# qintonguav/e2e-parking-carla

Measured on AMD Instinct MI355X. Metric: train samples/sec (4-cam frames) at B=8, 1/2/4/8 MI355X; CPU-ref baseline, higher is better.
Workload: dtype f32; 1 GPU; ParkingModel train step (fwd + control/seg/depth losses + bwd + Adam), 4 cams x 256x256, fp32, random init; global_batch=8, batch_per_gpu=8, parallelism=dp1

## Files before the change

e2e-parking-carla_amd/csrc/abi.cpp:

```cpp
#include <stdarg.h>
#include <stdio.h>

#include "e2ep.h"
#include "tune.h"

namespace e2ep {
static thread_local char g_err[512] = "";
void set_error(const char *fmt, ...) {
  va_list ap;
  va_start(ap, fmt);
  vsnprintf(g_err, sizeof(g_err), fmt, ap);
  va_end(ap);
}
int g_tune[TUNE_N] = {8192, 4096, 512, 512, 768, 1024, 512, 1, 1, 2, 1, 2, 2, 1, 2, 1, 1, 1, 1, 1, 1, 2, 1024, 2, 2048, 2, 1, 1, 2, 1, 2, 1, 1, 1, 1, 4, 2};
}

extern "C" {
int e2ep_abi_version(void) { return 4; }
int e2ep_tune(int key, int value) {
  if (key < 0 || key >= e2ep::TUNE_N || key == e2ep::TUNE_RETIRED_27 ||
      key == e2ep::TUNE_RETIRED_29 || key == e2ep::TUNE_RETIRED_31)
    return -1;
  const int prev = e2ep::g_tune[key];
  if (value > 0) e2ep::g_tune[key] = value;
  return prev;
}
const char *e2ep_last_error(void) { return e2ep::g_err; }
}
```

e2e-parking-carla_amd/csrc/conv.hip:

```cpp
#include <algorithm>

#include "common.h"
#include "conv.h"
#include "gemm.h"
#include "bnstats.h"
#include "handoff.h"

#pragma clang fp contract(on)

namespace e2ep {

typedef float f32x16 __attribute__((ext_vector_type(16)));
typedef __bf16 bf16x8 __attribute__((ext_vector_type(8)));
typedef _Float16 f16x8 __attribute__((ext_vector_type(8)));

constexpr int BM = 64, BK = 16;
constexpr int PADA = 4, PADB = 4;
constexpr int MAXPH = 4;
template <int BNT, int BMT>
constexpr int conv_gemm_lds_floats() { return 2 * BK * (BMT + PADA) + 2 * BK * (BNT + PADB); }

template <int MODE, int ACT, int BNT, int BMT, bool AV, int OP, bool ST, typename TS = float,
          typename TD = float>
__device__ __forceinline__ void conv_gemm_block(
    const float *__restrict__ w, const TS *__restrict__ src, const float *__restrict__ bias,
    TD *__restrict__ dst, long long dst_bytes, ConvGeom g, int M, int splits, int kper,
    float *__restrict__ part, unsigned int *__restrict__ cnt, double *__restrict__ stats, int bx,
    int by, int bz, int gx, float *lds) {
  constexpr int WC = BMT == 64 ? BNT / 2 : BNT / 4;
  constexpr int NACC = WC / 32;
  constexpr int BROWS = 256 / BNT;
  constexpr int BPER = BK / BROWS;
  constexpr int NA = BK * BMT / 256;
  float(*As)[BK][BMT + PADA] = reinterpret_cast<float(*)[BK][BMT + PADA]>(lds);
  float(*Bs)[BK][BNT + PADB] = reinterpret_cast<float(*)[BK][BNT + PADB]>(lds + 2 * BK * (BMT + PADA));
  __shared__ int s_tdy[MAXTAPS], s_tdx[MAXTAPS], s_trs[MAXTAPS];
  __shared__ int s_ntaps;

  const int tid = threadIdx.x, lane = tid & 63;
  const int wave = __builtin_amdgcn_readfirstlane(tid >> 6);
  const int wm = BMT == 64 ? (wave & 1) : 0, wn = BMT == 64 ? (wave >> 1) : wave;
  const int m0 = by * BMT, n0 = bx * BNT;
  const int split = bz % splits, z = bz / splits;
  const int RS = g.R * g.S;

  int py = 0, px = 0, Hc, Wc;
  if (MODE == 0) {
    Hc = g.P; Wc = g.Q;
  } else {
    py = z / g.sw; px = z % g.sw;
    Hc = py < g.H ? (g.H - py + g.sh - 1) / g.sh : 0;
    Wc = px < g.W ? (g.W - px + g.sw - 1) / g.sw : 0;
  }
  const int HWc = Hc * Wc;
  const int Ntot = g.N * HWc;
  if (n0 >= Ntot) return;

  if (tid == 0) {
    int n = 0;
    for (int r = 0; r < g.R; ++r) {
      int dy;
      if (MODE == 0) {
        dy = r * g.dh - g.ph;
      } else {
        const int ny = py + g.ph - r * g.dh;
        if (((ny % g.sh) + g.sh) % g.sh) continue;
        dy = floordiv(ny, g.sh);
      }
      for (int s = 0; s < g.S; ++s) {
        int dx;
        if (MODE == 0) {
          dx = s * g.dw - g.pw;
          if (!axis_live(dy, g.P, g.sh, g.H) || !axis_live(dx, g.Q, g.sw, g.W)) continue;
        } else {
          const int nx = px + g.pw - s * g.dw;
          if (((nx % g.sw) + g.sw) % g.sw) continue;
          dx = floordiv(nx, g.sw);
          if (!axis_live(dy, Hc, 1, g.P) || !axis_live(dx, Wc, 1, g.Q)) continue;
        }
        s_tdy[n] = dy;
        s_tdx[n] = dx;
        s_trs[n] = r * g.S + s;
        ++n;
      }
    }
    s_ntaps = n;
  }
  __syncthreads();
  const int ntaps = s_ntaps;
  const int Kc = MODE == 0 ? g.Cin : g.Cout;
  const int csteps = (Kc + BK - 1) / BK;
  const int ksteps_all = ntaps * csteps;
  const int kbeg = split * kper;
  const int kend = min(ksteps_all, kbeg + kper);
  const int nk = max(0, kend - kbeg);

  const int Hs = MODE == 0 ? g.H : g.P, Ws = MODE == 0 ? g.W : g.Q;
  const int HWs = Hs * Ws;
  constexpr int ES = sizeof(TS);
  const __amdgpu_buffer_rsrc_t rw = rsrc(w, 4LL * g.Cout * g.Cin * RS);
  const __amdgpu_buffer_rsrc_t rx = rsrc(src, (long long)ES * g.N * Kc * HWs);

  const int bn = tid % BNT;
  const int bk0 = __builtin_amdgcn_readfirstlane(tid / BNT);
  const int ncol = n0 + bn;
  const bool col_ok = ncol < Ntot;
  int img = 0, cp = 0;
  if (col_ok) {
    img = ncol / HWc;
    cp = ncol - img * HWc;
  }
  const int cy = cp / Wc, cx = cp - cy * Wc;
  const int ybase = MODE == 0 ? cy * g.sh : cy;
  const int xbase = MODE == 0 ? cx * g.sw : cx;
  const int simg = img * Kc * HWs;

  const int am = MODE == 0 ? tid / (BK / NA) : (tid & (BMT - 1));
  const int ac = MODE == 0 ? NA * (tid % (BK / NA)) : 0;
  const int ak0 = BMT == 64 ? __builtin_amdgcn_readfirstlane(tid / BMT) : tid / BMT;
  const bool arow_ok = (m0 + am) < M;
  const bool tm = g.wlayout == 1;
  const int a_mstride = MODE == 0 ? (tm ? g.Cin : g.Cin * RS) : (tm ? 1 : RS);
  const int a_cstride = MODE == 0 ? (tm ? 1 : RS) : (tm ? g.Cin : g.Cin * RS);
  const int a_tstride = tm ? g.Cout * g.Cin : 1;
  static_assert(!AV || (MODE == 0 && NA == 4), "AV: forward 64-row tiles only");
  const int arow = (m0 + am) * a_mstride;

  const int nrw = (int)min(4LL * g.Cout * g.Cin * RS, 0x7fffffffLL);
  const int nrx = (int)min((long long)ES * g.N * Kc * HWs, 0x7fffffffLL);

  float ra0[NA], rb0[BPER], ra1[NA], rb1[BPER];
  const int klast = kend - 1;
  auto load_tiles = [&](int ks_in, float(&ra)[NA], float(&rb)[BPER]) {
    const bool live = ks_in <= klast;
    const int ks = min(ks_in, klast);
    const int tap = g.korder ? ks % ntaps : ks / csteps;
    const int c0 = (g.korder ? ks / ntaps : ks - tap * csteps) * BK;
    const int dy = s_tdy[tap], dx = s_tdx[tap], rs = s_trs[tap] * a_tstride;
    if (MODE == 0) {
      const int c = c0 + ac;
      if (AV) {
        const float4 v = bload4(rw, (live && arow_ok && c < Kc) ? (arow + c + rs) * 4 : OOR);
        ra[0] = v.x; ra[1] = v.y; ra[NA > 2 ? 2 : 0] = v.z; ra[NA > 3 ? 3 : 0] = v.w;
      } else {
        const int abase = (live && arow_ok) ? (arow + rs) * 4 : nrw;
#pragma unroll
        for (int j = 0; j < NA; ++j)
          ra[j] = bload(rw, c + j < Kc ? abase + (c + j) * a_cstride * 4 : OOR);
      }
    } else {
      const int abase = (live && arow_ok) ? (arow + rs) * 4 : nrw;
#pragma unroll
      for (int j = 0; j < NA; ++j) {
        const int c = c0 + ak0 + (256 / BMT) * j;
        const int rterm = c < Kc ? c * a_cstride * 4 : nrw;
        ra[j] = bload(rw, abase + rterm);
      }
    }
    const int iy = ybase + dy, ix = xbase + dx;
// ... 785 lines not shown
  long long cap = pix / 2048;
  long long s = want < cap ? want : cap;
  if (s < 1) s = 1;
  if (s > 4096) s = 4096;
  return (int)s;
}

static void wgrad1x1_tiles(const ConvGeom &g, int &to, int &tc) {
  auto wide = [](int c) { return 8LL * cdiv(c, 64) * 64 <= 9LL * cdiv(c, 32) * 32; };
  to = tc = 32;
  if ((long long)g.N * g.P * g.Q < 65536) return;
  const int wo = wide(g.Cout) ? 64 : 32, wc = wide(g.Cin) ? 64 : 32;
  if ((long long)cdiv(g.Cout, wo) * cdiv(g.Cin, wc) * wgrad1x1_splits_for(g, wo, wc) < 128) return;
  to = wo;
  tc = wc;
}

static int wgrad1x1_splits(const ConvGeom &g) {
  int to, tc;
  wgrad1x1_tiles(g, to, tc);
  return wgrad1x1_splits_for(g, to, tc);
}

template <int TI, int TJ, int OP>
__device__ __forceinline__ void wgrad1x1_block(const float *__restrict__ gout,
                                               const float *__restrict__ x,
                                               float *__restrict__ part, ConvGeom g, int splits,
                                               int groups_per_split, int bt, int split,
                                               float (*red)[64]) {
  constexpr int NT = TI * TJ;
  const int lane = threadIdx.x & 63, wave = threadIdx.x >> 6;
  const int ntj = (g.Cin + 32 * TJ - 1) / (32 * TJ);
  const int ti = bt / ntj, tj = bt - ti * ntj;
  const int PQ = g.P * g.Q;
  const int ngroups = g.N * PQ / 8;
  const int gb = split * groups_per_split;
  const int ge = min(ngroups, gb + groups_per_split);
  const int row = lane & 31, h = lane >> 5;
  const int co0 = ti * 32 * TI + row, ci0 = tj * 32 * TJ + row;
  const __amdgpu_buffer_rsrc_t rg = rsrc(gout, 4LL * g.N * g.Cout * PQ);
  const __amdgpu_buffer_rsrc_t rx = rsrc(x, 4LL * g.N * g.Cin * PQ);
  const int gpq = PQ / 8;
  f32x16 acc[NT];
#pragma unroll
  for (int t = 0; t < NT; ++t) acc[t] = f32x16{0};
  for (int g0 = gb + wave * W1_GROUPS; g0 < ge; g0 += 4 * W1_GROUPS) {
    float4 a[W1_GROUPS][TI], b[W1_GROUPS][TJ];
#pragma unroll
    for (int u = 0; u < W1_GROUPS; ++u) {
      const int grp = g0 + u;
      const bool ok = grp < ge;
      const int n = grp / gpq, p = (grp - n * gpq) * 8 + 4 * h;
#pragma unroll
      for (int i = 0; i < TI; ++i) {
        const int co = co0 + 32 * i;
        a[u][i] = bload4(rg, (ok && co < g.Cout) ? (((n * g.Cout + co) * PQ) + p) * 4 : OOR);
      }
#pragma unroll
      for (int j = 0; j < TJ; ++j) {
        const int ci = ci0 + 32 * j;
        b[u][j] = bload4(rx, (ok && ci < g.Cin) ? (((n * g.Cin + ci) * PQ) + p) * 4 : OOR);
      }
    }
    if (OP == 0) {
#pragma unroll
      for (int u = 0; u < W1_GROUPS; ++u)
#pragma unroll
        for (int i = 0; i < TI; ++i)
#pragma unroll
          for (int j = 0; j < TJ; ++j) {
            f32x16 &c = acc[i * TJ + j];
            c = __builtin_amdgcn_mfma_f32_32x32x2f32(a[u][i].x, b[u][j].x, c, 0, 0, 0);
            c = __builtin_amdgcn_mfma_f32_32x32x2f32(a[u][i].y, b[u][j].y, c, 0, 0, 0);
            c = __builtin_amdgcn_mfma_f32_32x32x2f32(a[u][i].z, b[u][j].z, c, 0, 0, 0);
            c = __builtin_amdgcn_mfma_f32_32x32x2f32(a[u][i].w, b[u][j].w, c, 0, 0, 0);
          }
    } else {
#pragma unroll
      for (int u = 0; u < W1_GROUPS; u += 2)
#pragma unroll
        for (int i = 0; i < TI; ++i)
#pragma unroll
          for (int j = 0; j < TJ; ++j) {
            const bf16x8 av = {(__bf16)a[u][i].x, (__bf16)a[u][i].y, (__bf16)a[u][i].z,
                               (__bf16)a[u][i].w, (__bf16)a[u + 1][i].x, (__bf16)a[u + 1][i].y,
                               (__bf16)a[u + 1][i].z, (__bf16)a[u + 1][i].w};
            const bf16x8 bv = {(__bf16)b[u][j].x, (__bf16)b[u][j].y, (__bf16)b[u][j].z,
                               (__bf16)b[u][j].w, (__bf16)b[u + 1][j].x, (__bf16)b[u + 1][j].y,
                               (__bf16)b[u + 1][j].z, (__bf16)b[u + 1][j].w};
            acc[i * TJ + j] = __builtin_amdgcn_mfma_f32_32x32x16_bf16(av, bv, acc[i * TJ + j], 0, 0, 0);
          }
    }
  }
  for (int w = 0; w < 4; ++w) {
    if (wave == w)
#pragma unroll
      for (int t = 0; t < NT; ++t)
#pragma unroll
        for (int r = 0; r < 16; ++r)
          red[t * 16 + r][lane] = w == 0 ? acc[t][r] : red[t * 16 + r][lane] + acc[t][r];
    __syncthreads();
  }
  const int Kw = g.Cin;
  for (int e = threadIdx.x; e < NT * 16 * 64; e += 256) {
    const int tr = e >> 6, l = e & 63;
    const int t = tr >> 4, r = tr & 15;
    const int i = (r & 3) + 8 * (r >> 2) + 4 * (l >> 5), j = l & 31;
    const int oc = ti * 32 * TI + 32 * (t / TJ) + i, ic = tj * 32 * TJ + 32 * (t % TJ) + j;
    if (oc < g.Cout && ic < g.Cin) {
      part[((long long)split * g.Cout + oc) * Kw + ic] = red[tr][l];
    }
  }
}

template <int TI, int TJ, int OP>
__global__ void __launch_bounds__(256) k_wgrad_1x1(const float *__restrict__ gout,
                                                   const float *__restrict__ x,
                                                   float *__restrict__ part, ConvGeom g,
                                                   int splits, int groups_per_split) {
  __shared__ float red[TI * TJ * 16][64];
  wgrad1x1_block<TI, TJ, OP>(gout, x, part, g, splits, groups_per_split, blockIdx.x, blockIdx.y,
                             red);
}

template <int BNT, int BMT, int TI, int TJ>
__global__ void __launch_bounds__(256, 2) k_conv_bwd_pair1x1(
    const float *__restrict__ w, const float *__restrict__ gout, const float *__restrict__ res,
    float *__restrict__ dx, long long dx_bytes, ConvGeom g, int M, int splits, int kper,
    float *__restrict__ part1, unsigned int *__restrict__ cnt, int gx1, int gy1, int gz1,
    const float *__restrict__ x, float *__restrict__ part2, int splits2, int gps, int nt2,
    int wfirst) {
  constexpr int L1 = conv_gemm_lds_floats<BNT, BMT>();
  constexpr int L2 = TI * TJ * 16 * 64;
  __shared__ __attribute__((aligned(16))) float lds[L1 > L2 ? L1 : L2];
  const int n1 = gx1 * gy1 * gz1, n2 = nt2 * splits2;
  const int id = wfirst ? ((int)blockIdx.x >= n2 ? (int)blockIdx.x - n2 : n1 + (int)blockIdx.x)
                        : (int)blockIdx.x;
  if (id < n1) {
    conv_gemm_block<1, 0, BNT, BMT, false, 0, false>(w, gout, res, dx, dx_bytes, g, M, splits, kper,
                                                     part1, cnt, nullptr, id % gx1,
                                                     (id / gx1) % gy1, id / (gx1 * gy1), gx1, lds);
  } else {
    const int j = id - n1;
    wgrad1x1_block<TI, TJ, 0>(gout, x, part2, g, splits2, gps, j % nt2, j / nt2,
                              reinterpret_cast<float(*)[64]>(lds));
  }
}

__global__ void __launch_bounds__(1024) k_reduce_splits(const float *__restrict__ part, int splits,
                                                        int n, float *__restrict__ out,
                                                        int accumulate, int RS,
                                                        unsigned long long mask) {
  __shared__ float red[16][64];
  const int o = threadIdx.x & 63, r = threadIdx.x >> 6;
  const int i = blockIdx.x * 64 + o;
  const bool live = (mask >> (i % RS)) & 1ULL;
  float s0 = 0.f, s1 = 0.f, s2 = 0.f, s3 = 0.f;
  if (i < n && live) {
    int k = r;
    for (; k + 48 < splits; k += 64) {
      s0 += part[(size_t)(k + 0) * n + i];
      s1 += part[(size_t)(k + 16) * n + i];
      s2 += part[(size_t)(k + 32) * n + i];
      s3 += part[(size_t)(k + 48) * n + i];
    }
    for (; k < splits; k += 16) s0 += part[(size_t)k * n + i];
  }
  red[r][o] = (s0 + s1) + (s2 + s3);
  __syncthreads();
  if (r == 0 && i < n) {
    float s = 0.f;
#pragma unroll
    for (int j = 0; j < 16; ++j) s += red[j][o];
    out[i] = accumulate ? out[i] + s : s;
  }
}

__global__ void __launch_bounds__(256) k_reduce_splits4(const float *__restrict__ part, int splits,
                                                         int n, float *__restrict__ out,
                                                         int accumulate, int RS,
                                                         unsigned long long mask) {
  const int i = (blockIdx.x * 256 + threadIdx.x) * 4;
  if (i >= n) return;
  float4 acc = *reinterpret_cast<const float4 *>(part + i);
#pragma unroll 8
  for (int k = 1; k < splits; ++k) {
    const float4 v = *reinterpret_cast<const float4 *>(part + (size_t)k * n + i);
    acc.x += v.x;
    acc.y += v.y;
    acc.z += v.z;
    acc.w += v.w;
  }
  float r[4] = {acc.x, acc.y, acc.z, acc.w};
#pragma unroll
  for (int e = 0; e < 4; ++e)
    if (!((mask >> ((i + e) % RS)) & 1ULL)) r[e] = 0.f;
  float4 o = make_float4(r[0], r[1], r[2], r[3]);
  if (accumulate) {
    const float4 a = *reinterpret_cast<const float4 *>(out + i);
    o.x += a.x; o.y += a.y; o.z += a.z; o.w += a.w;
  }
  *reinterpret_cast<float4 *>(out + i) = o;
}

static void reduce_splits(const float *part, int splits, int n, float *out, int accumulate, int RS,
                          unsigned long long mask, hipStream_t s) {
  if (n % 4 == 0 && n >= 131072 && splits <= 64 && (reinterpret_cast<uintptr_t>(part) & 15) == 0 &&
      (reinterpret_cast<uintptr_t>(out) & 15) == 0)
    hipLaunchKernelGGL(k_reduce_splits4, dim3(cdiv(n / 4, 256)), dim3(256), 0, s, part, splits, n,
                       out, accumulate, RS, mask);
  else
    hipLaunchKernelGGL(k_reduce_splits, dim3(cdiv(n, 64)), dim3(1024), 0, s, part, splits, n, out,
                       accumulate, RS, mask);
}

constexpr int COLSUM_ROWS = 128;
__global__ void __launch_bounds__(256) k_col_sum_partial(const float *__restrict__ g, int rows,
                                                         int C, float *__restrict__ part) {
  const int tx = threadIdx.x & 63, ty = threadIdx.x >> 6;
  const int c = blockIdx.x * 64 + tx;
  const int r0 = blockIdx.y * COLSUM_ROWS, r1 = min(rows, r0 + COLSUM_ROWS);
  float s = 0.f;
  if (c < C) {
    float t[COLSUM_ROWS / 4];
#pragma unroll
    for (int u = 0; u < COLSUM_ROWS / 4; ++u) {
      const int r = r0 + ty + 4 * u;
      t[u] = r < r1 ? g[(long long)r * C + c] : 0.f;
    }
#pragma unroll
    for (int u = 0; u < COLSUM_ROWS / 4; ++u) s += t[u];
  }
  __shared__ float red[4][64];
  red[ty][tx] = s;
  __syncthreads();
  if (ty == 0 && c < C)
    part[(long long)blockIdx.y * C + c] = (red[0][tx] + red[1][tx]) + (red[2][tx] + red[3][tx]);
}

__global__ void k_col_sum_final(const float *__restrict__ part, int chunks, int C,
                                float *__restrict__ out) {
  const int c = blockIdx.x * blockDim.x + threadIdx.x;
  if (c >= C) return;
  float s = 0.f;
  for (int k0 = 0; k0 < chunks; k0 += 16) {
    float t[16];
#pragma unroll
    for (int u = 0; u < 16; ++u) t[u] = k0 + u < chunks ? part[(long long)(k0 + u) * C + c] : 0.f;
#pragma unroll
    for (int u = 0; u < 16; ++u) s += t[u];
  }
  out[c] = s;
}

__global__ void __launch_bounds__(1024) k_bias_grad(const float *__restrict__ g, int N, int C,
                                                    int HW, float *__restrict__ db) {
  const int c = blockIdx.x;
  float s = 0.f;
  if ((HW & 3) == 0) {
    const int HW4 = HW >> 2, tot = N * HW4;
    for (int t = threadIdx.x; t < tot; t += 1024) {
      const int n = t / HW4, p = t - n * HW4;
      const float4 v = *reinterpret_cast<const float4 *>(g + ((size_t)n * C + c) * HW + 4 * p);
      s += (v.x + v.y) + (v.z + v.w);
    }
  } else {
    const int tot = N * HW;
    for (int t = threadIdx.x; t < tot; t += 1024) {
      const int n = t / HW, p = t - n * HW;
      s += g[((size_t)n * C + c) * HW + p];
    }
  }
  __shared__ float red[16];
  s = wave_sum(s);
  if ((threadIdx.x & 63) == 0) red[threadIdx.x >> 6] = s;
  __syncthreads();
  if (threadIdx.x == 0) {
    float t = 0.f;
    for (int w = 0; w < 16; ++w) t += red[w];
    db[c] = t;
  }
}

__global__ void __launch_bounds__(256) k_skinny_gemm(const float *__restrict__ A, int ai, int ak,
                                                     const float *__restrict__ B, int bk, int bj,
                                                     const float *__restrict__ bias, int Mi, int Nj,
                                                     int K, float *__restrict__ C) {
  const int o = blockIdx.x * 4 + (threadIdx.x >> 6);
  if (o >= Mi * Nj) return;
  const int i = o / Nj, j = o - i * Nj;
  const int lane = threadIdx.x & 63;
  float s = 0.f;
  for (int k = lane; k < K; k += 64) s += A[(size_t)i * ai + (size_t)k * ak] * B[(size_t)k * bk + (size_t)j * bj];
  s = wave_sum(s);
  if (lane == 0) C[o] = s + (bias ? bias[j] : 0.f);
}

constexpr int DK = 32;

__device__ __forceinline__ int dk_w_index(const ConvGeom &g, int co, int k) {
  const int RS = g.R * g.S, ci = k / RS, rs = k - ci * RS;
  return g.wlayout == 1 ? (rs * g.Cout + co) * g.Cin + ci : (co * g.Cin + ci) * RS + rs;
}

__device__ __forceinline__ void dk_gather(const ConvGeom &g, const __amdgpu_buffer_rsrc_t &rx,
                                          int img, int oy, int ox, bool ok, float (&xin)[DK]) {
  const int RS = g.R * g.S, K = g.Cin * RS;
#pragma unroll
  for (int k = 0; k < DK; ++k) {
    const int ci = k / RS, rs = k - ci * RS, r = rs / g.S, sx = rs - r * g.S;
    const int iy = oy * g.sh - g.ph + r * g.dh, ix = ox * g.sw - g.pw + sx * g.dw;
    const bool in = ok && k < K && (unsigned)iy < (unsigned)g.H && (unsigned)ix < (unsigned)g.W;
    xin[k] = bload(rx, in ? (((img * g.Cin + ci) * g.H + iy) * g.W + ix) * 4 : OOR);
  }
}

constexpr int DCO = 64, DCH = 16;
__global__ void __launch_bounds__(256) k_conv_direct(const float *__restrict__ x,
                                                     const float *__restrict__ w,
                                                     const float *__restrict__ bias, ConvGeom g,
                                                     int act, float *__restrict__ y) {
  __shared__ float4 wl[DK][DCO / 4];
  __shared__ float xs[DK][256];
  const int K = g.Cin * g.R * g.S;
  for (int e = threadIdx.x; e < DK * DCO; e += 256) {
    const int k = e / DCO, co = e - k * DCO;
    reinterpret_cast<float *>(wl)[e] = (k < K && co < g.Cout) ? w[dk_w_index(g, co, k)] : 0.f;
  }
  const int PQ = g.P * g.Q;
  const int pix = blockIdx.x * 256 + threadIdx.x;
  const bool ok = pix < g.N * PQ;
  const int img = ok ? pix / PQ : 0, pq = ok ? pix - img * PQ : 0;
  const int oy = pq / g.Q, ox = pq - oy * g.Q;
  {
    const __amdgpu_buffer_rsrc_t rx = rsrc(x, 4LL * g.N * g.Cin * g.H * g.W);
    float xin[DK];
    dk_gather(g, rx, img, oy, ox, ok, xin);
#pragma unroll
    for (int k = 0; k < DK; ++k) xs[k][threadIdx.x] = xin[k];
  }
  __syncthreads();
  float *yp = y + (size_t)img * g.Cout * PQ + pq;
#pragma unroll 1
  for (int c0 = 0; c0 < g.Cout; c0 += DCH) {
    float acc[DCH];
#pragma unroll
    for (int j = 0; j < DCH; ++j) acc[j] = 0.f;
#pragma unroll 4
    for (int k = 0; k < K; ++k) {
      const float xv = xs[k][threadIdx.x];
#pragma unroll
      for (int j4 = 0; j4 < DCH / 4; ++j4) {
        const float4 wv = wl[k][c0 / 4 + j4];
        acc[4 * j4 + 0] = __builtin_fmaf(xv, wv.x, acc[4 * j4 + 0]);
        acc[4 * j4 + 1] = __builtin_fmaf(xv, wv.y, acc[4 * j4 + 1]);
        acc[4 * j4 + 2] = __builtin_fmaf(xv, wv.z, acc[4 * j4 + 2]);
        acc[4 * j4 + 3] = __builtin_fmaf(xv, wv.w, acc[4 * j4 + 3]);
      }
    }
    if (ok) {
#pragma unroll
// ... 753 lines not shown
```

e2e-parking-carla_amd/csrc/ln.hip:

```cpp
#include "common.h"
#include "dropout.h"

namespace e2ep {

constexpr int LN_MAXV = 8;

__global__ void __launch_bounds__(256) k_add_drop_ln_fwd(
    const float *__restrict__ a, const float *__restrict__ b, const float *__restrict__ u,
    const int *__restrict__ seed, float p, float scale, const float *__restrict__ gamma,
    const float *__restrict__ beta, int rows, int E, float eps, float *__restrict__ x,
    float *__restrict__ y, float *__restrict__ mean, float *__restrict__ rstd) {
  const int row = blockIdx.x * 4 + (threadIdx.x >> 6), lane = threadIdx.x & 63;
  if (row >= rows) return;
  const size_t base = (size_t)row * E;
  const bool hashed = !u && seed && p > 0.f;
  const uint32_t sm_ = hashed ? att_seedmix(seed) : 0u;
  float v[LN_MAXV];
  float s = 0.f;
#pragma unroll
  for (int j = 0; j < LN_MAXV; ++j) {
    const int c = lane + 64 * j;
    v[j] = 0.f;
    if (c < E) {
      float bv = b ? b[base + c] : 0.f;
      if (u) bv = u[base + c] >= p ? bv * scale : 0.f;
      else if (hashed) bv = att_keep(sm_, (uint32_t)(base + c), p) ? bv * scale : 0.f;
      v[j] = a[base + c] + bv;
      s += v[j];
    }
  }
  const float mu = wave_sum(s) / (float)E;
  float q = 0.f;
#pragma unroll
  for (int j = 0; j < LN_MAXV; ++j) {
    const int c = lane + 64 * j;
    if (c < E) {
      const float d = v[j] - mu;
      q += d * d;
    }
  }
  const float r = rsqrtf(wave_sum(q) / (float)E + eps);
#pragma unroll
  for (int j = 0; j < LN_MAXV; ++j) {
    const int c = lane + 64 * j;
    if (c < E) {
      if (x) x[base + c] = v[j];
      y[base + c] = (v[j] - mu) * r * (gamma ? gamma[c] : 1.f) + (beta ? beta[c] : 0.f);
    }
  }
  if (lane == 0) {
    mean[row] = mu;
    rstd[row] = r;
  }
}

constexpr int LN_ROWS_PER_WAVE = 1;

__global__ void __launch_bounds__(256) k_add_drop_ln_bwd(
    const float *__restrict__ dy, const float *__restrict__ x, const float *__restrict__ mean,
    const float *__restrict__ rstd, const float *__restrict__ gamma, const float *__restrict__ u,
    const int *__restrict__ seed, float p, float scale, int rows, int E, float *__restrict__ da,
    float *__restrict__ db, float *__restrict__ part) {
  const bool hashed = !u && seed && p > 0.f;
  const uint32_t sm_ = hashed ? att_seedmix(seed) : 0u;
  __shared__ float sg[4][LN_MAXV * 64], sb[4][LN_MAXV * 64];
  const int wave = threadIdx.x >> 6, lane = threadIdx.x & 63;
  float pg[LN_MAXV], pb[LN_MAXV];
#pragma unroll
  for (int j = 0; j < LN_MAXV; ++j) pg[j] = pb[j] = 0.f;
  const int r0 = (blockIdx.x * 4 + wave) * LN_ROWS_PER_WAVE;
  for (int i = 0; i < LN_ROWS_PER_WAVE; ++i) {
    const int row = r0 + i;
    if (row >= rows) break;
    const size_t base = (size_t)row * E;
    const float mu = mean[row], rs = rstd[row];
    float xh[LN_MAXV], gy[LN_MAXV];
    float s1 = 0.f, s2 = 0.f;
#pragma unroll
    for (int j = 0; j < LN_MAXV; ++j) {
      const int c = lane + 64 * j;
      xh[j] = gy[j] = 0.f;
      if (c < E) {
        const float g = dy[base + c];
        xh[j] = (x[base + c] - mu) * rs;
        gy[j] = g * (gamma ? gamma[c] : 1.f);
        pg[j] += g * xh[j];
        pb[j] += g;
        s1 += gy[j];
        s2 += gy[j] * xh[j];
      }
    }
    const float c1 = wave_sum(s1) / (float)E, c2 = wave_sum(s2) / (float)E;
#pragma unroll
    for (int j = 0; j < LN_MAXV; ++j) {
      const int c = lane + 64 * j;
      if (c < E) {
        const float dx = rs * (gy[j] - c1 - xh[j] * c2);
        if (da) da[base + c] = dx;
        if (db)
          db[base + c] = u        ? (u[base + c] >= p ? dx * scale : 0.f)
                         : hashed ? (att_keep(sm_, (uint32_t)(base + c), p) ? dx * scale : 0.f)
                                  : dx;
      }
    }
  }
  if (!part) return;
#pragma unroll
  for (int j = 0; j < LN_MAXV; ++j) {
    sg[wave][lane + 64 * j] = pg[j];
    sb[wave][lane + 64 * j] = pb[j];
  }
  __syncthreads();
  for (int c = threadIdx.x; c < E; c += 256) {
    part[(size_t)blockIdx.x * E + c] = (sg[0][c] + sg[1][c]) + (sg[2][c] + sg[3][c]);
    part[((size_t)gridDim.x + blockIdx.x) * E + c] = (sb[0][c] + sb[1][c]) + (sb[2][c] + sb[3][c]);
  }
}

__global__ void __launch_bounds__(1024) k_ln_param_grads(const float *__restrict__ part, int nblk,
                                                         int E, float *__restrict__ dgamma,
                                                         float *__restrict__ dbeta) {
  __shared__ float red[16][64];
  const int o = threadIdx.x & 63, r = threadIdx.x >> 6;
  const int c = blockIdx.x * 64 + o;
  const float *pp = part + (size_t)blockIdx.y * nblk * E;
  float s = 0.f;
  if (c < E)
    for (int k = r; k < nblk; k += 16) s += pp[(size_t)k * E + c];
  red[r][o] = s;
  __syncthreads();
  if (r == 0 && c < E) {
    float t = 0.f;
#pragma unroll
    for (int j = 0; j < 16; ++j) t += red[j][o];
    float *out = blockIdx.y == 0 ? dgamma : dbeta;
    if (out) out[c] = t;
  }
}

}

using namespace e2ep;

extern "C" {

static int add_drop_ln_fwd(const float *a, const float *b, const float *u, const int *seed,
                           float p, const float *gamma, const float *beta, int rows, int E,
                           float eps, float *x, float *y, float *mean, float *rstd,
                           hipStream_t stream) {
  E2EP_REQUIRE(rows > 0 && E > 0, E2EP_EINVAL, "e2ep_add_drop_ln_fwd: bad shape");
  E2EP_REQUIRE(E <= 64 * LN_MAXV, E2EP_ERANGE, "e2ep_add_drop_ln_fwd: E %d > %d", E, 64 * LN_MAXV);
  E2EP_REQUIRE(p >= 0.f && p < 1.f, E2EP_EINVAL, "e2ep_add_drop_ln_fwd: p must be in [0, 1)");
  E2EP_REQUIRE((long long)rows * E < 0xffffffffLL, E2EP_ERANGE, "e2ep_add_drop_ln_fwd: too large");
  const float scale = 1.f / (1.f - p);
  hipLaunchKernelGGL(k_add_drop_ln_fwd, dim3(cdiv(rows, 4)), dim3(256), 0, stream, a, b, u, seed,
                     p, scale, gamma, beta, rows, E, eps, x, y, mean, rstd);
  return launch_status("e2ep_add_drop_ln_fwd");
}

int e2ep_add_drop_ln_fwd(const float *a, const float *b, const float *u, float p,
                         const float *gamma, const float *beta, int rows, int E, float eps,
                         float *x, float *y, float *mean, float *rstd, void *stream) {
  return add_drop_ln_fwd(a, b, u, nullptr, p, gamma, beta, rows, E, eps, x, y, mean, rstd,
                         as_stream(stream));
}

int e2ep_add_drop_ln_fwd_seeded(const float *a, const float *b, const int *seed, float p,
                                const float *gamma, const float *beta, int rows, int E, float eps,
                                float *x, float *y, float *mean, float *rstd, void *stream) {
  E2EP_REQUIRE(seed || p == 0.f, E2EP_EINVAL, "e2ep_add_drop_ln_fwd_seeded: seed required for p > 0");
  return add_drop_ln_fwd(a, b, nullptr, seed, p, gamma, beta, rows, E, eps, x, y, mean, rstd,
                         as_stream(stream));
}

size_t e2ep_add_drop_ln_bwd_workspace(int rows, int E) {
  return (size_t)2 * cdiv(rows, 4 * LN_ROWS_PER_WAVE) * E * sizeof(float);
}

static int add_drop_ln_bwd(const float *dy, const float *x, const float *mean, const float *rstd,
                           const float *gamma, const float *u, const int *seed, float p, int rows,
                           int E, float *da, float *db, float *dgamma, float *dbeta,
                           void *workspace, hipStream_t stream) {
  E2EP_REQUIRE(rows > 0 && E > 0, E2EP_EINVAL, "e2ep_add_drop_ln_bwd: bad shape");
  E2EP_REQUIRE(E <= 64 * LN_MAXV, E2EP_ERANGE, "e2ep_add_drop_ln_bwd: E %d > %d", E, 64 * LN_MAXV);
  const float scale = 1.f / (1.f - p);
  const int nblk = cdiv(rows, 4 * LN_ROWS_PER_WAVE);
  float *part = (dgamma || dbeta) ? static_cast<float *>(workspace) : nullptr;
  E2EP_REQUIRE(!(dgamma || dbeta) || workspace, E2EP_EINVAL, "e2ep_add_drop_ln_bwd: workspace needed");
  hipLaunchKernelGGL(k_add_drop_ln_bwd, dim3(nblk), dim3(256), 0, stream, dy, x, mean, rstd,
                     gamma, u, seed, p, scale, rows, E, da, db, part);
  if (part)
    hipLaunchKernelGGL(k_ln_param_grads, dim3(cdiv(E, 64), 2), dim3(1024), 0, stream, part, nblk,
                       E, dgamma, dbeta);
  return launch_status("e2ep_add_drop_ln_bwd");
}

int e2ep_add_drop_ln_bwd(const float *dy, const float *x, const float *mean, const float *rstd,
                         const float *gamma, const float *u, float p, int rows, int E,
                         float *da, float *db, float *dgamma, float *dbeta, void *workspace,
                         void *stream) {
  return add_drop_ln_bwd(dy, x, mean, rstd, gamma, u, nullptr, p, rows, E, da, db, dgamma, dbeta,
                         workspace, as_stream(stream));
}

int e2ep_add_drop_ln_bwd_seeded(const float *dy, const float *x, const float *mean,
                                const float *rstd, const float *gamma, const int *seed, float p,
                                int rows, int E, float *da, float *db, float *dgamma,
                                float *dbeta, void *workspace, void *stream) {
  E2EP_REQUIRE(seed || p == 0.f, E2EP_EINVAL, "e2ep_add_drop_ln_bwd_seeded: seed required for p > 0");
  return add_drop_ln_bwd(dy, x, mean, rstd, gamma, nullptr, seed, p, rows, E, da, db, dgamma,
                         dbeta, workspace, as_stream(stream));
}

}
```

e2e-parking-carla_amd/csrc/se.hip:

```cpp
#include "common.h"

#pragma clang fp contract(on)

namespace e2ep {

constexpr int SE_MAXC = 4096, SE_MAXSQ = 256;
constexpr int SE_U = 4;

__device__ __forceinline__ float sigm(float v) { return sigmoid_f(v); }

struct SeIn {
  const float *sc, *sh;
  int C;
};
__device__ __forceinline__ float se_in(float v, float sc, float sh, bool t) {
  if (!t) return v;
  const float z = v * sc + sh;
  return swish_f(z);
}
__device__ __forceinline__ float4 se_in4(float4 v, float sc, float sh, bool t) {
  return make_float4(se_in(v.x, sc, sh, t), se_in(v.y, sc, sh, t), se_in(v.z, sc, sh, t),
                     se_in(v.w, sc, sh, t));
}

template <typename TX>
__device__ __forceinline__ float plane_sum(const TX *__restrict__ p, int HW, int lane,
                                           float sc, float sh, bool t) {
  float s = 0.f;
  if ((HW & 3) == 0) {
    const int HW4 = HW >> 2;
    for (int i0 = lane; i0 < HW4; i0 += 64 * SE_U) {
      float4 v[SE_U];
#pragma unroll
      for (int u = 0; u < SE_U; ++u) v[u] = ld4(p + 4 * min(i0 + u * 64, HW4 - 1));
#pragma unroll
      for (int u = 0; u < SE_U; ++u) {
        if (i0 + u * 64 >= HW4) break;
        const float4 w = se_in4(v[u], sc, sh, t);
        s += (w.x + w.y) + (w.z + w.w);
      }
    }
  } else {
    for (int i = lane; i < HW; i += 64) s += se_in(ld1(p + i), sc, sh, t);
  }
  return wave_sum(s);
}

template <typename TX>
__global__ void __launch_bounds__(256) k_se_squeeze(const TX *__restrict__ x, SeIn tf,
                                                    int planes, int HW,
                                                    float *__restrict__ pooled) {
  const int pl = blockIdx.x * 4 + (threadIdx.x >> 6);
  if (pl >= planes) return;
  const bool t = tf.sc != nullptr;
  const int c = pl % tf.C;
  const float s = plane_sum(x + (size_t)pl * HW, HW, threadIdx.x & 63, t ? tf.sc[c] : 1.f,
                            t ? tf.sh[c] : 0.f, t);
  if ((threadIdx.x & 63) == 0) pooled[pl] = s / (float)HW;
}

__global__ void __launch_bounds__(256) k_se_hidden(const float *__restrict__ pooled,
                                                   const float *__restrict__ w1,
                                                   const float *__restrict__ b1, int C, int sq,
                                                   float *__restrict__ hpre) {
  const int n = blockIdx.x, k = blockIdx.y * 4 + (threadIdx.x >> 6), lane = threadIdx.x & 63;
  if (k >= sq) return;
  const float *pn = pooled + (size_t)n * C, *wr = w1 + (size_t)k * C;
  float s0 = 0.f, s1 = 0.f;
  int c = lane;
  for (; c + 64 < C; c += 128) {
    s0 += wr[c] * pn[c];
    s1 += wr[c + 64] * pn[c + 64];
  }
  if (c < C) s0 += wr[c] * pn[c];
  const float s = wave_sum(s0 + s1);
  if (lane == 0) hpre[(size_t)n * sq + k] = s + (b1 ? b1[k] : 0.f);
}

constexpr int SE_CT = 32, SE_NT = 8;
__global__ void __launch_bounds__(256) k_se_logits(const float *__restrict__ hpre,
                                                   const float *__restrict__ w2,
                                                   const float *__restrict__ b2, int N, int C,
                                                   int sq, float *__restrict__ a) {
  extern __shared__ float lds[];
  const int ld = sq + 1;
  float *sw = lds, *sh = lds + SE_CT * ld;
  const int c0 = blockIdx.x * SE_CT, n0 = blockIdx.y * SE_NT;
  const int nc = min(SE_CT, C - c0), nn = min(SE_NT, N - n0);
  const float *src = w2 + (size_t)c0 * sq;
  for (int e = threadIdx.x; e < nc * sq; e += 256) {
    const int r = e / sq;
    sw[r * ld + (e - r * sq)] = src[e];
  }
  for (int e = threadIdx.x; e < nn * sq; e += 256) {
    const float z = hpre[(size_t)n0 * sq + e];
    sh[e] = z * sigm(z);
  }
  __syncthreads();
  const int ci = threadIdx.x % SE_CT, ni = threadIdx.x / SE_CT;
  if (ci >= nc || ni >= nn) return;
  const float *wr = sw + ci * ld, *hr = sh + ni * sq;
  float s = 0.f;
#pragma unroll 4
  for (int k = 0; k < sq; ++k) s += wr[k] * hr[k];
  a[(size_t)(n0 + ni) * C + c0 + ci] = s + (b2 ? b2[c0 + ci] : 0.f);
}

template <typename TX, typename TY = float>
__global__ void __launch_bounds__(256) k_se_excite(const TX *__restrict__ x, SeIn tf,
                                                   const float *__restrict__ a, int HW,
                                                   long long nvec, int vec,
                                                   TY *__restrict__ y) {
  const int i = (int)(blockIdx.x * blockDim.x + threadIdx.x);
  if (i >= nvec) return;
  const bool t = tf.sc != nullptr;
  const int pl = vec ? i / (HW >> 2) : i / HW;
  const int c = pl % tf.C;
  const float sc = t ? tf.sc[c] : 1.f, sh = t ? tf.sh[c] : 0.f;
  const float s = sigm(a[pl]);
  if (vec) {
    float4 v = se_in4(ld4(x + 4 * i), sc, sh, t);
    v.x *= s; v.y *= s; v.z *= s; v.w *= s;
    st4(y + 4 * i, v);
  } else {
    st1(y + i, se_in(ld1(x + i), sc, sh, t) * s);
  }
}

constexpr int SE_XP = 8;
template <typename TX, typename TY = float>
__global__ void __launch_bounds__(256) k_se_excite_mlp(const TX *__restrict__ x, SeIn tf,
                                                       const float *__restrict__ hpre,
                                                       const float *__restrict__ w2,
                                                       const float *__restrict__ b2, int sq,
                                                       float *__restrict__ a, int HW,
                                                       long long nvec, int vec,
                                                       TY *__restrict__ y) {
  __shared__ float sg[SE_XP];
  const int per = vec ? (HW >> 2) : HW;
  const int i0 = (int)(blockIdx.x * blockDim.x);
  const int last = (int)min((long long)i0 + (long long)blockDim.x, nvec) - 1;
  const int p0 = i0 / per, p1 = last / per;
  const int lane = threadIdx.x & 63, wv = threadIdx.x >> 6;
  for (int p = p0 + wv; p <= p1; p += 4) {
    const int n = p / tf.C, c = p - n * tf.C;
    const float *hr = hpre + (size_t)n * sq, *wr = w2 + (size_t)c * sq;
    float acc = 0.f;
    for (int k = lane; k < sq; k += 64) {
      const float z = hr[k];
      acc += wr[k] * (z * sigm(z));
    }
    acc = wave_sum(acc);
    const float av = acc + (b2 ? b2[c] : 0.f);
// ... 23 lines not shown
  const float *mean, *invstd, *gamma, *beta;
  double *sums;
};

template <bool BNS, typename TX, typename TD = float>
__global__ void __launch_bounds__(256) k_se_da(const TX *__restrict__ x, SeIn tf,
                                               const TD *__restrict__ dy,
                                               const float *__restrict__ a, int planes, int HW,
                                               float *__restrict__ da, SeBn bn) {
  const int pl = blockIdx.x * 4 + (threadIdx.x >> 6), lane = threadIdx.x & 63;
  if (pl >= planes) return;
  const bool t = tf.sc != nullptr;
  const int c = pl % tf.C;
  const float sc = t ? tf.sc[c] : 1.f, sh = t ? tf.sh[c] : 0.f;
  float mu = 0.f, is = 1.f, gm = 1.f, bt = 0.f;
  if constexpr (BNS) {
    mu = bn.mean[c];
    is = bn.invstd[c];
    gm = bn.gamma ? bn.gamma[c] : 1.f;
    bt = bn.beta ? bn.beta[c] : 0.f;
  }
  double s1 = 0.0, s2 = 0.0, s3 = 0.0, s4 = 0.0;
  const TX *xp = x + (size_t)pl * HW;
  const TD *gp = dy + (size_t)pl * HW;
  float acc = 0.f;
  if ((HW & 3) == 0) {
    const int HW4 = HW >> 2;
    for (int i0 = lane; i0 < HW4; i0 += 64 * SE_U) {
      float4 xv[SE_U], gv[SE_U];
#pragma unroll
      for (int u = 0; u < SE_U; ++u) {
        const int i = min(i0 + u * 64, HW4 - 1);
        xv[u] = ld4(xp + 4 * i);
        gv[u] = ld4(gp + 4 * i);
      }
#pragma unroll
      for (int u = 0; u < SE_U; ++u) {
        if (i0 + u * 64 >= HW4) break;
        const float4 g = gv[u];
        if constexpr (BNS) {
          const float xv4[4] = {xv[u].x, xv[u].y, xv[u].z, xv[u].w};
          const float gv4[4] = {g.x, g.y, g.z, g.w};
          float a0 = 0.f, a1 = 0.f, a2 = 0.f, a3 = 0.f, a4 = 0.f;
#pragma unroll
          for (int j = 0; j < 4; ++j) {
            const float xh = (xv4[j] - mu) * is;
            const float zb = xh * gm + bt;
            const float sg = sigmoid_f(zb);
            const float sp = sg * (1.f + zb * (1.f - sg));
            a0 += (zb * sg) * gv4[j];
            a1 += gv4[j] * sp;
            a2 += sp;
            a3 += gv4[j] * sp * xh;
            a4 += sp * xh;
          }
          acc += a0;
          s1 += a1; s2 += a2; s3 += a3; s4 += a4;
        } else {
          const float4 w = se_in4(xv[u], sc, sh, t);
          acc += (w.x * g.x + w.y * g.y) + (w.z * g.z + w.w * g.w);
        }
      }
    }
  } else {
    for (int i = lane; i < HW; i += 64) {
      const float xv = ld1(xp + i), g = ld1(gp + i);
      if constexpr (BNS) {
        const float xh = (xv - mu) * is;
        const float zb = xh * gm + bt;
        const float sg = sigmoid_f(zb);
        const float sp = sg * (1.f + zb * (1.f - sg));
        acc += (zb * sg) * g;
        s1 += g * sp; s2 += sp; s3 += g * sp * xh; s4 += sp * xh;
      } else {
        acc += se_in(xv, sc, sh, t) * g;
      }
    }
  }
  acc = wave_sum(acc);
  if constexpr (BNS) {
#pragma unroll
    for (int o = 32; o > 0; o >>= 1) {
      s1 += __shfl_xor(s1, o, 64);
      s2 += __shfl_xor(s2, o, 64);
      s3 += __shfl_xor(s3, o, 64);
      s4 += __shfl_xor(s4, o, 64);
    }
    if (lane == 0) {
      double *o = bn.sums + 4LL * pl;
      o[0] = s1; o[1] = s2; o[2] = s3; o[3] = s4;
    }
  }
  if (lane == 0) {
    const float s = sigm(a[pl]);
    da[pl] = acc * s * (1.f - s);
  }
}

constexpr int SE_DH_SPAN = 256;
static_assert(SE_MAXC / SE_DH_SPAN == 16, "e2ep_se_bwd workspace (e2ep.h) holds 16 dh partials");
__global__ void __launch_bounds__(256) k_se_dh(const float *__restrict__ da,
                                               const float *__restrict__ w2, int C, int sq, int KT,
                                               float *__restrict__ dhp) {
  __shared__ float red[256];
  const int n = blockIdx.x, j = blockIdx.y;
  const int k = threadIdx.x % KT, sl = threadIdx.x / KT, nsl = 256 / KT;
  const int cb = j * SE_DH_SPAN, ce = min(C, cb + SE_DH_SPAN);
  const float *dn = da + (size_t)n * C;
  float s = 0.f;
  if (k < sq)
#pragma unroll 4
    for (int c = cb + sl; c < ce; c += nsl) s += w2[(size_t)c * sq + k] * dn[c];
  red[threadIdx.x] = s;
  __syncthreads();
  if (threadIdx.x < KT && k < sq) {
    float t = 0.f;
    for (int q = 0; q < nsl; ++q) t += red[q * KT + k];
    dhp[((size_t)n * gridDim.y + j) * sq + k] = t;
  }
}

__global__ void __launch_bounds__(256) k_se_dpooled(const float *__restrict__ dhp, int spans,
                                                    const float *__restrict__ hpre,
                                                    const float *__restrict__ w1, int C, int sq,
                                                    float *__restrict__ dhpre,
                                                    float *__restrict__ dpooled) {
  __shared__ float sd[SE_MAXSQ];
  const int n = blockIdx.x;
  for (int k = threadIdx.x; k < sq; k += 256) {
    float t = 0.f;
    for (int j = 0; j < spans; ++j) t += dhp[((size_t)n * spans + j) * sq + k];
    const float z = hpre[(size_t)n * sq + k], sg = sigm(z);
    const float g = t * (sg * (1.f + z * (1.f - sg)));
    if (blockIdx.y == 0) dhpre[(size_t)n * sq + k] = g;
    sd[k] = g;
  }
  __syncthreads();
  const int c = blockIdx.y * 256 + threadIdx.x;
  if (c < C) {
    float s = 0.f;
#pragma unroll 8
    for (int k = 0; k < sq; ++k) s += w1[(size_t)k * C + c] * sd[k];
    dpooled[(size_t)n * C + c] = s;
  }
}

__global__ void __launch_bounds__(256) k_se_wgrad(const float *__restrict__ pooled,
                                                  const float *__restrict__ hpre,
                                                  const float *__restrict__ da,
                                                  const float *__restrict__ dhpre, int N, int C,
                                                  int sq, float *__restrict__ dw1,
                                                  float *__restrict__ db1, float *__restrict__ dw2,
                                                  float *__restrict__ db2) {
  const int i = blockIdx.x * blockDim.x + threadIdx.x;
  const int n1 = sq * C, n2 = C * sq;
  float s = 0.f;
  if (i < n1) {
    const int k = i / C, c = i - k * C;
#pragma unroll 8
    for (int n = 0; n < N; ++n) s += dhpre[(size_t)n * sq + k] * pooled[(size_t)n * C + c];
    if (dw1) dw1[i] = s;
  } else if (i < n1 + n2) {
    const int j = i - n1, c = j / sq, k = j - c * sq;
#pragma unroll 8
    for (int n = 0; n < N; ++n) {
      const float z = hpre[(size_t)n * sq + k];
      s += da[(size_t)n * C + c] * (z * sigm(z));
    }
    if (dw2) dw2[j] = s;
  } else if (i < n1 + n2 + sq) {
    const int k = i - n1 - n2;
#pragma unroll 8
    for (int n = 0; n < N; ++n) s += dhpre[(size_t)n * sq + k];
    if (db1) db1[k] = s;
  } else if (i < n1 + n2 + sq + C) {
    const int c = i - n1 - n2 - sq;
#pragma unroll 8
    for (int n = 0; n < N; ++n) s += da[(size_t)n * C + c];
    if (db2) db2[c] = s;
  }
}

__global__ void __launch_bounds__(256) k_se_dx(const float *__restrict__ dy,
                                               const float *__restrict__ a,
                                               const float *__restrict__ dpooled, int HW,
                                               long long nvec, int vec, float *__restrict__ dx) {
  const long long i = (long long)blockIdx.x * blockDim.x + threadIdx.x;
  if (i >= nvec) return;
  const float inv = 1.f / (float)HW;
  if (vec) {
    const long long pl = i / (HW >> 2);
    const float s = sigm(a[pl]), d = dpooled[pl] * inv;
    float4 g = reinterpret_cast<const float4 *>(dy)[i];
    g.x = g.x * s + d; g.y = g.y * s + d; g.z = g.z * s + d; g.w = g.w * s + d;
    reinterpret_cast<float4 *>(dx)[i] = g;
  } else {
    const long long pl = i / HW;
    dx[i] = dy[i] * sigm(a[pl]) + dpooled[pl] * inv;
  }
}

}

using namespace e2ep;

static int se_fwd_impl(const void *x, const float *x_scale, const float *x_shift, const float *w1,
                       const float *b1, const float *w2, const float *b2, int N, int C, int HW, int sq,
                       float *pooled, float *hpre, float *a, void *y, void *stream, int io,
                       bool squeeze) {
  E2EP_REQUIRE(io == 0 || ((io == E2EP_IO_X_BF16 || io == (E2EP_IO_X_BF16 | E2EP_IO_DX_BF16)) &&
                           HW % 4 == 0),
               E2EP_EINVAL, "e2ep_se_fwd: storage mask %d not supported (0, X or X|DX bf16, "
               "HW %% 4 == 0)", io);
  E2EP_REQUIRE(N > 0 && C > 0 && HW > 0 && sq > 0, E2EP_EINVAL, "e2ep_se_fwd: bad shape");
  E2EP_REQUIRE(!x_scale == !x_shift, E2EP_EINVAL, "e2ep_se_fwd: x_scale / x_shift both or neither");
  const SeIn tf{x_scale, x_shift, C};
  E2EP_REQUIRE(C <= SE_MAXC && sq <= SE_MAXSQ, E2EP_ERANGE, "e2ep_se_fwd: C %d > %d or sq %d > %d",
               C, SE_MAXC, sq, SE_MAXSQ);
  hipStream_t s = as_stream(stream);
  const int planes = N * C;
  const int vec = (HW & 3) == 0;
  const long long nvec = (long long)planes * HW / (vec ? 4 : 1);
  E2EP_REQUIRE(nvec < (1LL << 29), E2EP_ERANGE, "e2ep_se_fwd: %lld vectors >= 2^29", nvec);
  if (!squeeze)
    ;
  else if (io)
    hipLaunchKernelGGL(k_se_squeeze<bf16_t>, dim3(cdiv(planes, 4)), dim3(256), 0, s,
                       static_cast<const bf16_t *>(x), tf, planes, HW, pooled);
  else
    hipLaunchKernelGGL(k_se_squeeze<float>, dim3(cdiv(planes, 4)), dim3(256), 0, s,
                       static_cast<const float *>(x), tf, planes, HW, pooled);
  hipLaunchKernelGGL(k_se_hidden, dim3(N, cdiv(sq, 4)), dim3(256), 0, s, pooled, w1, b1, C, sq,
                     hpre);
  const int per = vec ? HW / 4 : HW;
  if (g_tune[TUNE_SE_EXCITE_MLP] == 2 && cdiv(256, per) + 1 <= SE_XP) {
#define E2EP_SEX(TXV, TYV)                                                                      \
  hipLaunchKernelGGL((k_se_excite_mlp<TXV, TYV>), dim3(cdiv(nvec, 256)), dim3(256), 0, s,       \
                     static_cast<const TXV *>(x), tf, hpre, w2, b2, sq, a, HW, nvec, vec,        \
                     static_cast<TYV *>(y))
    if (io & E2EP_IO_DX_BF16) E2EP_SEX(bf16_t, bf16_t);
    else if (io) E2EP_SEX(bf16_t, float);
    else E2EP_SEX(float, float);
#undef E2EP_SEX
    return launch_status("e2ep_se_fwd");
  }
  hipLaunchKernelGGL(k_se_logits, dim3(cdiv(C, SE_CT), cdiv(N, SE_NT)), dim3(256),
                     (SE_CT * (sq + 1) + SE_NT * sq) * sizeof(float), s, hpre, w2, b2, N, C, sq, a);
  if (io & E2EP_IO_DX_BF16)
    hipLaunchKernelGGL((k_se_excite<bf16_t, bf16_t>), dim3(cdiv(nvec, 256)), dim3(256), 0, s,
                       static_cast<const bf16_t *>(x), tf, a, HW, nvec, vec, static_cast<bf16_t *>(y));
  else if (io)
    hipLaunchKernelGGL((k_se_excite<bf16_t, float>), dim3(cdiv(nvec, 256)), dim3(256), 0, s,
                       static_cast<const bf16_t *>(x), tf, a, HW, nvec, vec, static_cast<float *>(y));
  else
    hipLaunchKernelGGL((k_se_excite<float, float>), dim3(cdiv(nvec, 256)), dim3(256), 0, s,
                       static_cast<const float *>(x), tf, a, HW, nvec, vec, static_cast<float *>(y));
  return launch_status("e2ep_se_fwd");
}

extern "C" {

int e2ep_se_fwd(const void *x, const float *x_scale, const float *x_shift, const float *w1,
                const float *b1, const float *w2, const float *b2, int N, int C, int HW, int sq,
                float *pooled, float *hpre, float *a, void *y, void *stream, int io) {
  return se_fwd_impl(x, x_scale, x_shift, w1, b1, w2, b2, N, C, HW, sq, pooled, hpre, a, y, stream,
                     io, true);
}

int e2ep_se_fwd_pooled(const void *x, const float *x_scale, const float *x_shift, const float *w1,
                       const float *b1, const float *w2, const float *b2, int N, int C, int HW,
                       int sq, const float *pooled, float *hpre, float *a, void *y, void *stream,
                       int io) {
  E2EP_REQUIRE(pooled, E2EP_EINVAL, "e2ep_se_fwd_pooled: pooled is required");
  return se_fwd_impl(x, x_scale, x_shift, w1, b1, w2, b2, N, C, HW, sq,
                     const_cast<float *>(pooled), hpre, a, y, stream, io, false);
}

static int se_bwd_impl(const void *x, int io, const float *x_scale, const float *x_shift,
                       const void *dy, const float *w1, const float *w2, const float *pooled,
                       const float *hpre, const float *a, int N, int C, int HW, int sq, float *dx,
                       float *dpooled_out, float *dw1, float *db1, float *dw2, float *db2,
                       float *workspace, const SeBn &bn, void *stream) {
  E2EP_REQUIRE(N > 0 && C > 0 && HW > 0 && sq > 0, E2EP_EINVAL, "e2ep_se_bwd: bad shape");
  E2EP_REQUIRE(!x_scale == !x_shift, E2EP_EINVAL, "e2ep_se_bwd: x_scale / x_shift both or neither");
  E2EP_REQUIRE(io == 0 || ((io == E2EP_IO_X_BF16 || io == (E2EP_IO_X_BF16 | E2EP_IO_DY_BF16)) &&
                           HW % 4 == 0 && !dx),
               E2EP_EINVAL, "e2ep_se_bwd: storage mask %d not supported (0, X or X|DY bf16 with "
               "dx formed by the BN backward, HW %% 4 == 0)", io);
  E2EP_REQUIRE(!(x_scale && dx), E2EP_EINVAL,
               "e2ep_se_bwd: with an input transform dx is formed by e2ep_bn_bwd (gate_logit / "
               "gate_dpooled); pass dx = NULL");
  const SeIn tf{x_scale, x_shift, C};
  E2EP_REQUIRE(C <= SE_MAXC && sq <= SE_MAXSQ, E2EP_ERANGE, "e2ep_se_bwd: C %d > %d or sq %d > %d",
               C, SE_MAXC, sq, SE_MAXSQ);
  hipStream_t s = as_stream(stream);
  const int planes = N * C;
  float *da = workspace, *dhpre = workspace + 2 * planes;
  float *dpooled = dpooled_out ? dpooled_out : workspace + planes;
  float *dhp = workspace + 2 * planes + N * sq;
  const int spans = cdiv(C, SE_DH_SPAN);
  int KT = 1;
  while (KT < sq) KT *= 2;
  const float *xf = static_cast<const float *>(x);
  const bf16_t *xh = static_cast<const bf16_t *>(x);
  const float *df = static_cast<const float *>(dy);
  const bf16_t *dh = static_cast<const bf16_t *>(dy);
  const dim3 gda(cdiv(planes, 4));
  const bool hx = io & E2EP_IO_X_BF16, hd = io & E2EP_IO_DY_BF16;
#define SE_DA(BNSV)                                                                                   \
  do {                                                                                                \
    if (hx && hd)                                                                                     \
      hipLaunchKernelGGL((k_se_da<BNSV, bf16_t, bf16_t>), gda, dim3(256), 0, s, xh, tf, dh, a, planes, \
                         HW, da, bn);                                                                 \
    else if (hx)                                                                                      \
      hipLaunchKernelGGL((k_se_da<BNSV, bf16_t, float>), gda, dim3(256), 0, s, xh, tf, df, a, planes, \
                         HW, da, bn);                                                                 \
    else                                                                                              \
      hipLaunchKernelGGL((k_se_da<BNSV, float, float>), gda, dim3(256), 0, s, xf, tf, df, a, planes,  \
                         HW, da, bn);                                                                 \
  } while (0)
  if (bn.sums) SE_DA(true);
  else SE_DA(false);
#undef SE_DA
  hipLaunchKernelGGL(k_se_dh, dim3(N, spans), dim3(256), 0, s, da, w2, C, sq, KT, dhp);
  hipLaunchKernelGGL(k_se_dpooled, dim3(N, cdiv(C, 256)), dim3(256), 0, s, dhp, spans, hpre, w1,
                     C, sq, dhpre, dpooled);
  if (dw1 || db1 || dw2 || db2) {
    const int outs = 2 * sq * C + sq + C;
    hipLaunchKernelGGL(k_se_wgrad, dim3(cdiv(outs, 256)), dim3(256), 0, s, pooled, hpre, da, dhpre,
                       N, C, sq, dw1, db1, dw2, db2);
  }
  if (dx) {
    const int vec = (HW & 3) == 0;
    const long long nvec = (long long)planes * HW / (vec ? 4 : 1);
    hipLaunchKernelGGL(k_se_dx, dim3(cdiv(nvec, 256)), dim3(256), 0, s, static_cast<const float *>(dy), a,
                       dpooled, HW, nvec, vec, dx);
  }
  return launch_status("e2ep_se_bwd");
}

int e2ep_se_bwd(const void *x, const float *x_scale, const float *x_shift, const void *dy,
                const float *w1, const float *w2, const float *pooled, const float *hpre,
                const float *a, int N, int C, int HW, int sq, float *dx, float *dpooled_out,
                float *dw1, float *db1, float *dw2, float *db2, float *workspace, void *stream,
                int io) {
  return se_bwd_impl(x, io, x_scale, x_shift, dy, w1, w2, pooled, hpre, a, N, C, HW, sq, dx,
                     dpooled_out, dw1, db1, dw2, db2, workspace, SeBn{}, stream);
}

int e2ep_se_bwd_bn(const void *x, const float *x_scale, const float *x_shift,
                   const float *bn_mean, const float *bn_invstd, const float *gamma,
                   const float *beta, const void *dy, const float *w1, const float *w2,
                   const float *pooled, const float *hpre, const float *a, int N, int C, int HW,
                   int sq, float *dpooled_out, float *dw1, float *db1, float *dw2, float *db2,
                   double *plane_sums, float *workspace, void *stream, int io) {
  E2EP_REQUIRE(x_scale && x_shift && bn_mean && bn_invstd && dpooled_out && plane_sums,
               E2EP_EINVAL, "e2ep_se_bwd_bn: the BN transform, its statistics, dpooled_out and "
               "plane_sums are required");
  return se_bwd_impl(x, io, x_scale, x_shift, dy, w1, w2, pooled, hpre, a, N, C, HW, sq, nullptr,
                     dpooled_out, dw1, db1, dw2, db2, workspace,
                     SeBn{bn_mean, bn_invstd, gamma, beta, plane_sums}, stream);
}

}
```

e2e-parking-carla_amd/csrc/tune.h:

```cpp
#pragma once

namespace e2ep {
enum Tune {
  TUNE_BN_SPLIT_TARGET = 0,
  TUNE_BN_SPLIT_MIN = 1,
  TUNE_BN_APPLY_PER = 2,
  TUNE_DW_WGRAD_TARGET = 3,
  TUNE_GEMM_SPLIT_TARGET = 4,
  TUNE_WGRAD1X1_TARGET = 5,
  TUNE_CONV_WIDE_MIN = 6,
  TUNE_CONV_FORCE_TILE = 7,
  TUNE_CONV_FORCE_SPLITS = 8,
  TUNE_WGRAD_GEN = 9,
  TUNE_LP_FORCE_TILE = 10,
  TUNE_LP = 11,
  TUNE_LP_WGRAD = 12,
  TUNE_LP_WGRAD_TILE = 13,
  TUNE_LP32 = 14,
  TUNE_LP32W = 15,
  TUNE_LP_LK = 16,
  TUNE_LPW_LK = 17,
  TUNE_KORDER = 18,
  TUNE_XCD = 19,
  TUNE_ATT_LANES = 20,
  TUNE_ATT_MF = 21,
  TUNE_LPW_TARGET = 22,
  TUNE_DW_VEC = 23,
  TUNE_DW_FWD_BLOCKS = 24,
  TUNE_BNS_WIDE = 25,
  TUNE_BNS_WIDE_LO = 26,
  TUNE_RETIRED_27 = 27,
  TUNE_SPLITK_FOLD = 28,
  TUNE_RETIRED_29 = 29,
  TUNE_PAIR1X1_ORDER = 30,
  TUNE_RETIRED_31 = 31,
  TUNE_LSS_FWD = 32,
  TUNE_BN_ORDER = 33,
  TUNE_SE_EXCITE_MLP = 34,
  TUNE_STEM_DIRECT = 35,
  TUNE_MBCONV_MID = 36,
  TUNE_N = 37
};
extern int g_tune[TUNE_N];
}
```

e2e-parking-carla_amd/e2ep_amd/_lib.py:

```python
import ctypes
import os

import torch

_HERE = os.path.dirname(os.path.abspath(__file__))
LIB_PATH = os.environ.get("E2EP_LIB", os.path.join(_HERE, "libe2ep_hip.so"))

_p, _i, _i64, _f, _sz = ctypes.c_void_p, ctypes.c_int, ctypes.c_longlong, ctypes.c_float, ctypes.c_size_t
_d = ctypes.c_double
_fp3 = ctypes.POINTER(ctypes.c_float)

SIGNATURES = {
    "e2ep_abi_version": (_i, []),
    "e2ep_last_error": (ctypes.c_char_p, []),
    "e2ep_rig_transforms": (_i, [_p, _p, _i, _p, _p, _p]),
    "e2ep_geom_index": (_i, [_p, _p, _p, _fp3, _fp3, _i, _i, _i, _i, _i, _i, _i, _i, _p, _p]),
    "e2ep_lss_plan_workspace": (_sz, [_i, _i]),
    "e2ep_lss_tiles": (_i, [_i]),
    "e2ep_debug_fwd_trace": (_i, [_p]),
    "e2ep_lss_plan": (_i, [_p, _i, _i, _i, _i, _i, _i, _p, _p, _p, _p, _sz, _p]),
    "e2ep_lss_fwd": (_i, [_p, _p, _p, _p, _p, _i, _i, _i, _i, _i, _i, _p, _i64, _p]),
    "e2ep_lss_bwd": (_i, [_p, _p, _p, _p, _i, _i, _i, _i, _i, _i, _p, _p, _p]),
    "e2ep_transpose": (_i, [_p, _i64, _i, _i, _i, _p, _p]),
    "e2ep_transpose_multi": (_i, [_p, _i, _i, _p]),
    "e2ep_target_bev": (_i, [_p, _p, _i, _i, _i, _f, _f, _p, _i64, _p]),
    "e2ep_conv_fwd_workspace": (_sz, [_p]),
    "e2ep_conv_fwd": (_i, [_p, _p, _p, _p, _i, _i, _p, _p, _sz, _p, _i]),
    "e2ep_conv_fwd_stats_tiles": (_i, [_p, _i]),
    "e2ep_conv_fwd_stats": (_i, [_p, _p, _p, _p, _i, _i, _p, _p, _sz, _p, _sz, _p, _i]),
    "e2ep_conv_dgrad_workspace": (_sz, [_p, _i]),
    "e2ep_conv_dgrad": (_i, [_p, _p, _p, _i, _i, _p, _p, _sz, _p]),
    "e2ep_conv_dgrad_acc": (_i, [_p, _p, _p, _i, _i, _p, _p, _p, _sz, _p, _i]),
    "e2ep_conv_gemm_variant": (_i, [_i]),
    "e2ep_conv_split_params": (_i, [_i, _i, _i]),
    "e2ep_conv_precision": (_i, [_i]),
    "e2ep_gemm_precision": (_i, [_i]),
    "e2ep_fusion_tokens_fwd": (_i, [_p, _p, _p, _i, _i, _i, _i, _f, _p, _p, _p]),
    "e2ep_fusion_tokens_bwd": (_i, [_p, _i, _i, _i, _i, _f, _p, _p, _p, _p, _p]),
    "e2ep_embed_tokens_fwd": (_i, [_p, _i, _p, _i, _p, _i, _i, _i, _f, _p, _p, _p]),
    "e2ep_embed_tokens_bwd": (_i, [_p, _p, _i, _i, _i, _i, _i, _f, _p, _p, _p, _p]),
    "e2ep_conv_wgrad_kstep": (_i, [_i]),
    "e2ep_conv_wgrad_splits": (_i, [_p]),
    "e2ep_conv_wgrad_workspace": (_sz, [_p, _i]),
    "e2ep_conv_wgrad": (_i, [_p, _p, _p, _i, _p, _sz, _p, _i, _p, _i]),
    "e2ep_conv_bwd_pair_ok": (_i, [_p, _i]),
    "e2ep_conv_bwd": (_i, [_p, _p, _p, _p, _i, _p, _p, _p, _sz, _i, _p, _sz, _p, _p, _i]),
    "e2ep_bias_grad": (_i, [_p, _i, _i, _i, _p, _p]),
    "e2ep_col_sum_workspace": (_sz, [_i, _i]),
    "e2ep_col_sum": (_i, [_p, _i, _i, _p, _p, _p]),
    "e2ep_skinny_gemm": (_i, [_p, _i, _i, _p, _i, _i, _p, _i, _i, _i, _p, _p]),
    "e2ep_bn_workspace": (_sz, [_i, _i, _i, _i]),
    "e2ep_bn_fwd": (_i, [_p, _p, _p, _p, _p, _f, _p, _p, _i, _i, _i, _i, _i, _f, _f, _i, _p, _p, _p, _p, _sz, _p]),
    "e2ep_bn_stats": (_i, [_p, _p, _p, _p, _p, _i, _i, _i, _i, _i, _f, _f, _p, _p, _p, _p, _p, _sz, _p, _i]),
    "e2ep_bn_fwd_split": (_i, [_i, _i, _i, _i]),
    "e2ep_bn_finalize_part_workspace": (_sz, [_i, _i]),
    "e2ep_bn_finalize_part": (_i, [_p, _i, _p, _p, _p, _p, _i, _i, _i, _i, _f, _f, _p, _p, _p, _p, _p, _sz, _p]),
    "e2ep_bn_apply": (_i, [_p, _p, _p, _p, _p, _f, _i, _i, _i, _i, _i, _p, _p]),
    "e2ep_bn_bwd": (_i, [_p, _p, _p, _p, _p, _p, _p, _p, _f, _p, _p, _i, _i, _i, _i, _i, _i, _p, _p, _p, _p, _p, _sz, _p, _i]),
    "e2ep_act_fwd": (_i, [_p, _i64, _i, _p, _p]),
    "e2ep_act_bwd": (_i, [_p, _p, _i64, _i, _p, _p]),
    "e2ep_cat_channels": (_i, [_p, _p, _i, _i, _i64, _p, _p]),
    "e2ep_split_channels": (_i, [_p, _p, _i, _i, _i64, _p, _p]),
    "e2ep_sum3": (_i, [_p, _p, _p, _p, _p]),
    "e2ep_add_f32": (_i, [_p, _p, _i64, _p, _p]),
    "e2ep_rng_draw": (_i, [_p, _i, _p, _i, _p, _p]),
    "e2ep_eq_mask_i64": (_i, [_p, _i64, _i, _i, _i64, _p, _p]),
    "e2ep_add_i64_multi": (_i, [_p, _i, _i64, _p]),
    "e2ep_resize_fwd": (_i, [_p, _i, _i, _i64, _i, _i, _i, _i, _f, _f, _p, _i64, _p]),
    "e2ep_resize_bwd_workspace": (_sz, [_i, _i, _i]),
    "e2ep_resize_bwd": (_i, [_p, _i64, _i, _i, _i, _i, _i, _f, _f, _p, _i, _p, _p]),
    "e2ep_resize_bwd_cl": (_i, [_p, _i64, _i, _i, _i, _i, _i, _i, _f, _f, _p, _p]),
    "e2ep_dwconv_fwd": (_i, [_p, _p, _p, _p, _p, _i, _p, _p]),
    "e2ep_dwconv_fwd_stats_tiles": (_i, [_p]),
    "e2ep_dwconv_fwd_stats": (_i, [_p, _p, _p, _p, _p, _i, _p, _p, _sz, _p, _i]),
    "e2ep_dwconv_dgrad": (_i, [_p, _p, _p, _p, _p, _i]),
    "e2ep_dwconv_wgrad_workspace": (_sz, [_p]),
    "e2ep_dwconv_wgrad": (_i, [_p, _p, _p, _p, _p, _i, _p, _sz, _p, _p, _i]),
    "e2ep_dwconv_bwd_pair_ok": (_i, [_p]),
    "e2ep_dwconv_bwd": (_i, [_p, _p, _p, _p, _p, _p, _i, _p, _p, _sz, _p, _p, _i]),
    "e2ep_maxpool3s2_fwd": (_i, [_p, _i, _i, _i, _p, _p, _p]),
    "e2ep_maxpool3s2_bwd": (_i, [_p, _p, _i, _i, _i, _p, _p]),
    "e2ep_avgpool_fwd": (_i, [_p, _i, _i, _p, _p]),
    "e2ep_avgpool_bwd": (_i, [_p, _i, _i, _p, _p]),
    "e2ep_add_drop_ln_fwd": (_i, [_p, _p, _p, _f, _p, _p, _i, _i, _f, _p, _p, _p, _p, _p]),
    "e2ep_add_drop_ln_bwd_workspace": (_sz, [_i, _i]),
    "e2ep_add_drop_ln_fwd_seeded": (_i, [_p, _p, _p, _f, _p, _p, _i, _i, _f, _p, _p, _p, _p, _p]),
    "e2ep_add_drop_ln_bwd_seeded": (_i, [_p, _p, _p, _p, _p, _p, _f, _i, _i, _p, _p, _p, _p, _p, _p]),
    "e2ep_add_drop_ln_bwd": (_i, [_p, _p, _p, _p, _p, _p, _f, _i, _i, _p, _p, _p, _p, _p, _p]),
    "e2ep_attn_fwd": (_i, [_p, _p, _p] + [_i] * 11 + [_f, _i, _p, _f, _p, _p, _p, _p]),
    "e2ep_attn_weights": (_i, [_p, _p, _p] + [_i] * 9 + [_f, _i, _p, _i, _p, _p]),
    "e2ep_attn_bwd_workspace": (_sz, [_i, _i, _i]),
    "e2ep_attn_bwd": (_i, [_p] * 6 + [_i] * 11 + [_f, _i, _p, _f, _p, _p, _p, _p, _p, _p]),
    "e2ep_attn_bwd_part": (_i, [_p] * 6 + [_i] * 11 + [_f, _i, _p, _f, _p, _p, _p, _p, _p, _i, _p]),
    "e2ep_attn_keep_mask": (_i, [_p, _i, _i, _i, _f, _p, _p]),
    "e2ep_softmax_c_fwd": (_i, [_p, _i, _i, _i, _p, _p]),
    "e2ep_softmax_c_bwd": (_i, [_p, _p, _i, _i, _i, _p, _p]),
    "e2ep_relu_dropout_fwd": (_i, [_p, _i64, _f, _p, _p, _p]),
    "e2ep_relu_dropout_bwd": (_i, [_p, _p, _i64, _f, _p, _p, _p]),
    "e2ep_se_fwd": (_i, [_p, _p, _p, _p, _p, _p, _p, _i, _i, _i, _i, _p, _p, _p, _p, _p, _i]),
    "e2ep_se_fwd_pooled": (_i, [_p, _p, _p, _p, _p, _p, _p, _i, _i, _i, _i, _p, _p, _p, _p, _p, _i]),
    "e2ep_mbconv_mid_ok": (_i, [_p]),
    "e2ep_mbconv_mid_fwd": (_i, [_p, _p, _p, _p, _p, _p, _p, _f, _f, _p, _p, _p, _p, _p, _f, _f, _p, _p, _p, _p]),
    "e2ep_mbconv_mid_bwd": (_i, [_p] * 20),
    "e2ep_se_bwd": (_i, [_p, _p, _p, _p, _p, _p, _p, _p, _p, _i, _i, _i, _i, _p, _p, _p, _p, _p, _p, _p, _p, _i]),
    "e2ep_se_bwd_bn": (_i, [_p, _p, _p, _p, _p, _p, _p, _p, _p, _p, _p, _p, _p, _i, _i, _i, _i, _p, _p, _p, _p, _p, _p, _p, _p, _i]),
    "e2ep_bn_bwd_planes": (_i, [_p, _p, _p, _p, _p, _p, _p, _p, _p, _i, _i, _i, _i, _i, _p, _p, _p, _p, _i]),
    "e2ep_bn_bwd_split": (_i, [_i, _i, _i, _i]),
    "e2ep_bn_eval_multi": (_i, [_p, _i, _p]),
    "e2ep_se_gate_fwd": (_i, [_p, _p, _i, _i, _p, _p]),
    "e2ep_se_gate_bwd": (_i, [_p, _p, _p, _i, _i, _p, _p, _p]),
    "e2ep_adam_chunk_elems": (_i, []),
    "e2ep_adam_step": (_i, [_p, _i, _p, _p, _p, _p, _p, _p, _p, _p, _d, _d, _d, _d, _f, _p, _p]),
    "e2ep_grad_gather": (_i, [_p, _i, _p, _p, _p, _p]),
    "e2ep_grad_sqnorm": (_i, [_p, _i, _p, _p, _p, _p, _p]),
    "e2ep_grad_norm_finalize": (_i, [_p, _i, _f, _d, _i, _p, _p, _p, _p, _p]),
    "e2ep_adam_step_clipped": (_i, [_p, _i, _p, _p, _p, _p, _p, _p, _p, _p, _d, _d, _d, _d, _f,
                                    _p, _p, _p, _p]),
    "e2ep_grad_accumulate": (_i, [_p, _i, _p, _p, _p, _p]),
    "e2ep_graph_replace_memsets": (_i, [_p, ctypes.POINTER(_i)]),
    "e2ep_graph_exec_create": (_i, [_p, _p]),
    "e2ep_graph_exec_launch": (_i, [_p, _p]),
    "e2ep_graph_exec_destroy": (_i, [_p]),
    "e2ep_capture_unjoined": (_i, [_p, _p, ctypes.POINTER(_i)]),
    "e2ep_tokens_init": (_i, [_p, _i, _i, _i, _p, _i, _i64, _p]),
    "e2ep_token_argmax_append": (_i, [_p, _i64, _i, _i, _p, _i, _i, _p]),
    "e2ep_dec_self_attn": (_i, [_p, _i, _p, _p, _f, _p, _i, _p, _p, _p, _i, _i64, _p, _p, _p, _p,
                                _i, _i, _i, _i, _i, _p]),
    "e2ep_dec_cross_attn": (_i, [_p, _i, _p, _p, _f, _p, _p, _p, _i, _p, _i, _i, _i, _i, _p]),
    "e2ep_dec_row_gemv": (_i, [_p, _i, _p, _p, _f, _p, _p, _p, _i, _p, _p, _f, _p, _i, _i, _i, _i,
                               _i, _p]),
    "e2ep_dwconv_bf16_ok": (_i, [_p]),
    "e2ep_control_ce_workspace": (_sz, [_i]),
    "e2ep_control_ce_fwd": (_i, [_p, _p, _i, _i, _i, _i, _i, _i, _p, _p, _p, _p, _p]),
    "e2ep_control_ce_bwd": (_i, [_p, _p, _p, _p, _p, _i, _i, _i, _i, _i, _i, _p, _p]),
    "e2ep_seg_ce_workspace": (_sz, [_i, _i]),
    "e2ep_seg_ce_fwd": (_i, [_p, _p, _p, _i, _i, _i, _i, _p, _p, _p]),
    "e2ep_seg_ce_bwd": (_i, [_p, _p, _p, _p, _i, _i, _i, _i, _p, _p]),
    "e2ep_depth_bce_workspace": (_sz, [_i, _i, _i, _i]),
    "e2ep_depth_bce_fwd": (_i, [_p, _p, _i, _i, _i, _i, _i, _f, _f, _p, _p, _p, _p, _p]),
    "e2ep_depth_bce_fwd_f64": (_i, [_p, _p, _i, _i, _i, _i, _i, _d, _d, _p, _p, _p, _p, _p]),
    "e2ep_gemm_workspace": (_sz, [_i, _i, _i]),
    "e2ep_gemm_force": (_i, [_i, _i, _i]),
    "e2ep_gemm_skinny": (_i, [_i]),
    "e2ep_gemm_split_min": (_i, [_i]),
    "e2ep_bn_small": (_i, [_i]),
    "e2ep_bn_small_limits": (_i, [_i, _i]),
    "e2ep_tune": (_i, [_i, _i]),
    "e2ep_gemm": (_i, [_p, _i, _i, _p, _i, _i, _p, _p, _i, _p, _i, _i, _i, _i, _i, _p, _sz, _p]),
    "e2ep_gemm_rowsum_workspace": (_sz, [_i, _i, _i]),
    "e2ep_gemm_rowsum": (_i, [_p, _i, _p, _i, _p, _i, _p, _i, _i, _i, _p, _sz, _p]),
    "e2ep_linear_bwd": (_i, [_p, _i, _p, _i, _p, _i, _p, _i, _p, _i, _p, _i, _p, _i, _i, _i, _p, _sz, _p, _sz, _p]),
    "e2ep_decode_frames": (_i, [_p, _p, _p, _i64, _i, _p, _p, _p]),
    "e2ep_widen_u8_i64": (_i, [_p, _p, _i64, _i, _p, _p]),
    "e2ep_depth_bce_bwd": (_i, [_p, _p, _p, _p, _i, _i, _i, _p, _p]),
    "e2ep_decode_bgra": (_i, [_p, _i, _i, _i, _i, _p, _p, _p]),
    "e2ep_slot_stats_workspace": (_sz, [_i, _i]),
    "e2ep_slot_partials": (_i, [_p, _i64, _i64, _i64, _i64, _i, _i, _i, _i, _i, _p, _p, _p, _sz, _p]),
    "e2ep_slot_finish": (_i, [_p, _sz, _i, _i, _i, _d, _d, _p, _p, _p, _p, _i, _i, _i, _i, _p, _p,
                              _p]),
    "e2ep_target_select": (_i, [_p, _p, _i, _p, _p]),
}

_LIB = None
_ERR = None


class E2EPError(RuntimeError):
    pass


def load():
    global _LIB, _ERR
    if _LIB is not None:
        return _LIB
    if _ERR is not None:
        raise _ERR
    try:
        lib = ctypes.CDLL(LIB_PATH, mode=ctypes.RTLD_GLOBAL)
        for name, (res, args) in SIGNATURES.items():
            fn = getattr(lib, name)
            fn.restype, fn.argtypes = res, args
    except (OSError, AttributeError) as e:
        _ERR = E2EPError(f"libe2ep_hip.so unavailable ({LIB_PATH}): {e}. Build it with "
                         f"`make -C e2e-parking-carla_amd/csrc` or __graft_entry__.build().")
        raise _ERR
    _LIB = lib
    if os.environ.get("E2EP_CONV_VARIANT"):
        lib.e2ep_conv_gemm_variant(int(os.environ["E2EP_CONV_VARIANT"]))
    if os.environ.get("E2EP_GEMM_SKINNY"):
        lib.e2ep_gemm_skinny(int(os.environ["E2EP_GEMM_SKINNY"]))
    if os.environ.get("E2EP_CONV_SPLIT"):
        v = [int(x) for x in os.environ["E2EP_CONV_SPLIT"].split(",")] + [0]
        lib.e2ep_conv_split_params(v[0], v[1], v[2])
    if os.environ.get("E2EP_BN_SMALL_LIMITS"):
        f, b = (int(x) for x in os.environ["E2EP_BN_SMALL_LIMITS"].split(","))
        lib.e2ep_bn_small_limits(f, b)
    if os.environ.get("E2EP_TUNE"):
        for kv in os.environ["E2EP_TUNE"].split(","):
            k, v = kv.split("=")
            lib.e2ep_tune(int(k), int(v))
    if os.environ.get("E2EP_GEMM_SPLIT_MIN"):
        lib.e2ep_gemm_split_min(int(os.environ["E2EP_GEMM_SPLIT_MIN"]))
    return lib


def call(name, *args):
    lib = load()
    rc = getattr(lib, name)(*args)
    if rc != 0:
        raise E2EPError(f"{name} failed ({rc}): {lib.e2ep_last_error().decode()}")


def call_raw(name, *args):
    return getattr(load(), name)(*args)


def ptr(t):
    return None if t is None else ctypes.c_void_p(t.data_ptr())


def nbytes(t):
    return 0 if t is None else t.numel() * t.element_size()


def stream():
    return ctypes.c_void_p(torch.cuda.current_stream().cuda_stream)


def dims(vals):
    return (ctypes.c_int * len(vals))(*[int(v) for v in vals])


def host3(vals):
    return (ctypes.c_float * 3)(*[float(v) for v in vals])
```

e2e-parking-carla_amd/e2ep_amd/bev_stem.py:

```python
import torch

from . import _lib, conv, timing


class _BevStem(torch.autograd.Function):
    @staticmethod
    def forward(ctx, bev, tgt, w, size):
        B, C, X, Y = bev.shape
        H, W = size
        assert bev.stride(3) == 1 and bev.stride(2) == Y and bev.stride(1) == X * Y
        tgt = tgt.contiguous()
        Cin = C + 1
        x = torch.empty(B, Cin, H, W, dtype=torch.float32, device=bev.device)
        s = _lib.stream()
        sh, sw = X / H, Y / W
        with timing.region("resize_fwd"):
            _lib.call("e2ep_resize_fwd", _lib.ptr(bev), B, C, bev.stride(0), X, Y, H, W, sh, sw,
                      _lib.ptr(x), Cin * H * W, s)
            _lib.call("e2ep_resize_fwd", _lib.ptr(tgt), B, 1, X * Y, X, Y, H, W, sh, sw,
                      _lib.ptr(x[:, C:]), Cin * H * W, s)
        Cout, _, R, S = w.shape
        P, Q = (H + 6 - R) // 2 + 1, (W + 6 - S) // 2 + 1
        dims = (B, Cin, H, W, Cout, R, S, P, Q, 2, 2, 3, 3, 1, 1)
        wt = conv.tap_major(w)
        y = conv.conv_fwd(x, wt, None, dims, 0,
                          torch.empty(B, Cout, P, Q, dtype=torch.float32, device=bev.device), w_layout=1)
        ctx.save_for_backward(x, w, wt)
        ctx.meta = (B, C, X, Y, H, W, sh, sw, dims)
        return y

    @staticmethod
    def backward(ctx, gy):
        x, w, wt = ctx.saved_tensors
        B, C, X, Y, H, W, sh, sw, dims = ctx.meta
        gy = gy.contiguous()
        s = _lib.stream()
        d = _lib.dims(dims)
        dbev = dw = None
        fork = None
        if ctx.needs_input_grad[2]:
            dw = torch.empty_like(w)
            ws = torch.empty(_lib.load().e2ep_conv_wgrad_splits(d) * dw.numel(), dtype=torch.float32,
                             device=gy.device)
            fork = conv._Fork(gy.device, on=ctx.needs_input_grad[0],
                              work_us=conv.est_us(conv.conv_flops(dims)))
            with fork:
                conv.conv_wgrad(gy, x, dims, dw, ws)
        if ctx.needs_input_grad[0]:
            dres = conv.conv_dgrad(gy, wt, dims, C,
                                   torch.empty(B, C, H, W, dtype=torch.float32, device=gy.device), w_layout=1)
            dbev = torch.empty(B, C, X, Y, dtype=torch.float32, device=gy.device,
                               memory_format=torch.channels_last)
            with timing.region("resize_bwd"):
                _lib.call("e2ep_resize_bwd_cl", _lib.ptr(dres), H * W, B, C, X, Y, H, W, sh, sw,
                          _lib.ptr(dbev), s)
        if fork is not None:
            fork.join()
        return dbev, None, dw, None


def bev_stem(bev, tgt, weight, size=(256, 256)):
    if not bev.is_cuda:
        raise _lib.E2EPError("e2ep bev_stem runs on a HIP device only")
    return _BevStem.apply(bev, tgt.detach(), weight, tuple(size))
```

e2e-parking-carla_amd/e2ep_amd/conv.py:

```python
import os

import torch

from . import _lib, streams, timing


def _ws(nbytes, device):
    return torch.empty(nbytes // 4, dtype=torch.float32, device=device) if nbytes else None


def _rname(kind, dims, extra=""):
    return f"{kind}{tuple(dims)}{extra}" if timing.detail() else kind


def conv_flops(dims, in_channels=None):
    N, Cin, H, W, Cout, R, S, P, Q = dims[:9]
    return 2.0 * N * Cout * P * Q * (in_channels or Cin) * R * S


class TapMajorBatch:

    def __init__(self):
        self.recorded = None
        self._log = None
        self._views = {}
        self._key = None
        self._table = None
        self._buf = None
        self._tiles = 0
        self.active = False

    def _build(self, ws):
        dev = ws[0].device
        sizes = [w.numel() for w in ws]
        self._buf = torch.empty(sum(sizes), dtype=torch.float32, device=dev)
        rows, off, tile0 = [], 0, 0
        views = []
        for w, n in zip(ws, sizes):
            Cout, Cin, R, S = w.shape
            v = self._buf[off:off + n].view(R * S, Cout, Cin)
            r, c = Cout * Cin, R * S
            ct = (c + 63) // 64
            rows.append([w.data_ptr(), v.data_ptr(), r, c, tile0, ct])
            tile0 += ((r + 63) // 64) * ct
            off += n
            views.append(v)
        self._table = torch.tensor(rows, dtype=torch.int64).to(dev)
        self._tiles = tile0
        self._key = [(w.data_ptr(), tuple(w.shape)) for w in ws]
        self._vlist = views

    def __enter__(self):
        ws = self.recorded
        if ws is None:
            self._log = []
        elif [(w.data_ptr(), tuple(w.shape)) for w in ws] != self._key:
            self.recorded, self._log = None, []
        else:
            _lib.call("e2ep_transpose_multi", _lib.ptr(self._table), len(ws), self._tiles,
                      _lib.stream())
            self._views = {id(w): v for w, v in zip(ws, self._vlist)}
        self.active = True
        _TAP_BATCH.append(self)
        return self

    def __exit__(self, *exc):
        _TAP_BATCH.pop()
        self.active = False
        self._views = {}
        if (self.recorded is None and self._log is not None and not exc[0]
                and not torch.cuda.is_current_stream_capturing()):
            log = [w for w in self._log if w.dtype == torch.float32 and w.is_contiguous()]
            if 0 < len(log) <= 256:
                self.recorded = log
                self._build(log)
        self._log = None
        return False

    def lookup(self, w):
        v = self._views.get(id(w))
        if v is None and self._log is not None and all(w is not o for o in self._log):
            self._log.append(w)
        return v


_TAP_BATCH = []


def tap_major(w):
    Cout, Cin, R, S = w.shape
    if R * S == 1:
        return w.contiguous()
    if _TAP_BATCH:
        v = _TAP_BATCH[-1].lookup(w)
        if v is not None:
            return v
    out = torch.empty(R * S, Cout, Cin, dtype=torch.float32, device=w.device)
    _lib.call("e2ep_transpose", _lib.ptr(w.contiguous()), Cout * Cin * R * S, 1, Cout * Cin, R * S,
              _lib.ptr(out), _lib.stream())
    return out


_IO_X, _IO_DX = 1, 4


def _io_x(x):
    return _IO_X if x.dtype == torch.bfloat16 else 0


def conv_fwd(x, w, b, dims, act, y, w_layout=0, stats=None):
    d = _lib.dims(dims)
    ws = _ws(_lib.load().e2ep_conv_fwd_workspace(d), x.device)
    with timing.region(_rname("conv_fwd", dims), conv_flops(dims)):
        if stats is None:
            _lib.call("e2ep_conv_fwd", _lib.ptr(x), _lib.ptr(w), _lib.ptr(b), d, act, w_layout,
                      _lib.ptr(y), _lib.ptr(ws), _lib.nbytes(ws), _lib.stream(), _io_x(x))
        else:
            _lib.call("e2ep_conv_fwd_stats", _lib.ptr(x), _lib.ptr(w), _lib.ptr(b), d, act, w_layout,
                      _lib.ptr(y), _lib.ptr(ws), _lib.nbytes(ws), _lib.ptr(stats),
                      _lib.nbytes(stats), _lib.stream(), _io_x(x))
    return y


_BN_STATS = [os.environ.get("E2EP_NO_BN_STATS", "0") in ("", "0")]


def bn_partials(y):
    return getattr(y, "_e2ep_bn_part", None)


def conv_dgrad(gy, w, dims, m_channels, dx, w_layout=0, res=None):
    d = _lib.dims(dims)
    ws = _ws(_lib.load().e2ep_conv_dgrad_workspace(d, m_channels), gy.device)
    with timing.region(_rname("conv_dgrad", dims, f"gc{m_channels}"), conv_flops(dims, m_channels)):
        _lib.call("e2ep_conv_dgrad_acc", _lib.ptr(gy), _lib.ptr(w), d, m_channels, w_layout,
                  _lib.ptr(res), _lib.ptr(dx), _lib.ptr(ws), _lib.nbytes(ws), _lib.stream(),
                  _IO_DX if dx.dtype == torch.bfloat16 else 0)
    return dx


def conv_wgrad(gy, x, dims, dw, ws=None):
    d = _lib.dims(dims)
    splits = _lib.load().e2ep_conv_wgrad_splits(d)
    if ws is None:
        ws = torch.empty(splits * dw.numel(), dtype=torch.float32, device=gy.device)
    with timing.region(_rname("conv_wgrad", dims), conv_flops(dims)):
        _lib.call("e2ep_conv_wgrad", _lib.ptr(gy), _lib.ptr(x), d, splits, _lib.ptr(ws), _lib.nbytes(ws),
                  _lib.ptr(dw), 0, _lib.stream(), _io_x(x))
    return dw


_SIDE = {}
_OVERLAP = [os.environ.get("E2EP_WGRAD_OVERLAP", "1") != "0"]
_FORK_MIN_US = [float(os.environ.get("E2EP_FORK_MIN_US", "0"))]


def est_us(flops=0.0, nbytes=0.0):
    return flops / 4e7 + nbytes / 3e6


def set_fork_min_us(us):
    prev = _FORK_MIN_US[0]
    _FORK_MIN_US[0] = float(us)
    return prev


def set_wgrad_overlap(on):
    prev = _OVERLAP[0]
    _OVERLAP[0] = bool(on)
    return prev


def wgrad_overlap():
    return _OVERLAP[0]


_WGRAD_STREAM = [os.environ.get("E2EP_WGRAD_STREAM", "own")]
_FORK_FROM_BRANCH = os.environ.get("E2EP_FORK_FROM_BRANCH", "0") == "1"


def side_stream(device):
    idx = device.index if device.index is not None else torch.cuda.current_device()
    if _WGRAD_STREAM[0] in ("cam", "heads"):
        return streams._side(torch.device("cuda", idx), _WGRAD_STREAM[0])
    key = (idx, torch.cuda.current_stream(idx).cuda_stream)
    st = _SIDE.get(key)
    if st is None:
        st = _SIDE[key] = torch.cuda.Stream(device=idx)
    return st


class _Fork:

    def __init__(self, device, on=True, work_us=float("inf")):
        self.main = torch.cuda.current_stream(device)
        self.on = (on and _OVERLAP[0] and work_us >= _FORK_MIN_US[0]
                   and (_FORK_FROM_BRANCH or not streams.is_branch_stream(self.main)))
        self.side = side_stream(device) if self.on else self.main

    def __enter__(self):
        if self.on:
            self.side.wait_stream(self.main)
            self._ctx = torch.cuda.stream(self.side)
            self._ctx.__enter__()
        return self

    def __exit__(self, *exc):
        if self.on:
            self._ctx.__exit__(*exc)
        return False

    def join(self):
        if self.on:
            self.main.wait_stream(self.side)


_CONV_PAIR = [os.environ.get("E2EP_CONV_PAIR", "1") != "0"]


def set_conv_pair(on):
    prev = _CONV_PAIR[0]
    _CONV_PAIR[0] = bool(on)
    return prev


def _conv_bwd_pair(gy, x, wt, dims, gc, gskip, wshape):
    N, Cin, H, W = dims[:4]
    lib = _lib.load()
    d = _lib.dims(dims)
    dw = torch.empty(wshape, dtype=torch.float32, device=x.device)
    splits = lib.e2ep_conv_wgrad_splits(d)
    wsw = torch.empty(splits * dw.numel(), dtype=torch.float32, device=x.device)
    wsd = _ws(lib.e2ep_conv_dgrad_workspace(d, gc), gy.device)
    res = gskip.contiguous() if (gskip is not None and gc == Cin) else None
    dxg = torch.empty(N, gc, H, W, dtype=x.dtype, device=x.device)
    with timing.region(_rname("conv_bwd", dims, f"gc{gc}"), conv_flops(dims, gc) + conv_flops(dims)):
        _lib.call("e2ep_conv_bwd", _lib.ptr(gy), _lib.ptr(x), _lib.ptr(wt), d, gc, _lib.ptr(res),
                  _lib.ptr(dxg), _lib.ptr(wsd), _lib.nbytes(wsd), splits, _lib.ptr(wsw),
                  _lib.nbytes(wsw), _lib.ptr(dw), _lib.stream(), (_IO_X | _IO_DX) if _io_x(x) else 0)
    if gc == Cin:
        dx = dxg
    elif gskip is not None:
        dx = gskip.clone()
        dx[:, :gc] += dxg
    else:
        dx = torch.zeros_like(x)
        dx[:, :gc] = dxg
    return dx, dw


class _Conv2d(torch.autograd.Function):
    @staticmethod
    def forward(ctx, x, w, b, dims, act, grad_channels, skip=False, stats=None):
        x = x.contiguous()
        wt = tap_major(w)
        N, Cin, H, W, Cout, R, S, P, Q = dims[:9]
        y = conv_fwd(x, wt, b, dims, act, torch.empty(N, Cout, P, Q, dtype=torch.float32, device=x.device),
                     w_layout=1, stats=stats)
        ctx.dims, ctx.act, ctx.has_bias, ctx.gc = dims, act, b is not None, grad_channels
        ctx.save_for_backward(x, wt, y if act else None)
        ctx.wshape = w.shape
        ctx.skip = skip
        ctx.set_materialize_grads(False)
        return (y, x) if skip else y

    @staticmethod
    def backward(ctx, gy, gskip=None):
        x, wt, y = ctx.saved_tensors
        dims = ctx.dims
        N, Cin, H, W, Cout, R, S, P, Q = dims[:9]
        gy = gy.contiguous()
        s = _lib.stream()
        if ctx.act == 1:
            gm = torch.empty_like(gy)
            _lib.call("e2ep_act_bwd", _lib.ptr(y), _lib.ptr(gy), gy.numel(), 1, _lib.ptr(gm), s)
            gy = gm
        dx = dw = db = None
        want_w, want_b = ctx.needs_input_grad[1], ctx.has_bias and ctx.needs_input_grad[2]
        gc = ctx.gc or Cin
        xb = x.dtype == torch.bfloat16
        if want_w and ctx.needs_input_grad[0] and _CONV_PAIR[0] and (not xb or gskip is None) and \
                _lib.load().e2ep_conv_bwd_pair_ok(_lib.dims(dims), gc):
            dx, dw = _conv_bwd_pair(gy, x, wt, dims, gc, gskip, ctx.wshape)
            if want_b:
                db = torch.empty(Cout, dtype=torch.float32, device=x.device)
                _lib.call("e2ep_bias_grad", _lib.ptr(gy), N, Cout, P * Q, _lib.ptr(db), s)
            return dx, dw, db, None, None, None, None, None
        fork = None
        if want_w or want_b:
            if want_w:
                dw = torch.empty(ctx.wshape, dtype=torch.float32, device=x.device)
                ws = torch.empty(_lib.load().e2ep_conv_wgrad_splits(_lib.dims(dims)) * dw.numel(),
                                 dtype=torch.float32, device=x.device)
            if want_b:
                db = torch.empty(Cout, dtype=torch.float32, device=x.device)
            fork = _Fork(x.device, on=ctx.needs_input_grad[0], work_us=est_us(conv_flops(dims)))
            with fork:
                if want_w:
                    conv_wgrad(gy, x, dims, dw, ws)
                if want_b:
                    _lib.call("e2ep_bias_grad", _lib.ptr(gy), N, Cout, P * Q, _lib.ptr(db),
                              _lib.stream())
        if ctx.needs_input_grad[0]:
            res = gskip.contiguous() if (gskip is not None and gc == Cin) else None
            dxg = conv_dgrad(gy, wt, dims, gc, torch.empty(N, gc, H, W, dtype=x.dtype, device=x.device),
                             w_layout=1, res=res)
            if gc == Cin:
                dx = dxg
            elif gskip is not None:
                dx = gskip.clone()
                dx[:, :gc] += dxg
            else:
                dx = torch.zeros_like(x)
                dx[:, :gc] = dxg
        if fork is not None:
            fork.join()
        if dx is None and gskip is not None and ctx.needs_input_grad[0]:
            dx = gskip
        return dx, dw, db, None, None, None, None, None


def _skinny(A, ai, ak, B, bk, bj, bias, Mi, Nj, K, out):
    _lib.call("e2ep_skinny_gemm", _lib.ptr(A), ai, ak, _lib.ptr(B), bk, bj, _lib.ptr(bias), Mi, Nj,
              K, _lib.ptr(out), _lib.stream())
    return out


class _Linear1x1(torch.autograd.Function):

    @staticmethod
    def forward(ctx, x, w, b):
        N, K = x.shape[0], x.shape[1]
        M = w.shape[0]
        x2 = x.reshape(N, K).contiguous()
        w2 = w.reshape(M, K).contiguous()
        y = torch.empty(N, M, dtype=torch.float32, device=x.device)
        _skinny(x2, K, 1, w2, 1, K, b, N, M, K, y)
        ctx.save_for_backward(x2, w2)
        ctx.has_bias, ctx.wshape, ctx.xshape = b is not None, w.shape, x.shape
        return y.view(N, M, 1, 1)

    @staticmethod
    def backward(ctx, gy):
        x2, w2 = ctx.saved_tensors
        N, K = x2.shape
        M = w2.shape[0]
        g = gy.reshape(N, M).contiguous()
        dx = dw = db = None
        if ctx.needs_input_grad[0]:
            dx = _skinny(g, M, 1, w2, K, 1, None, N, K, M,
                         torch.empty(N, K, dtype=torch.float32, device=g.device)).view(ctx.xshape)
        if ctx.needs_input_grad[1]:
            dw = _skinny(g, 1, M, x2, K, 1, None, M, K, N,
                         torch.empty(M, K, dtype=torch.float32, device=g.device)).view(ctx.wshape)
        if ctx.has_bias and ctx.needs_input_grad[2]:
            db = torch.empty(M, dtype=torch.float32, device=g.device)
            _lib.call("e2ep_bias_grad", _lib.ptr(g), N, M, 1, _lib.ptr(db), _lib.stream())
        return dx, dw, db


def conv2d(x, w, b=None, stride=(1, 1), pad=(0, 0, 0, 0), dilation=(1, 1), act=0, grad_channels=None,
           skip=False, bn_stats=False):
    if not x.is_cuda:
        raise _lib.E2EPError("e2ep conv2d runs on a HIP device only")
    N, Cin, H, W = x.shape
    Cout, cin_w, R, S = w.shape
    if cin_w != Cin:
        raise _lib.E2EPError(f"e2ep conv2d: groups must be 1 (w {tuple(w.shape)}, x {tuple(x.shape)})")
    if H == 1 and W == 1 and R == 1 and S == 1 and act == 0 and not any(pad) and grad_channels is None:
        y = _Linear1x1.apply(x, w, b)
        return (y, x) if skip else y
    sh, sw = stride
    dh, dw = dilation
    l, r, t, btm = pad
    P = (H + t + btm - dh * (R - 1) - 1) // sh + 1
    Q = (W + l + r - dw * (S - 1) - 1) // sw + 1
    dims = (N, Cin, H, W, Cout, R, S, P, Q, sh, sw, t, l, dh, dw)
    lib = _lib.load()
    tiles = (lib.e2ep_conv_fwd_stats_tiles(_lib.dims(dims), 1)
             if bn_stats and _BN_STATS[0] and lib.e2ep_bn_fwd_split(N, Cout, P, Q) else 0)
    if tiles <= 0:
        return _Conv2d.apply(x, w, b, dims, act, grad_channels, bool(skip))
    part = torch.empty(Cout * tiles * 2, dtype=torch.float64, device=x.device)
    out = _Conv2d.apply(x, w, b, dims, act, grad_channels, bool(skip), part)
    y = out[0] if skip else out
    y._e2ep_bn_part = (part, tiles)
    return out
```

e2e-parking-carla_amd/e2ep_amd/nn_ops.py:

```python
import ctypes
import os

import torch
import torch.nn.functional as F

from . import _lib, conv, rng, timing

ACT = {None: 0, "none": 0, "relu": 1, "swish": 2}


def _dev(*ts):
    for t in ts:
        if t is not None and not t.is_cuda:
            raise _lib.E2EPError("e2ep ops run on a HIP device only; got a CPU tensor")


def _ws(nbytes, device):
    return torch.empty(max(int(nbytes), 16), dtype=torch.uint8, device=device)


_IO_X, _IO_DY, _IO_DX = 1, 2, 4
_BF16_STORE = [int(os.environ.get("E2EP_BF16_STORE", "0"))]


def set_bf16_store(level):
    prev = _BF16_STORE[0]
    _BF16_STORE[0] = int(level) * (2 if level is True else 1)
    return prev


def _store_bf16(train, level=1):
    if not (train and _BF16_STORE[0] >= level):
        return False
    from . import precision
    return precision.get() == "bf16"


def _is_bf16(t):
    return t is not None and t.dtype == torch.bfloat16



class _BnAct(torch.autograd.Function):
    @staticmethod
    def forward(ctx, x, gamma, beta, res, rm, rv, train, momentum, eps, act, dc_rand, dc_keep,
                part=None, tiles=0):
        x = x.contiguous()
        res = res.contiguous() if res is not None else None
        N, C, H, W = x.shape
        y = torch.empty_like(x)
        if part is not None and train:
            st = torch.empty(4, C, dtype=torch.float32, device=x.device)
            mean, invstd = st[0], st[1]
            with timing.region(timing.name("bn_fwd", x.shape, "_BnAct")):
                fws = _ws(_lib.load().e2ep_bn_finalize_part_workspace(C, tiles), x.device)
                _lib.call("e2ep_bn_finalize_part", _lib.ptr(part), tiles, _lib.ptr(gamma),
                          _lib.ptr(beta), _lib.ptr(rm), _lib.ptr(rv), N, C, H, W, float(momentum),
                          float(eps), _lib.ptr(st[0]), _lib.ptr(st[1]), _lib.ptr(st[2]),
                          _lib.ptr(st[3]), _lib.ptr(fws), _lib.nbytes(fws), _lib.stream())
                _lib.call("e2ep_bn_apply", _lib.ptr(x), _lib.ptr(st[2]), _lib.ptr(st[3]),
                          _lib.ptr(res), _lib.ptr(dc_rand), float(dc_keep), N, C, H, W, act,
                          _lib.ptr(y), _lib.stream())
            ctx.save_for_backward(x, gamma, beta, res, mean, invstd, dc_rand)
            ctx.train, ctx.act, ctx.dc_keep = train, act, dc_keep
            return y
        mean = torch.empty(C, dtype=torch.float32, device=x.device)
        invstd = torch.empty_like(mean)
        ws = _ws(_lib.load().e2ep_bn_workspace(N, C, H, W), x.device)
        with timing.region(timing.name("bn_fwd", x.shape, "_BnAct")):
            _lib.call("e2ep_bn_fwd", _lib.ptr(x), _lib.ptr(gamma), _lib.ptr(beta), _lib.ptr(res),
                      _lib.ptr(dc_rand), float(dc_keep), _lib.ptr(rm), _lib.ptr(rv), N, C, H, W,
                      int(train), float(momentum), float(eps), act, _lib.ptr(mean),
                      _lib.ptr(invstd), _lib.ptr(y), _lib.ptr(ws), _lib.nbytes(ws), _lib.stream())
        ctx.save_for_backward(x, gamma, beta, res, mean, invstd, dc_rand)
        ctx.train, ctx.act, ctx.dc_keep = train, act, dc_keep
        return y

    @staticmethod
    def backward(ctx, dy):
        x, gamma, beta, res, mean, invstd, dc_rand = ctx.saved_tensors
        dy = dy.contiguous()
        N, C, H, W = x.shape
        nig = ctx.needs_input_grad
        dx = torch.empty_like(x) if nig[0] else None
        dg = torch.empty_like(gamma) if (gamma is not None and nig[1]) else None
        db = torch.empty_like(beta) if (beta is not None and nig[2]) else None
        dres_is_dy = res is not None and nig[3] and ctx.act == 0
        dres = torch.empty_like(x) if (res is not None and nig[3] and not dres_is_dy) else None
        ws = _ws(_lib.load().e2ep_bn_workspace(N, C, H, W), x.device)
        with timing.region(timing.name("bn_bwd", x.shape, "_BnAct")):
            _lib.call("e2ep_bn_bwd", _lib.ptr(x), _lib.ptr(dy), _lib.ptr(mean), _lib.ptr(invstd),
                      _lib.ptr(gamma), _lib.ptr(beta), _lib.ptr(res), _lib.ptr(dc_rand),
                      float(ctx.dc_keep), None, None, N, C, H, W, int(ctx.train), ctx.act, _lib.ptr(dx),
                      _lib.ptr(dg), _lib.ptr(db), _lib.ptr(dres), _lib.ptr(ws), _lib.nbytes(ws), _lib.stream(),
                      0)
        if dres_is_dy:
            dres = dy
        return dx, dg, db, dres, None, None, None, None, None, None, None, None, None, None


class BnCounters:

    def __init__(self):
        self.recorded = None
        self._log = None
        self.batched = False

    def __enter__(self):
        if self.recorded is None:
            self._log = []
        else:
            ctrs = [bn.num_batches_tracked for bn in self.recorded]
            key = tuple(c.data_ptr() for c in ctrs)
            if getattr(self, "_table_key", None) == key:
                _lib.call("e2ep_add_i64_multi", _lib.ptr(self._table), len(ctrs), 1, _lib.stream())
            else:
                torch._foreach_add_(ctrs, 1)
            self.batched = True
        _COUNTERS.append(self)
        return self

    def __exit__(self, *exc):
        _COUNTERS.pop()
        if self.recorded is None and self._log is not None and not exc[0]:
            self.recorded = self._log
            ctrs = [bn.num_batches_tracked for bn in self.recorded]
            if (ctrs and all(c.is_cuda and c.dtype == torch.int64 for c in ctrs)
                    and not torch.cuda.is_current_stream_capturing()):
                self._table = torch.tensor([c.data_ptr() for c in ctrs], dtype=torch.int64,
                                           device=ctrs[0].device)
                self._table_key = tuple(c.data_ptr() for c in ctrs)
        self._log = None
        self.batched = False
        return False

    def note(self, bn):
        if self.batched:
            return
        bn.num_batches_tracked.add_(1)
        if self._log is not None:
            self._log.append(bn)


_COUNTERS = []


class EvalBnBatch:

    def __init__(self):
        self.recorded = None
        self._log = None
        self._views = {}
        self._key = None
        self._table = None
        self._buf = None
        self.active = False

    @staticmethod
    def _key_of(bns):
# ... 294 lines not shown
                          _lib.ptr(db), None, _lib.ptr(ws), _lib.nbytes(ws), s, _IO_DY if hb else 0)
        if fork is not None:
            fork.join()
        return dx, dg, db, None, None, None, None, None, None, dw, None, None, None, None, None


def depthwise_conv2d(x, w, stride, pad, bn_stats=False):
    _dev(x)
    N, C, H, W = x.shape
    K = w.shape[-1]
    l, r, t, b = pad
    P = (H + t + b - K) // stride + 1
    Q = (W + l + r - K) // stride + 1
    dims = (N, C, H, W, K, P, Q, stride, t, l)
    ys, tiles = _dw_stats_buffer(dims, x.device, bn_stats)
    y = _DwConv.apply(x, w, dims, ys)
    if ys is not None:
        y._e2ep_bn_part = (ys, tiles)
    return y


def _dw_stats_buffer(dims, device, want):
    lib = _lib.load()
    if not want or not conv._BN_STATS[0] or not lib.e2ep_bn_fwd_split(dims[0], dims[1], dims[5], dims[6]):
        return None, 0
    tiles = lib.e2ep_dwconv_fwd_stats_tiles(_lib.dims(dims))
    if tiles <= 0:
        return None, 0
    return torch.empty(dims[1] * tiles * 2, dtype=torch.float64, device=device), tiles


def bn_act_depthwise_conv2d(x, bn, act, w, stride, pad, bn_stats=False):
    _dev(x)
    train = _bn_train_and_count(bn)
    rm = bn.running_mean if bn.track_running_stats else None
    rv = bn.running_var if bn.track_running_stats else None
    mom = bn.momentum if bn.momentum is not None else 0.1
    N, C, H, W = x.shape
    K = w.shape[-1]
    l, r, t, b = pad
    P = (H + t + b - K) // stride + 1
    Q = (W + l + r - K) // stride + 1
    pp = conv.bn_partials(x) if train else None
    dims = (N, C, H, W, K, P, Q, stride, t, l)
    ys, tiles = _dw_stats_buffer(dims, x.device, bn_stats)
    y = _BnActDwConv.apply(x, bn.weight, bn.bias, rm, rv, train, mom, bn.eps, ACT[act], w, dims,
                           *(pp or (None, 0)), ys, None if train else _eval_bn_stats(bn))
    if ys is not None:
        y._e2ep_bn_part = (ys, tiles)
    return y


class _MaxPool(torch.autograd.Function):
    @staticmethod
    def forward(ctx, x):
        x = x.contiguous()
        N, C, H, W = x.shape
        P, Q = (H - 1) // 2 + 1, (W - 1) // 2 + 1
        y = torch.empty(N, C, P, Q, dtype=torch.float32, device=x.device)
        arg = torch.empty(N, C, P, Q, dtype=torch.int8, device=x.device)
        _lib.call("e2ep_maxpool3s2_fwd", _lib.ptr(x), N * C, H, W, _lib.ptr(y), _lib.ptr(arg),
                  _lib.stream())
        ctx.save_for_backward(arg)
        ctx.shape = x.shape
        return y

    @staticmethod
    def backward(ctx, gy):
        (arg,) = ctx.saved_tensors
        N, C, H, W = ctx.shape
        dx = torch.empty(N, C, H, W, dtype=torch.float32, device=gy.device)
        _lib.call("e2ep_maxpool3s2_bwd", _lib.ptr(gy.contiguous()), _lib.ptr(arg), N * C, H, W,
                  _lib.ptr(dx), _lib.stream())
        return dx


def max_pool3s2(x):
    _dev(x)
    return _MaxPool.apply(x)


class _AvgPool(torch.autograd.Function):
    @staticmethod
    def forward(ctx, x):
        x = x.contiguous()
        N, C, H, W = x.shape
        y = torch.empty(N, C, 1, 1, dtype=torch.float32, device=x.device)
        _lib.call("e2ep_avgpool_fwd", _lib.ptr(x), N * C, H * W, _lib.ptr(y), _lib.stream())
        ctx.shape = x.shape
        return y

    @staticmethod
    def backward(ctx, gy):
        N, C, H, W = ctx.shape
        dx = torch.empty(N, C, H, W, dtype=torch.float32, device=gy.device)
        _lib.call("e2ep_avgpool_bwd", _lib.ptr(gy.contiguous()), N * C, H * W, _lib.ptr(dx),
                  _lib.stream())
        return dx


def global_avg_pool(x):
    _dev(x)
    return _AvgPool.apply(x)


class _SeGate(torch.autograd.Function):
    @staticmethod
    def forward(ctx, x, a):
        x = x.contiguous()
        a = a.contiguous()
        N, C, H, W = x.shape
        y = torch.empty_like(x)
        with timing.region(timing.name("se_gate_fwd", x.shape, "_SeGate")):
            _lib.call("e2ep_se_gate_fwd", _lib.ptr(x), _lib.ptr(a), N * C, H * W, _lib.ptr(y),
                      _lib.stream())
        ctx.save_for_backward(x, a)
        return y

    @staticmethod
    def backward(ctx, dy):
        x, a = ctx.saved_tensors
        N, C, H, W = x.shape
        dx = torch.empty_like(x)
        da = torch.empty_like(a)
        with timing.region(timing.name("se_gate_bwd", x.shape, "_SeGate")):
            _lib.call("e2ep_se_gate_bwd", _lib.ptr(x), _lib.ptr(a), _lib.ptr(dy.contiguous()), N * C,
                      H * W, _lib.ptr(dx), _lib.ptr(da), _lib.stream())
        return dx, da


def se_gate(x, a):
    _dev(x, a)
    return _SeGate.apply(x, a)


class _SqueezeExcite(torch.autograd.Function):
    @staticmethod
    def forward(ctx, x, w1, b1, w2, b2):
        x = x.contiguous()
        N, C, H, W = x.shape
        sq = w1.shape[0]
        dev = x.device
        pooled = torch.empty(N, C, dtype=torch.float32, device=dev)
        hpre = torch.empty(N, sq, dtype=torch.float32, device=dev)
        a = torch.empty(N, C, dtype=torch.float32, device=dev)
        y = torch.empty_like(x)
        w1c, w2c = w1.reshape(sq, C).contiguous(), w2.reshape(C, sq).contiguous()
        with timing.region(timing.name("se_fwd", x.shape, "_SqueezeExcite")):
            _lib.call("e2ep_se_fwd", _lib.ptr(x), None, None, _lib.ptr(w1c), _lib.ptr(b1), _lib.ptr(w2c),
                      _lib.ptr(b2), N, C, H * W, sq, _lib.ptr(pooled), _lib.ptr(hpre), _lib.ptr(a),
                      _lib.ptr(y), _lib.stream(), 0)
        ctx.save_for_backward(x, w1c, w2c, pooled, hpre, a)
        ctx.shapes = (w1.shape, w2.shape, b1 is not None, b2 is not None)
        return y

    @staticmethod
    def backward(ctx, dy):
        x, w1c, w2c, pooled, hpre, a = ctx.saved_tensors
        w1s, w2s, hb1, hb2 = ctx.shapes
        N, C, H, W = x.shape
        sq = w1c.shape[0]
        nig = ctx.needs_input_grad
        dev = x.device
        dx = torch.empty_like(x) if nig[0] else None
        dw1 = torch.empty(w1s, dtype=torch.float32, device=dev) if nig[1] else None
        db1 = torch.empty(sq, dtype=torch.float32, device=dev) if (hb1 and nig[2]) else None
        dw2 = torch.empty(w2s, dtype=torch.float32, device=dev) if nig[3] else None
        db2 = torch.empty(C, dtype=torch.float32, device=dev) if (hb2 and nig[4]) else None
        ws = torch.empty(2 * N * C + 17 * N * sq, dtype=torch.float32, device=dev)
        with timing.region(timing.name("se_bwd", x.shape, "_SqueezeExcite")):
            _lib.call("e2ep_se_bwd", _lib.ptr(x), None, None, _lib.ptr(dy.contiguous()),
                      _lib.ptr(w1c), _lib.ptr(w2c), _lib.ptr(pooled), _lib.ptr(hpre), _lib.ptr(a),
                      N, C, H * W, sq, _lib.ptr(dx), None, _lib.ptr(dw1), _lib.ptr(db1), _lib.ptr(dw2), _lib.ptr(db2),
                      _lib.ptr(ws), _lib.stream(), 0)
        return dx, dw1, db1, dw2, db2


_SE_BN_SUMS = [os.environ.get("E2EP_BN_SE_SUMS", "1") != "0"]


def set_se_bn_sums(on):
    prev = _SE_BN_SUMS[0]
    _SE_BN_SUMS[0] = bool(on)
    return prev


class _BnSwishSE(torch.autograd.Function):

    @staticmethod
    def forward(ctx, x, gamma, beta, rm, rv, train, momentum, eps, w1, b1, w2, b2, part=None,
                tiles=0, pre=None):
        x = x.contiguous()
        N, C, H, W = x.shape
        sq = w1.shape[0]
        dev = x.device
        f32 = dict(dtype=torch.float32, device=dev)
        stats = pre if pre is not None else torch.empty(4, C, **f32)
        s = _lib.stream()
        with timing.region(timing.name("bn_fwd", x.shape, "_BnSwishSE")):
            if pre is not None:
                pass
            elif part is not None and train:
                fws = _ws(_lib.load().e2ep_bn_finalize_part_workspace(C, tiles), x.device)
                _lib.call("e2ep_bn_finalize_part", _lib.ptr(part), tiles, _lib.ptr(gamma),
                          _lib.ptr(beta), _lib.ptr(rm), _lib.ptr(rv), N, C, H, W, float(momentum),
                          float(eps), _lib.ptr(stats[0]), _lib.ptr(stats[1]), _lib.ptr(stats[2]),
                          _lib.ptr(stats[3]), _lib.ptr(fws), _lib.nbytes(fws), s)
            else:
                ws = _ws(_lib.load().e2ep_bn_workspace(N, C, H, W), dev)
                _lib.call("e2ep_bn_stats", _lib.ptr(x), _lib.ptr(gamma), _lib.ptr(beta), _lib.ptr(rm),
                          _lib.ptr(rv), N, C, H, W, int(train), float(momentum), float(eps),
                          _lib.ptr(stats[0]), _lib.ptr(stats[1]), _lib.ptr(stats[2]),
                          _lib.ptr(stats[3]), _lib.ptr(ws), _lib.nbytes(ws), s,
                          _IO_X if _is_bf16(x) else 0)
        pooled, hpre, a = torch.empty(N, C, **f32), torch.empty(N, sq, **f32), torch.empty(N, C, **f32)
        hb = _is_bf16(x)
        yb = hb and _BF16_STORE[0] >= 2
        y = torch.empty(x.shape, dtype=torch.bfloat16 if yb else torch.float32, device=dev)
        w1c, w2c = w1.reshape(sq, C).contiguous(), w2.reshape(C, sq).contiguous()
        with timing.region(timing.name("se_fwd", x.shape, "_BnSwishSE")):
            _lib.call("e2ep_se_fwd", _lib.ptr(x), _lib.ptr(stats[2]), _lib.ptr(stats[3]),
                      _lib.ptr(w1c), _lib.ptr(b1), _lib.ptr(w2c), _lib.ptr(b2), N, C, H * W, sq,
                      _lib.ptr(pooled), _lib.ptr(hpre), _lib.ptr(a), _lib.ptr(y), s,
                      (_IO_X | (_IO_DX if yb else 0)) if hb else 0)
        ctx.save_for_backward(x, gamma, beta, stats, w1c, w2c, pooled, hpre, a)
        ctx.shapes = (w1.shape, w2.shape, b1 is not None, b2 is not None)
        ctx.train = train
        return y

    @staticmethod
    def backward(ctx, dy):
        x, gamma, beta, stats, w1c, w2c, pooled, hpre, a = ctx.saved_tensors
        w1s, w2s, hb1, hb2 = ctx.shapes
        N, C, H, W = x.shape
        sq = w1c.shape[0]
        nig = ctx.needs_input_grad
        dev = x.device
        f32 = dict(dtype=torch.float32, device=dev)
        dy = dy.contiguous()
        s = _lib.stream()
        dw1 = torch.empty(w1s, **f32) if nig[8] else None
        db1 = torch.empty(sq, **f32) if (hb1 and nig[9]) else None
        dw2 = torch.empty(w2s, **f32) if nig[10] else None
        db2 = torch.empty(C, **f32) if (hb2 and nig[11]) else None
        dpooled = torch.empty(N, C, **f32)
        ws = torch.empty(2 * N * C + 17 * N * sq, **f32)
        dx = torch.empty_like(x) if nig[0] else None
        dg = torch.empty_like(gamma) if (gamma is not None and nig[1]) else None
        db = torch.empty_like(beta) if (beta is not None and nig[2]) else None
        hb = _is_bf16(x)
        io_in = (_IO_X | (_IO_DY if _is_bf16(dy) else 0)) if hb else 0
        fused = (_SE_BN_SUMS[0] and ctx.train and dx is not None
                 and _lib.load().e2ep_bn_bwd_split(N, C, H, W) == 1)
        if fused:
            planes = torch.empty(N * C * 4, dtype=torch.float64, device=dev)
            with timing.region(timing.name("se_bwd", x.shape, "_BnSwishSE")):
                _lib.call("e2ep_se_bwd_bn", _lib.ptr(x), _lib.ptr(stats[2]), _lib.ptr(stats[3]),
                          _lib.ptr(stats[0]), _lib.ptr(stats[1]), _lib.ptr(gamma), _lib.ptr(beta),
                          _lib.ptr(dy), _lib.ptr(w1c), _lib.ptr(w2c), _lib.ptr(pooled),
                          _lib.ptr(hpre), _lib.ptr(a), N, C, H * W, sq, _lib.ptr(dpooled),
                          _lib.ptr(dw1), _lib.ptr(db1), _lib.ptr(dw2), _lib.ptr(db2),
                          _lib.ptr(planes), _lib.ptr(ws), s, io_in)
            with timing.region(timing.name("bn_bwd", x.shape, "_BnSwishSE")):
                _lib.call("e2ep_bn_bwd_planes", _lib.ptr(x), _lib.ptr(dy), _lib.ptr(stats[0]),
                          _lib.ptr(stats[1]), _lib.ptr(gamma), _lib.ptr(beta), _lib.ptr(a),
                          _lib.ptr(dpooled), _lib.ptr(planes), N, C, H, W, ACT["swish"],
                          _lib.ptr(dx), _lib.ptr(dg), _lib.ptr(db), s, (io_in | _IO_DX) if hb else 0)
            return dx, dg, db, None, None, None, None, None, dw1, db1, dw2, db2, None, None, None
        with timing.region(timing.name("se_bwd", x.shape, "_BnSwishSE")):
            _lib.call("e2ep_se_bwd", _lib.ptr(x), _lib.ptr(stats[2]), _lib.ptr(stats[3]),
                      _lib.ptr(dy), _lib.ptr(w1c), _lib.ptr(w2c), _lib.ptr(pooled),
                      _lib.ptr(hpre), _lib.ptr(a), N, C, H * W, sq, None, _lib.ptr(dpooled),
                      _lib.ptr(dw1), _lib.ptr(db1), _lib.ptr(dw2), _lib.ptr(db2), _lib.ptr(ws), s,
                      io_in)
        if dx is not None or dg is not None or db is not None:
            bws = _ws(_lib.load().e2ep_bn_workspace(N, C, H, W), dev)
            with timing.region(timing.name("bn_bwd", x.shape, "_BnSwishSE")):
                _lib.call("e2ep_bn_bwd", _lib.ptr(x), _lib.ptr(dy), _lib.ptr(stats[0]),
                          _lib.ptr(stats[1]), _lib.ptr(gamma), _lib.ptr(beta), None, None, 1.0,
                          _lib.ptr(a), _lib.ptr(dpooled), N, C, H, W, int(ctx.train), ACT["swish"],
                          _lib.ptr(dx), _lib.ptr(dg), _lib.ptr(db), None, _lib.ptr(bws), _lib.nbytes(bws), s,
                          (io_in | _IO_DX) if hb else 0)
        return dx, dg, db, None, None, None, None, None, dw1, db1, dw2, db2, None, None, None


def bn_swish_squeeze_excite(x, bn, w1, b1, w2, b2):
    _dev(x)
    train = _bn_train_and_count(bn)
    rm = bn.running_mean if bn.track_running_stats else None
    rv = bn.running_var if bn.track_running_stats else None
    mom = bn.momentum if bn.momentum is not None else 0.1
    pp = conv.bn_partials(x) if train else None
    return _BnSwishSE.apply(x, bn.weight, bn.bias, rm, rv, train, mom, bn.eps, w1, b1, w2, b2,
                            *(pp or (None, 0)), None if train else _eval_bn_stats(bn))


def _bn_trains(bn):
    return bn.training or not bn.track_running_stats


def _mid_dims(N, C, H, W, w, stride, pad):
    K = w.shape[-1]
    l, r, t, b = pad
    P = (H + t + b - K) // stride + 1
    Q = (W + l + r - K) // stride + 1
    return (N, C, H, W, K, P, Q, stride, t, l)


def mbconv_mid_ok(shape, dtype, bn0, bn1, w, stride, pad):
    if dtype != torch.float32 or not (_bn_trains(bn0) and _bn_trains(bn1)) or _store_bf16(True):
        return False
    return _lib.load().e2ep_mbconv_mid_ok(_lib.dims(_mid_dims(*shape, w, stride, pad))) == 1


class _MBConvMid(torch.autograd.Function):

    @staticmethod
    def forward(ctx, x, g0, b0, rm0, rv0, mom0, eps0, w, dims, g1, b1, rm1, rv1, mom1, eps1,
                w1, sb1, w2, sb2):
        x = x.contiguous()
        w = w.contiguous()
        N, C = dims[:2]
        sq = w1.shape[0]
        f32 = dict(dtype=torch.float32, device=x.device)
        st0, st1 = torch.empty(4, C, **f32), torch.empty(4, C, **f32)
        y1, pooled = torch.empty_like(x), torch.empty(N, C, **f32)
        s = _lib.stream()
        with timing.region(timing.name("mbconv_mid_fwd", x.shape, "_MBConvMid")):
            _lib.call("e2ep_mbconv_mid_fwd", _lib.ptr(x), _lib.ptr(w), _lib.dims(dims), _lib.ptr(g0),
                      _lib.ptr(b0), _lib.ptr(rm0), _lib.ptr(rv0), float(mom0), float(eps0),
                      _lib.ptr(st0), _lib.ptr(g1), _lib.ptr(b1), _lib.ptr(rm1), _lib.ptr(rv1),
                      float(mom1), float(eps1), _lib.ptr(st1), _lib.ptr(y1), _lib.ptr(pooled), s)
        hpre, a, y = torch.empty(N, sq, **f32), torch.empty(N, C, **f32), torch.empty_like(x)
        w1c, w2c = w1.reshape(sq, C).contiguous(), w2.reshape(C, sq).contiguous()
        with timing.region(timing.name("se_fwd", x.shape, "_MBConvMid")):
            _lib.call("e2ep_se_fwd_pooled", _lib.ptr(y1), _lib.ptr(st1[2]), _lib.ptr(st1[3]),
                      _lib.ptr(w1c), _lib.ptr(sb1), _lib.ptr(w2c), _lib.ptr(sb2), N, C, 256, sq,
                      _lib.ptr(pooled), _lib.ptr(hpre), _lib.ptr(a), _lib.ptr(y), s, 0)
        ctx.save_for_backward(x, y1, w, g0, b0, st0, g1, b1, st1, w1c, w2c, pooled, hpre, a)
        ctx.dims = dims
        ctx.shapes = (w1.shape, w2.shape, sb1 is not None, sb2 is not None)
        return y

    @staticmethod
    def backward(ctx, dy):
        x, y1, w, g0, b0, st0, g1, b1, st1, w1c, w2c, pooled, hpre, a = ctx.saved_tensors
        w1s, w2s, hb1, hb2 = ctx.shapes
        N, C = ctx.dims[:2]
        sq = w1c.shape[0]
        nig = ctx.needs_input_grad
        f32 = dict(dtype=torch.float32, device=x.device)
        dy = dy.contiguous()
        s = _lib.stream()
        dw1 = torch.empty(w1s, **f32) if nig[15] else None
        dsb1 = torch.empty(sq, **f32) if (hb1 and nig[16]) else None
        dw2 = torch.empty(w2s, **f32) if nig[17] else None
        dsb2 = torch.empty(C, **f32) if (hb2 and nig[18]) else None
        dpooled = torch.empty(N, C, **f32)
        ws = torch.empty(2 * N * C + 17 * N * sq, **f32)
        with timing.region(timing.name("se_bwd", x.shape, "_MBConvMid")):
            _lib.call("e2ep_se_bwd", _lib.ptr(y1), _lib.ptr(st1[2]), _lib.ptr(st1[3]), _lib.ptr(dy),
                      _lib.ptr(w1c), _lib.ptr(w2c), _lib.ptr(pooled), _lib.ptr(hpre), _lib.ptr(a),
                      N, C, 256, sq, None, _lib.ptr(dpooled), _lib.ptr(dw1), _lib.ptr(dsb1),
                      _lib.ptr(dw2), _lib.ptr(dsb2), _lib.ptr(ws), s, 0)
        dx, dw = torch.empty_like(x), torch.empty_like(w)
        dg0 = torch.empty_like(g0) if (g0 is not None and nig[1]) else None
        db0 = torch.empty_like(b0) if (b0 is not None and nig[2]) else None
        dg1 = torch.empty_like(g1) if (g1 is not None and nig[9]) else None
        db1 = torch.empty_like(b1) if (b1 is not None and nig[10]) else None
        with timing.region(timing.name("mbconv_mid_bwd", x.shape, "_MBConvMid")):
            _lib.call("e2ep_mbconv_mid_bwd", _lib.ptr(dy), _lib.ptr(a), _lib.ptr(dpooled),
                      _lib.ptr(y1), _lib.ptr(x), _lib.ptr(w), _lib.dims(ctx.dims), _lib.ptr(st1),
                      _lib.ptr(g1), _lib.ptr(b1), _lib.ptr(st0), _lib.ptr(g0), _lib.ptr(b0),
                      _lib.ptr(dx), _lib.ptr(dg1), _lib.ptr(db1), _lib.ptr(dg0), _lib.ptr(db0),
                      _lib.ptr(dw), s)
        return (dx if nig[0] else None, dg0, db0, None, None, None, None, dw if nig[7] else None,
                None, dg1, db1, None, None, None, None, dw1, dsb1, dw2, dsb2)


def mbconv_mid(x, bn0, w, stride, pad, bn1, w1, b1, w2, b2):
    _dev(x)
    _bn_train_and_count(bn0)
    _bn_train_and_count(bn1)

    def args(bn):
        rs = bn.track_running_stats
        return (bn.weight, bn.bias, bn.running_mean if rs else None, bn.running_var if rs else None,
                bn.momentum if bn.momentum is not None else 0.1, bn.eps)

    dims = _mid_dims(*x.shape, w, stride, pad)
    return _MBConvMid.apply(x, *args(bn0), w, dims, *args(bn1), w1, b1, w2, b2)


def squeeze_excite(x, w1, b1, w2, b2):
    _dev(x)
    return _SqueezeExcite.apply(x, w1, b1, w2, b2)


class _CatChannels(torch.autograd.Function):
    @staticmethod
    def forward(ctx, *xs):
        xs = [x.contiguous() for x in xs]
        N, _, H, W = xs[0].shape
        chans = [x.shape[1] for x in xs]
        y = torch.empty(N, sum(chans), H, W, dtype=torch.float32, device=xs[0].device)
        n = len(xs)
        _lib.call("e2ep_cat_channels", (ctypes.c_void_p * n)(*[x.data_ptr() for x in xs]),
                  (ctypes.c_int * n)(*chans), n, N, H * W, _lib.ptr(y), _lib.stream())
        ctx.chans = chans
        return y

    @staticmethod
    def backward(ctx, g):
        g = g.contiguous()
        N, _, H, W = g.shape
        outs = [torch.empty(N, c, H, W, dtype=torch.float32, device=g.device) for c in ctx.chans]
        n = len(outs)
        _lib.call("e2ep_split_channels", _lib.ptr(g), (ctypes.c_int * n)(*ctx.chans), n, N, H * W,
                  (ctypes.c_void_p * n)(*[o.data_ptr() for o in outs]), _lib.stream())
        return tuple(outs)


def cat_channels(xs):
    _dev(*xs)
    if (len(xs) > 8 or any(x.dim() != 4 or x.dtype != torch.float32 for x in xs)
            or (xs[0].shape[2] * xs[0].shape[3]) % 4):
        return torch.cat(xs, 1)
    return _CatChannels.apply(*xs)


class _Transpose12(torch.autograd.Function):

    @staticmethod
    def forward(ctx, x):
        x = x.contiguous()
        B, R, C = x.shape
        out = torch.empty(B, C, R, dtype=torch.float32, device=x.device)
        _lib.call("e2ep_transpose", _lib.ptr(x), R * C, B, R, C, _lib.ptr(out), _lib.stream())
        return out

    @staticmethod
    def backward(ctx, g):
        g = g.contiguous()
        B, C, R = g.shape
        dx = torch.empty(B, R, C, dtype=torch.float32, device=g.device)
        _lib.call("e2ep_transpose", _lib.ptr(g), R * C, B, C, R, _lib.ptr(dx), _lib.stream())
        return dx


def transpose12(x):
    _dev(x)
    return _Transpose12.apply(x)


class _Fork2(torch.autograd.Function):
    @staticmethod
    def forward(ctx, x):
        return x.view_as(x), x.view_as(x)

    @staticmethod
    def backward(ctx, g1, g2):
        if g1 is None or g2 is None:
            return g2 if g1 is None else g1
        g1, g2 = g1.contiguous(), g2.contiguous()
        out = torch.empty_like(g1)
        _lib.call("e2ep_add_f32", _lib.ptr(g1), _lib.ptr(g2), g1.numel(), _lib.ptr(out),
                  _lib.stream())
        return out


def fork2(x):
    _dev(x)
    return _Fork2.apply(x)


class _Sum3(torch.autograd.Function):
    @staticmethod
    def forward(ctx, a, b, c):
        out = torch.empty((), dtype=torch.float32, device=a.device)
        _lib.call("e2ep_sum3", _lib.ptr(a), _lib.ptr(b), _lib.ptr(c), _lib.ptr(out), _lib.stream())
        return out

    @staticmethod
    def backward(ctx, g):
        return g, g, g


def sum3(a, b, c):
    _dev(a, b, c)
    return _Sum3.apply(a, b, c)


def eq_mask(tok, value):
    if tok.dtype != torch.int64 or tok.dim() != 2 or tok.stride(1) != 1 or not tok.is_cuda:
        raise _lib.E2EPError("eq_mask: (B, T) int64 device tensor with unit column stride")
    B, T = tok.shape
    m = torch.empty(B, T, dtype=torch.bool, device=tok.device)
    _lib.call("e2ep_eq_mask_i64", _lib.ptr(tok), tok.stride(0), B, T, int(value), _lib.ptr(m),
              _lib.stream())
    return m


class _AddDropLN(torch.autograd.Function):
    @staticmethod
    def forward(ctx, a, b, gamma, beta, u, seed, p, eps):
        a = a.contiguous()
        b = b.contiguous()
        E = a.shape[-1]
        rows = a.numel() // E
        x = torch.empty_like(a)
        y = torch.empty_like(a)
        mean = torch.empty(rows, dtype=torch.float32, device=a.device)
        rstd = torch.empty_like(mean)
        fn, mask = ("e2ep_add_drop_ln_fwd", u) if seed is None else ("e2ep_add_drop_ln_fwd_seeded", seed)
        with timing.region(timing.name("ln_fwd", a.shape, "_AddDropLN")):
            _lib.call(fn, _lib.ptr(a), _lib.ptr(b), _lib.ptr(mask), float(p),
                      _lib.ptr(gamma), _lib.ptr(beta), rows, E, float(eps), _lib.ptr(x), _lib.ptr(y),
                      _lib.ptr(mean), _lib.ptr(rstd), _lib.stream())
        ctx.save_for_backward(x, mean, rstd, gamma, mask)
        ctx.p, ctx.rows, ctx.E, ctx.seeded = float(p), rows, E, seed is not None
        return y

    @staticmethod
    def backward(ctx, dy):
        x, mean, rstd, gamma, mask = ctx.saved_tensors
        nig = ctx.needs_input_grad
        da = torch.empty_like(x) if nig[0] else None
        db = torch.empty_like(x) if nig[1] else None
        dg = torch.empty_like(gamma) if (gamma is not None and nig[2]) else None
        dbeta = torch.empty_like(gamma) if (gamma is not None and nig[3]) else None
        ws = _ws(_lib.load().e2ep_add_drop_ln_bwd_workspace(ctx.rows, ctx.E), x.device)
        with timing.region(timing.name("ln_bwd", x.shape, "_AddDropLN")):
            _lib.call("e2ep_add_drop_ln_bwd_seeded" if ctx.seeded else "e2ep_add_drop_ln_bwd",
                      _lib.ptr(dy.contiguous()), _lib.ptr(x), _lib.ptr(mean),
                      _lib.ptr(rstd), _lib.ptr(gamma), _lib.ptr(mask), ctx.p, ctx.rows, ctx.E,
                      _lib.ptr(da), _lib.ptr(db), _lib.ptr(dg), _lib.ptr(dbeta), _lib.ptr(ws),
                      _lib.stream())
        return da, db, dg, dbeta, None, None, None, None


def add_drop_layer_norm(a, b, norm, p=0.0, u=None, seed=None):
    _dev(a, b)
    if p > 0.0 and u is None and seed is None:
        seed = rng.seed(a.device)
    if p == 0.0:
        u = seed = None
    return _AddDropLN.apply(a, b, norm.weight, norm.bias, u, seed, p, norm.eps)


def gemm(A, a_kcontig, B, b_kcontig, M, N, K, bias=None, cadd=None, out=None, relu=False,
         tag="gemm", ws=None):
    for t, n in ((A, "A"), (B, "B")):
        if t.dim() != 2 or t.stride(1) != 1 or t.dtype != torch.float32:
            raise _lib.E2EPError(f"gemm: {n} must be a 2-D fp32 matrix with unit inner stride")
    want_a = (M, K) if a_kcontig else (K, M)
    want_b = (N, K) if b_kcontig else (K, N)
    if tuple(A.shape) != want_a or tuple(B.shape) != want_b:
        raise _lib.E2EPError(f"gemm: A {tuple(A.shape)} / B {tuple(B.shape)} vs M={M} N={N} K={K}")
    if out is None:
        out = torch.empty(M, N, dtype=torch.float32, device=A.device)
    if cadd is not None and (cadd.shape != (M, N) or cadd.stride(1) != 1):
        raise _lib.E2EPError("gemm: cadd must be (M, N) with unit inner stride")
    if ws is None:
        ws = _ws(_lib.load().e2ep_gemm_workspace(M, N, K), A.device)
    with timing.region(timing.name("gemm", (M, N, K), tag), 2.0 * M * N * K):
        _lib.call("e2ep_gemm", _lib.ptr(A), A.stride(0), int(a_kcontig), _lib.ptr(B), B.stride(0),
                  int(b_kcontig), _lib.ptr(bias), _lib.ptr(cadd),
                  cadd.stride(0) if cadd is not None else 0, _lib.ptr(out), out.stride(0), M, N, K,
                  int(relu), _lib.ptr(ws), _lib.nbytes(ws), _lib.stream())
    return out


class _Linear(torch.autograd.Function):

    @staticmethod
    def forward(ctx, x, weight, bias, skip=False, relu=False):
        K = x.shape[-1]
        x2 = x.reshape(-1, K)
        if x2.stride(1) != 1 or x2.stride(0) != K:
            x2 = x2.contiguous()
        N = weight.shape[0]
        y = gemm(x2, True, weight, True, x2.shape[0], N, K, bias=bias, relu=relu, tag="linear_fwd")
        ctx.save_for_backward(x2, weight, y if relu else None)
        ctx.has_bias, ctx.relu, ctx.xshape = bias is not None, relu, x.shape
        y = y.view(*x.shape[:-1], N)
        return (y, x) if skip else y

    @staticmethod
    def backward(ctx, gy, gskip=None):
        x2, weight, y = ctx.saved_tensors
        nig = ctx.needs_input_grad
        M, K = x2.shape
        N = weight.shape[0]
        g2 = gy.reshape(M, N)
        if g2.stride(1) != 1 or g2.stride(0) != N:
            g2 = g2.contiguous()
        if ctx.relu:
            gr = torch.empty_like(g2)
            _lib.call("e2ep_act_bwd", _lib.ptr(y), _lib.ptr(g2), g2.numel(), 1, _lib.ptr(gr),
                      _lib.stream())
            g2 = gr
        dx, dw, db = _linear_bwd(g2, x2, weight, nig[0], nig[1], ctx.has_bias and nig[2], gskip)
        return (dx.view(ctx.xshape) if dx is not None else None), dw, db, None, None


_PAIR = [os.environ.get("E2EP_LINEAR_PAIR", "1") != "0"]


def _linear_bwd(g2, x2, weight, want_x, want_w, want_b, gskip=None, dw=None, db=None):
    M, K = x2.shape
    N = weight.shape[0]
    dx = None
    if want_x and want_w and want_b and _PAIR[0]:
        if dw is None:
            dw = torch.empty(N, K, dtype=torch.float32, device=g2.device)
        if db is None:
            db = torch.empty(N, dtype=torch.float32, device=g2.device)
        cadd = gskip.reshape(M, K) if gskip is not None else None
        if cadd is not None and cadd.stride(1) != 1:
            cadd = cadd.contiguous()
        dx = torch.empty(M, K, dtype=torch.float32, device=g2.device)
        lib = _lib.load()
        wsx = _ws(lib.e2ep_gemm_workspace(M, K, N), g2.device)
        wsw = _ws(lib.e2ep_gemm_rowsum_workspace(N, K, M), g2.device)
        w2 = weight if weight.stride(1) == 1 else weight.contiguous()
        with timing.region(timing.name("gemm", (M, N, K), "linear_bwd_pair"), 4.0 * M * N * K):
            _lib.call("e2ep_linear_bwd", _lib.ptr(g2), g2.stride(0), _lib.ptr(x2), x2.stride(0),
                      _lib.ptr(w2), w2.stride(0), _lib.ptr(cadd),
                      cadd.stride(0) if cadd is not None else 0, _lib.ptr(dx), dx.stride(0),
                      _lib.ptr(dw), dw.stride(0), _lib.ptr(db), M, N, K, _lib.ptr(wsx),
                      _lib.nbytes(wsx), _lib.ptr(wsw), _lib.nbytes(wsw), _lib.stream())
        return dx, dw, db
    fork = None
    if want_w or want_b:
        if want_w:
            if dw is None:
                dw = torch.empty(N, K, dtype=torch.float32, device=g2.device)
            wsw = _ws(_lib.load().e2ep_gemm_rowsum_workspace(N, K, M) if want_b
                      else _lib.load().e2ep_gemm_workspace(N, K, M), g2.device)
        if want_b:
            if db is None:
                db = torch.empty(N, dtype=torch.float32, device=g2.device)
            wsb = None if want_w else _ws(_lib.load().e2ep_col_sum_workspace(M, N), g2.device)
        fork = conv._Fork(g2.device, on=want_x, work_us=conv.est_us(2.0 * N * K * M))
        with fork:
            if want_w and want_b:
                with timing.region(timing.name("gemm", (N, K, M), "linear_wgrad"), 2.0 * N * K * M):
                    _lib.call("e2ep_gemm_rowsum", _lib.ptr(g2), g2.stride(0), _lib.ptr(x2),
                              x2.stride(0), _lib.ptr(dw), dw.stride(0), _lib.ptr(db), N, K, M,
                              _lib.ptr(wsw), _lib.nbytes(wsw), _lib.stream())
            elif want_w:
                gemm(g2, False, x2, False, N, K, M, out=dw, ws=wsw, tag="linear_wgrad")
            else:
                _lib.call("e2ep_col_sum", _lib.ptr(g2), M, N, _lib.ptr(db), _lib.ptr(wsb),
                          _lib.stream())
    if want_x:
        cadd = gskip.reshape(M, K) if gskip is not None else None
        if cadd is not None and cadd.stride(1) != 1:
            cadd = cadd.contiguous()
        dx = gemm(g2, True, weight, False, M, K, N, cadd=cadd, tag="linear_dgrad")
    if fork is not None:
        fork.join()
    return dx, (dw if want_w else None), (db if want_b else None)


def _rows2(x):
    K = x.shape[-1]
    x2 = x.reshape(-1, K)
    return x2 if (x2.stride(1) == 1 and x2.stride(0) == K) else x2.contiguous()


class _InProjQKV(torch.autograd.Function):

    @staticmethod
    def forward(ctx, xq, xkv, weight, bias, E):
        xq2, xkv2 = _rows2(xq), _rows2(xkv)
        K = xq2.shape[1]
        Wq, Wkv = weight[:E], weight[E:]
        bq, bkv = (None, None) if bias is None else (bias[:E], bias[E:])
        q = gemm(xq2, True, Wq, True, xq2.shape[0], E, K, bias=bq, tag="linear_fwd")
        kv = gemm(xkv2, True, Wkv, True, xkv2.shape[0], 2 * E, K, bias=bkv, tag="linear_fwd")
        ctx.save_for_backward(xq2, xkv2, weight)
        ctx.E, ctx.has_bias, ctx.shapes = E, bias is not None, (xq.shape, xkv.shape)
        ctx.set_materialize_grads(False)
        return q.view(*xq.shape[:-1], E), kv.view(*xkv.shape[:-1], 2 * E), xq, xkv
# ... 158 lines not shown
```

e2e-parking-carla_amd/e2ep_amd/train.py:

```python
import os

import torch
import torch.distributed as dist

from . import _lib, graphs, segments
from .optim import FlatAdam

BUCKET_MB = 25.0


def _rig_key(batch):
    k, e = batch.get("intrinsics"), batch.get("extrinsics")
    if not (torch.is_tensor(k) and torch.is_tensor(e)):
        return None
    k, e = k.detach().float().cpu().contiguous(), e.detach().float().cpu().contiguous()
    return (tuple(k.shape), tuple(e.shape), k.numpy().tobytes(), e.numpy().tobytes())


class GradBuckets:

    def __init__(self, params, opt, flat, bucket_mb=BUCKET_MB):
        self.params, self.opt, self.flat = params, opt, flat
        self.cuda = flat.is_cuda
        cap = int(bucket_mb * 2 ** 20) // 4
        spans = opt.spans
        self.buckets = []
        i1 = len(params)
        while i1 > 0:
            i0, n = i1, 0
            while i0 > 0 and (n == 0 or n + spans[i0 - 1][1] <= cap):
                i0 -= 1
                n += spans[i0][1]
            lo = spans[i0][0]
            hi = flat.numel() if i1 == len(params) else spans[i1][0]
            self.buckets.append((i0, i1, lo, hi))
            i1 = i0
        self.of = {}
        for b, (i0, i1, _, _) in enumerate(self.buckets):
            for i in range(i0, i1):
                self.of[i] = b
        self.comm = torch.cuda.Stream(device=flat.device) if self.cuda else None
        self.has = torch.zeros(len(params), dtype=torch.int64, device=flat.device)
        self.active = False
        self._handles = [p.register_post_accumulate_grad_hook(self._hook_for(i))
                         for i, p in enumerate(params)]

    def _hook_for(self, i):
        def hook(_p):
            if self.active:
                self._arrived(i)
        return hook

    def arm(self):
        self.pending = [i1 - i0 for (i0, i1, _, _) in self.buckets]
        self.streams = [[] for _ in self.buckets]
        self.next = 0
        self.works = []
        self.active = True
        if self.cuda:
            self.main = torch.cuda.current_stream()
            self.capturing = torch.cuda.is_current_stream_capturing()

    def _arrived(self, i):
        b = self.of[i]
        if self.cuda and not self.capturing:
            here = torch.cuda.current_stream()
            if here != self.main and all(here != s for s in self.streams[b]):
                self.streams[b].append(here)
        self.pending[b] -= 1
        while self.next < len(self.buckets) and self.pending[self.next] == 0:
            self._launch(self.next)
            self.next += 1

    def _launch(self, b):
        i0, i1, lo, hi = self.buckets[b]
        if not self.cuda:
            self.opt.prepare(params=(i0, i1))
            self.opt.gather_grads(self.flat, params=(i0, i1))
            self.works.append(dist.all_reduce(self.flat[lo:hi], async_op=True))
            return
        ev = torch.cuda.Event()
        ev.record(self.main)
        self.comm.wait_event(ev)
        for st in self.streams[b]:
            ev2 = torch.cuda.Event()
            ev2.record(st)
            self.comm.wait_event(ev2)
        with torch.cuda.stream(self.comm):
            if not self.capturing:
                self.opt.prepare(params=(i0, i1))
            self.opt.gather_grads(self.flat, params=(i0, i1))
            self.works.append(dist.all_reduce(self.flat[lo:hi], async_op=True))

    def finish(self):
        while self.next < len(self.buckets):
            self._launch(self.next)
            self.next += 1
        for w in self.works:
            w.wait()
        if self.cuda:
            self.main.wait_stream(self.comm)
        self.opt.prepare()
        self.opt.has_grad(self.has)
        dist.all_reduce(self.has, op=dist.ReduceOp.MAX)
        self.works = []
        self.active = False


class TrainStep:

    def __init__(self, module, batch, lr=1e-4, weight_decay=1e-4, world=1, graph=True,
                 warmup=3, optimizer=None, bucket_mb=BUCKET_MB, overlap=None, ddp=None,
                 segment=True, max_grad_norm=None, skip_nonfinite=None, accumulate=None):
        self.module = module
        self.batch = batch
        self.world = world
        self.ddp = world > 1 if ddp is None else bool(ddp)
        self.graph = graph
        self.params = [p for p in module.parameters() if p.requires_grad]
        self.opt = optimizer if optimizer is not None else FlatAdam(
            self.params, lr=lr, weight_decay=weight_decay)
        cfg = getattr(module, "cfg", None)
        skip_given = skip_nonfinite is not None
        if max_grad_norm is None:
            max_grad_norm = getattr(cfg, "gradient_clip_val", None)
        if not skip_given:
            skip_nonfinite = getattr(cfg, "skip_nonfinite_steps", None)
        if accumulate is None:
            accumulate = getattr(cfg, "accumulate_grad_batches", None)
        self.accumulate = 1 if accumulate is None else int(accumulate)
        if self.accumulate < 1:
            raise ValueError(f"TrainStep: accumulate must be >= 1, got {accumulate}")
        if isinstance(self.opt, FlatAdam):
            if max_grad_norm is not None:
                self.opt.max_grad_norm = float(max_grad_norm)
            if skip_given or skip_nonfinite:
                self.opt.skip_nonfinite = bool(skip_nonfinite)
        elif max_grad_norm is not None or skip_nonfinite or self.accumulate > 1:
            raise ValueError("TrainStep: max_grad_norm, skip_nonfinite and accumulate need a "
                             "FlatAdam optimizer")
        self._micro = 0
        dev = self.params[0].device
        flat = self.ddp or self.accumulate > 1
        self.flat_grad = (torch.zeros(self.opt.numel, dtype=torch.float32, device=dev)
                          if flat else None)
        self.has_grad = (torch.zeros(len(self.params), dtype=torch.int64, device=dev)
                         if flat else None)
        self.backend = dist.get_backend() if self.ddp else None
        if overlap is None:
            overlap = os.environ.get("E2EP_DDP_OVERLAP", "1") != "0"
        self._bucket_mb = bucket_mb
        self.overlap = bool(self.ddp and overlap and not graph and self.accumulate == 1 and
                            (self.backend == "nccl" or not self.flat_grad.is_cuda))
        self.buckets = (GradBuckets(self.params, self.opt, self.flat_grad, bucket_mb)
                        if self.overlap else None)
        if self.buckets is not None:
            self.has_grad = self.buckets.has
        self._host = (torch.empty(self.opt.numel, dtype=torch.float32, pin_memory=True)
                      if self.ddp and self.backend != "nccl" and not self.overlap
                      and self.flat_grad.is_cuda else None)
        self.loss = None
        self.g_bwd = self.g_gather = self.g_acc = self.g_opt = None
        self.segmented = bool(segment and self.ddp and graph and self.accumulate == 1 and
                              (self.backend == "nccl" or self._host is not None))
        self.g_s1 = self.g_s1g = self.g_s2 = self.g_s2g = None
        self.seg_buckets = None
        self._rig = _rig_key(batch)
        self._test_skip = None
        self._plans = []
        if graph:
            self._plans = [m.prepare_capture(batch) for m in module.modules()
                           if hasattr(m, "prepare_capture")]
            self._capture(warmup)

    def _fwd_bwd(self):
        self.opt.zero_grad(set_to_none=True)
        if self.buckets is not None:
            self.buckets.arm()
        loss = self.module.training_step(self.batch, 0)
        if getattr(self, "_one", None) is None or self._one.device != loss.device:
            self._one = torch.ones((), dtype=loss.dtype, device=loss.device)
        loss.backward(self._one)
        if self.buckets is not None:
            self.buckets.finish()
        return loss.detach()

    def _gather(self):
        if self.ddp and self.buckets is None:
            self.opt.gather_grads(self.flat_grad)
            self.opt.has_grad(self.has_grad)

    def _allreduce(self):
        if not self.ddp or self.buckets is not None:
            return
        if self._host is None:
            dist.all_reduce(self.flat_grad)
            dist.all_reduce(self.has_grad, op=dist.ReduceOp.MAX)
            return
        self._host.copy_(self.flat_grad, non_blocking=True)
        has = self.has_grad.cpu()
        torch.cuda.current_stream().synchronize()
        dist.all_reduce(self._host)
        dist.all_reduce(has, op=dist.ReduceOp.MAX)
        self.flat_grad.copy_(self._host, non_blocking=True)
        self.has_grad.copy_(has, non_blocking=True)

    def _update(self):
        if self.flat_grad is not None:
            self.opt.step(self.flat_grad, 1.0 / (self.world * self.accumulate),
                          has_grad=self.has_grad)
        else:
            self.opt.step()

    def _accumulate(self, first):
        self.opt.accumulate_grads(self.flat_grad, first)
        self.opt.has_grad(self.has_grad, union=not first)

    def _eager(self):
        loss = self._fwd_bwd()
        self.opt.prepare()
        if self.accumulate > 1:
            k = self._micro
            self._accumulate(k == 0)
            if k == self.accumulate - 1:
                self._allreduce()
                self._update()
            self._micro = (k + 1) % self.accumulate
            return loss
        self._gather()
        self._allreduce()
        self._update()
        return loss

    def _stage1(self):
        self.opt.zero_grad(set_to_none=True)
        with segments.record() as rec:
            loss = self.module.training_step(self.batch, 0)
        self._pairs = rec.pairs
        loss.backward()
        return loss.detach()

    def _stage2(self):
        segments.backward_rest(self._pairs)

    def _buckets_of(self, i0, i1, bucket_mb):
        cap = int(bucket_mb * 2 ** 20) // 4
        spans, out = self.opt.spans, []
        end = self.opt.numel if i1 == len(self.params) else spans[i1][0]
        j1 = i1
        while j1 > i0:
            j0, n = j1, 0
            while j0 > i0 and (n == 0 or n + spans[j0 - 1][1] <= cap):
                j0 -= 1
                n += spans[j0][1]
            lo = spans[j0][0]
            out.append((lo, end))
            end, j1 = lo, j0
        return out

    def _capture_segmented(self, bucket_mb):
        segments.ensure_anchor(self.params[0].device)
        g1, loss, _ = graphs.capture(self._stage1)
        if not self._pairs:
            return False
        has1 = [p.grad is not None for p in self.params]
        if not any(has1):
            return False
        i1 = has1.index(True)
        if not all(has1[i1:]):
            return False
        self.opt.prepare(params=(i1, len(self.params)))
        g1g, _, _ = graphs.capture(lambda: self.opt.gather_grads(self.flat_grad,
                                                                 params=(i1, len(self.params))),
                                   pool=g1.pool())
        marks = segments.grad_marks(self.params[i1:])
        g2, _, _ = graphs.capture(self._stage2, pool=g1.pool())
        if not segments.stage2_leaves_stage1(self.params[i1:], marks):
            return False
        self.opt.prepare()
        if i1 > 0:
            g2g, _, _ = graphs.capture(lambda: self.opt.gather_grads(self.flat_grad, params=(0, i1)),
                                       pool=g1.pool())
        else:
            g2g = None
        self.g_s1, self.g_s1g, self.g_s2, self.g_s2g, self.loss = g1, g1g, g2, g2g, loss
        self.seg_buckets = (self._buckets_of(i1, len(self.params), bucket_mb),
                            self._buckets_of(0, i1, bucket_mb))
        self.comm = torch.cuda.Stream(device=self.flat_grad.device)
        self.opt.has_grad(self.has_grad)
        if self._host is None:
            dist.all_reduce(self.has_grad, op=dist.ReduceOp.MAX)
        else:
            has = self.has_grad.cpu()
            dist.all_reduce(has, op=dist.ReduceOp.MAX)
            self.has_grad.copy_(has)
        return True

    def _replay_segmented(self):
        if self._host is not None:
            self._replay_segmented_host()
            return
        main = torch.cuda.current_stream()
        works = []

        def issue(stage, ranges):
            ev = torch.cuda.Event()
            ev.record(main)
            self.comm.wait_event(ev)
            with torch.cuda.stream(self.comm):
                for j, (lo, hi) in enumerate(ranges):
                    if self._test_skip != (stage, j):
                        works.append(dist.all_reduce(self.flat_grad[lo:hi], async_op=True))

        self.g_s1.replay()
        self.g_s1g.replay()
        issue(0, self.seg_buckets[0])
        self.g_s2.replay()
        if self.g_s2g is not None:
            self.g_s2g.replay()
        issue(1, self.seg_buckets[1])
        for w in works:
            w.wait()
        self.g_opt.replay()

    def _replay_segmented_host(self):
        main = torch.cuda.current_stream()
        h, flat = self._host, self.flat_grad

        def copy_out(ranges):
            ev = torch.cuda.Event()
            ev.record(main)
            self.comm.wait_event(ev)
            with torch.cuda.stream(self.comm):
                for lo, hi in ranges:
                    h[lo:hi].copy_(flat[lo:hi], non_blocking=True)
            done = torch.cuda.Event()
            done.record(self.comm)
            return done

        def exchange(stage, ranges, done):
            done.synchronize()
            works = [dist.all_reduce(h[lo:hi], async_op=True)
                     for j, (lo, hi) in enumerate(ranges) if self._test_skip != (stage, j)]
            for w in works:
                w.wait()
            with torch.cuda.stream(self.comm):
                for lo, hi in ranges:
                    flat[lo:hi].copy_(h[lo:hi], non_blocking=True)

        self.g_s1.replay()
        self.g_s1g.replay()
        d1 = copy_out(self.seg_buckets[0])
        self.g_s2.replay()
        exchange(0, self.seg_buckets[0], d1)
        if self.g_s2g is not None:
            self.g_s2g.replay()
        exchange(1, self.seg_buckets[1], copy_out(self.seg_buckets[1]))
        main.wait_stream(self.comm)
        self.g_opt.replay()

    def _capture(self, warmup):
        s = torch.cuda.Stream()
        s.wait_stream(torch.cuda.current_stream())
        with torch.cuda.stream(s):
            for _ in range(warmup):
                self._eager()
        torch.cuda.current_stream().wait_stream(s)
        torch.cuda.synchronize()
        if self.segmented:
            self.segmented = self._capture_segmented(self._bucket_mb)
            if self.segmented:
                self.g_opt, _, _ = graphs.capture(self._update, pool=self.g_s1.pool())
                return
            self.opt.zero_grad(set_to_none=True)
            self._pairs = None
        self.g_bwd, self.loss, self.memsets = graphs.capture(self._fwd_bwd)
        self.opt.prepare()
        if self.accumulate > 1:
            self.g_gather, _, _ = graphs.capture(lambda: self._accumulate(True),
                                                 pool=self.g_bwd.pool())
            self.g_acc, _, _ = graphs.capture(lambda: self._accumulate(False),
                                              pool=self.g_bwd.pool())
        elif self.ddp and self.buckets is None:
            self.g_gather, _, _ = graphs.capture(self._gather, pool=self.g_bwd.pool())
        self.g_opt, _, _ = graphs.capture(self._update, pool=self.g_bwd.pool())

    def __call__(self, batch=None):
        if batch is not None:
            if self.graph and _rig_key(batch) != self._rig:
                raise _lib.E2EPError(
                    "TrainStep(graph=True) captured the lift-splat plan of the first batch's "
                    "camera rig; this batch has different intrinsics/extrinsics (build a new "
                    "TrainStep, or use graph=False, which plans every batch's rig)")
            for k, v in batch.items():
                if torch.is_tensor(v) and torch.is_tensor(self.batch.get(k)) and self.batch[k].is_cuda:
                    self.batch[k].copy_(v, non_blocking=True)
# ... 28 lines not shown
```

include/e2ep.h:

```cpp
#ifndef E2EP_H
#define E2EP_H

#include <stddef.h>
#include <stdint.h>

#ifdef __cplusplus
extern "C" {
#endif

#define E2EP_EINVAL (-1)
#define E2EP_ERANGE (-2)

int e2ep_abi_version(void);
const char *e2ep_last_error(void);


#define E2EP_IO_X_BF16 1
#define E2EP_IO_DY_BF16 2
#define E2EP_IO_DX_BF16 4


int e2ep_rig_transforms(const float *K, const float *E, int BN, float *combine, float *trans,
                        void *stream);

// ... 168 lines not shown
                         void *stream);

int e2ep_attn_fwd(const float *q, const float *k, const float *v, int B, int H, int Sq, int Sk,
                  int dh, int q_ss, int q_sb, int kv_ss, int kv_sb, int o_ss, int o_sb,
                  float scale, int causal, const uint8_t *key_pad, float p, const int32_t *seed,
                  float *o, float *lse, void *stream);
int e2ep_attn_weights(const float *q, const float *k, const float *lse, int B, int H, int Sq,
                      int Sk, int dh, int q_ss, int q_sb, int kv_ss, int kv_sb, float scale,
                      int causal, const uint8_t *key_pad, int average, float *w, void *stream);
size_t e2ep_attn_bwd_workspace(int B, int H, int Sq);
int e2ep_attn_bwd(const float *q, const float *k, const float *v, const float *o, const float *dout,
                  const float *lse, int B, int H, int Sq, int Sk, int dh, int q_ss, int q_sb,
                  int kv_ss, int kv_sb, int o_ss, int o_sb, float scale, int causal,
                  const uint8_t *key_pad, float p, const int32_t *seed, float *dq, float *dk,
                  float *dv, void *workspace, void *stream);
int e2ep_attn_bwd_part(const float *q, const float *k, const float *v, const float *o,
                       const float *dout, const float *lse, int B, int H, int Sq, int Sk, int dh,
                       int q_ss, int q_sb, int kv_ss, int kv_sb, int o_ss, int o_sb, float scale,
                       int causal, const uint8_t *key_pad, float p, const int32_t *seed, float *dq,
                       float *dk, float *dv, void *workspace, int part, void *stream);
int e2ep_attn_keep_mask(const int32_t *seed, int BH, int Sq, int Sk, float p, uint8_t *out,
                        void *stream);
int e2ep_softmax_c_fwd(const float *x, int N, int C, int HW, float *y, void *stream);
int e2ep_softmax_c_bwd(const float *y, const float *dy, int N, int C, int HW, float *dx,
                       void *stream);
int e2ep_relu_dropout_fwd(const float *x, long long n, float p, const int32_t *seed, float *y,
                          void *stream);
int e2ep_relu_dropout_bwd(const float *x, const float *dy, long long n, float p,
                          const int32_t *seed, float *dx, void *stream);

int e2ep_resize_fwd(const float *x, int N, int C, long long x_nstride, int Hi, int Wi, int Ho,
                    int Wo, float scale_h, float scale_w, float *y, long long y_nstride,
                    void *stream);
size_t e2ep_resize_bwd_workspace(int planes, int Ho, int Wi);
int e2ep_resize_bwd(const float *g, long long g_pstride, int planes, int Hi, int Wi, int Ho,
                    int Wo, float scale_h, float scale_w, float *gx, int accumulate,
                    void *workspace, void *stream);
int e2ep_resize_bwd_cl(const float *g, long long g_pstride, int N, int C, int Hi, int Wi, int Ho,
                       int Wo, float scale_h, float scale_w, float *gxT, void *stream);

int e2ep_dwconv_fwd(const float *x, const float *w, const int *dims, const float *in_scale,
                    const float *in_shift, int in_act, float *y, void *stream);
int e2ep_dwconv_fwd_stats_tiles(const int *dims);
int e2ep_dwconv_fwd_stats(const float *x, const float *w, const int *dims, const float *in_scale,
                          const float *in_shift, int in_act, void *y, double *stats,
                          size_t stats_bytes, void *stream, int io);
int e2ep_dwconv_dgrad(const void *gy, const float *w, const int *dims, void *dx, void *stream,
                      int io);
int e2ep_dwconv_bwd_pair_ok(const int *dims);
int e2ep_dwconv_bf16_ok(const int *dims);
int e2ep_dwconv_bwd(const void *gy, const float *x, const float *w, const int *dims,
                    const float *in_scale, const float *in_shift, int in_act, void *dx,
                    void *workspace, size_t workspace_bytes, float *dw, void *stream,
                    int io );
size_t e2ep_dwconv_wgrad_workspace(const int *dims);
int e2ep_dwconv_wgrad(const void *gy, const float *x, const int *dims, const float *in_scale,
                      const float *in_shift, int in_act, void *workspace, size_t workspace_bytes,
                      float *dw, void *stream, int io );

int e2ep_maxpool3s2_fwd(const float *x, int planes, int H, int W, float *y, int8_t *arg,
                        void *stream);
int e2ep_maxpool3s2_bwd(const float *gy, const int8_t *arg, int planes, int H, int W, float *dx,
                        void *stream);
int e2ep_avgpool_fwd(const float *x, int planes, int HW, float *y, void *stream);
int e2ep_avgpool_bwd(const float *gy, int planes, int HW, float *dx, void *stream);
int e2ep_se_gate_fwd(const float *x, const float *a, int planes, int HW, float *y, void *stream);
int e2ep_se_gate_bwd(const float *x, const float *a, const float *dy, int planes, int HW,
                     float *dx, float *da, void *stream);

int e2ep_fusion_tokens_fwd(const float *bev, const float *motion, const float *pos, int B, int C,
                           int S, int E, float p, const int32_t *seed, float *tokens,
                           void *stream);
int e2ep_fusion_tokens_bwd(const float *dtokens, int B, int C, int S, int E, float p,
                           const int32_t *seed, float *dbev, float *dmotion, float *dpos,
                           void *stream);
int e2ep_embed_tokens_fwd(const int64_t *tok, int tok_stride, const float *table, int V,
                          const float *pos, int B, int T, int E, float p, const int32_t *seed,
                          float *out, void *stream);
int e2ep_tokens_init(const int64_t *prefix, int prefix_stride, int B, int L, int64_t *seq, int T,
                     int64_t pad, void *stream);
int e2ep_token_argmax_append(const float *logits, long long row_stride, int B, int V,
                             int64_t *seq, int seq_stride, int pos, void *stream);
int e2ep_embed_tokens_bwd(const float *dout, const int64_t *tok, int tok_stride, int V, int B,
                          int T, int E, float p, const int32_t *seed, float *dtable, float *dpos,
                          void *stream);

int e2ep_dec_self_attn(const float *x, int ldx, const float *gamma, const float *beta, float eps,
                       const float *table, int V, const float *pos, float *x0, const int64_t *seq,
                       int seq_stride, int64_t pad, const float *w_in, const float *b_in,
                       float *cache, float *out, int B, int T, int t, int E, int H, void *stream);
int e2ep_dec_cross_attn(const float *x, int ldx, const float *gamma, const float *beta, float eps,
                        const float *w_q, const float *b_q, const float *kv, int ldkv, float *out,
                        int B, int Sk, int E, int H, void *stream);
int e2ep_dec_row_gemv(const float *x, int ldx, const float *gamma, const float *beta, float eps,
                      const float *w, const float *bias, const float *res, int ldr,
                      const float *res_gamma, const float *res_beta, float res_eps, float *out,
                      int ldo, int B, int N, int K, int relu, void *stream);

int e2ep_adam_chunk_elems(void);
int e2ep_adam_step(const int *chunks, int n_chunks, const long long *offsets,
                   const long long *grad_ptrs, const float *grad_flat, float *param, float *exp_avg,
                   float *exp_avg_sq, float *step, const double *lr, double beta1, double beta2,
                   double eps, double weight_decay, float grad_scale, int *stepped,
                   void *stream);
int e2ep_grad_gather(const int *chunks, int n_chunks, const long long *offsets,
                     const long long *grad_ptrs, float *grad_flat, void *stream);
int e2ep_grad_sqnorm(const int *chunks, int n_chunks, const long long *offsets,
                     const long long *grad_ptrs, const float *grad_flat, double *partials,
                     void *stream);
int e2ep_grad_norm_finalize(const double *partials, int n_chunks, float grad_scale,
                            double max_norm, int skip_nonfinite, double *norm, float *clip_coef,
                            int *skip, long long *skipped, void *stream);
int e2ep_adam_step_clipped(const int *chunks, int n_chunks, const long long *offsets,
                           const long long *grad_ptrs, const float *grad_flat, float *param,
                           float *exp_avg, float *exp_avg_sq, float *step, const double *lr,
                           double beta1, double beta2, double eps, double weight_decay,
                           float grad_scale, const float *clip_coef, const int *skip,
                           int *stepped, void *stream);
int e2ep_grad_accumulate(const int *chunks, int n_chunks, const long long *offsets,
                         const long long *grad_ptrs, float *grad_flat, void *stream);

size_t e2ep_control_ce_workspace(int rows);
int e2ep_control_ce_fwd(const float *logits, const long long *gt, int B, int T, int gt_stride,
                        int gt_offset, int vocab, int pad, float *loss, float *lse, float *count,
                        void *workspace, void *stream);
int e2ep_control_ce_bwd(const float *logits, const long long *gt, const float *lse,
                        const float *count, const float *gloss, int B, int T, int gt_stride,
                        int gt_offset, int vocab, int pad, float *dlogits, void *stream);
size_t e2ep_seg_ce_workspace(int images, int HW);
int e2ep_seg_ce_fwd(const float *logits, const long long *target, const float *weights, int images,
                    int C, int HW, int ignore, float *loss, void *workspace, void *stream);
int e2ep_seg_ce_bwd(const float *logits, const long long *target, const float *weights,
                    const float *gloss, int images, int C, int HW, int ignore, float *dlogits,
                    void *stream);
size_t e2ep_depth_bce_workspace(int BN, int H, int W, int down);
int e2ep_depth_bce_fwd(const float *prob, const float *gt, int BN, int D, int H, int W, int down,
                       float lo, float step, float *loss, float *den, int *cls, void *workspace,
                       void *stream);
int e2ep_depth_bce_fwd_f64(const float *prob, const double *gt, int BN, int D, int H, int W,
                           int down, double lo, double step, float *loss, float *den, int *cls,
                           void *workspace, void *stream);
int e2ep_depth_bce_bwd(const float *prob, const int *cls, const float *den, const float *gloss,
                       int BN, int D, int hw, float *dprob, void *stream);

size_t e2ep_gemm_workspace(int M, int N, int K);
int e2ep_gemm_force(int tile, int splits, int unused);
int e2ep_gemm_skinny(int max_rows);
int e2ep_gemm_precision(int precision);
int e2ep_gemm_split_min(int ksteps);

int e2ep_bn_small(int on);
int e2ep_bn_small_limits(int fwd_max_vec, int bwd_max_vec);
int e2ep_tune(int key, int value);
int e2ep_gemm(const float *A, int lda, int a_kcontig, const float *B, int ldb, int b_kcontig,
              const float *bias, const float *Cadd, int ldadd, float *C, int ldc, int M, int N,
              int K, int relu, void *workspace, size_t workspace_bytes, void *stream);
size_t e2ep_gemm_rowsum_workspace(int M, int N, int K);
int e2ep_gemm_rowsum(const float *A, int lda, const float *B, int ldb, float *C, int ldc,
                     float *rowsum, int M, int N, int K, void *workspace,
                     size_t workspace_bytes, void *stream);
int e2ep_linear_bwd(const float *dy, int ldy, const float *x, int ldx, const float *w, int ldw,
                    const float *gskip, int ldskip, float *dx, int lddx, float *dw, int lddw,
                    float *db, int M, int N, int K, void *ws_dx, size_t ws_dx_bytes, void *ws_dw,
                    size_t ws_dw_bytes, void *stream);

int e2ep_decode_frames(const void *rgb, const void *depth_rgb, const long long *src_frame,
                       long long frames, int hw, float *image, double *depth, void *stream);
int e2ep_widen_u8_i64(const void *src, const long long *src_row, long long rows, int row_len,
                      long long *dst, void *stream);

int e2ep_decode_bgra(const void *bgra, int N, int H, int W, int crop, float *image, void *rgb,
                     void *stream);
size_t e2ep_slot_stats_workspace(int B, int X);
int e2ep_slot_partials(const float *logits, long long stride_b, long long stride_c,
                       long long stride_x, long long stride_y, int B, int C, int X, int Y,
                       int target_class, const unsigned char *class_lut, void *class_image,
                       void *workspace, size_t workspace_bytes, void *stream);
int e2ep_slot_finish(const void *workspace, size_t workspace_bytes, int B, int X, int Y,
                     double res_x, double res_y, float *state, int32_t *found, int64_t *stats,
                     const int64_t *seq, int seq_stride, int seq_len, int first, int token_nums,
                     double *controls, int64_t *tokens_out, void *stream);
int e2ep_target_select(const float *state, const float *goal, int B, float *target,
                       void *stream);

int e2ep_graph_replace_memsets(void *graph, int *replaced);
int e2ep_graph_exec_create(void *graph, void **exec);
int e2ep_capture_unjoined(void *origin, void *side, int *unjoined);
int e2ep_graph_exec_launch(void *exec, void *stream);
int e2ep_graph_exec_destroy(void *exec);

#ifdef __cplusplus
}
#endif
#endif
```

Before: 396.4 samples/s.

## Defer and batch parameter-gradient reduction kernels into grouped launches per backward

Adds a deferral scope that records split-K reductions, LayerNorm gamma/beta gradient reductions and SE weight-gradient kernels during backward. At the end of the scope it issues them as a few batched kernels that look up their record through a binary search on block index. This cuts the many small launches in backward and the per-launch overhead, and lets the reductions run with more blocks in flight. The cost is keeping workspace tensors alive until the flush, host mutex and bookkeeping on every call, and more complex ordering. Batches are split whenever the same output appears twice, which preserves accumulation order.

```diff
diff --git a/e2e-parking-carla_amd/csrc/abi.cpp b/e2e-parking-carla_amd/csrc/abi.cpp
--- a/e2e-parking-carla_amd/csrc/abi.cpp
+++ b/e2e-parking-carla_amd/csrc/abi.cpp
@@ -12,7 +12,7 @@
   vsnprintf(g_err, sizeof(g_err), fmt, ap);
   va_end(ap);
 }
-int g_tune[TUNE_N] = {8192, 4096, 512, 512, 768, 1024, 512, 1, 1, 2, 1, 2, 2, 1, 2, 1, 1, 1, 1, 1, 1, 2, 1024, 2, 2048, 2, 1, 1, 2, 1, 2, 1, 1, 1, 1, 4, 2};
+int g_tune[TUNE_N] = {8192, 4096, 512, 512, 768, 1024, 512, 1, 1, 2, 1, 2, 2, 1, 2, 1, 1, 1, 1, 1, 1, 2, 1024, 2, 2048, 2, 1, 1, 2, 1, 2, 1, 1, 1, 1, 4, 2, 2};
 }
 
 extern "C" {
diff --git a/e2e-parking-carla_amd/csrc/conv.hip b/e2e-parking-carla_amd/csrc/conv.hip
--- a/e2e-parking-carla_amd/csrc/conv.hip
+++ b/e2e-parking-carla_amd/csrc/conv.hip
@@ -5,6 +5,7 @@
 #include "gemm.h"
 #include "bnstats.h"
 #include "handoff.h"
+#include "pgrad.h"
 
 #pragma clang fp contract(on)
 
@@ -1096,28 +1097,7 @@
                                                         int accumulate, int RS,
                                                         unsigned long long mask) {
   __shared__ float red[16][64];
-  const int o = threadIdx.x & 63, r = threadIdx.x >> 6;
-  const int i = blockIdx.x * 64 + o;
-  const bool live = (mask >> (i % RS)) & 1ULL;
-  float s0 = 0.f, s1 = 0.f, s2 = 0.f, s3 = 0.f;
-  if (i < n && live) {
-    int k = r;
-    for (; k + 48 < splits; k += 64) {
-      s0 += part[(size_t)(k + 0) * n + i];
-      s1 += part[(size_t)(k + 16) * n + i];
-      s2 += part[(size_t)(k + 32) * n + i];
-      s3 += part[(size_t)(k + 48) * n + i];
-    }
-    for (; k < splits; k += 16) s0 += part[(size_t)k * n + i];
-  }
-  red[r][o] = (s0 + s1) + (s2 + s3);
-  __syncthreads();
-  if (r == 0 && i < n) {
-    float s = 0.f;
-#pragma unroll
-    for (int j = 0; j < 16; ++j) s += red[j][o];
-    out[i] = accumulate ? out[i] + s : s;
-  }
+  reduce_splits_block(part, splits, n, out, accumulate, RS, mask, (int)blockIdx.x, red);
 }
 
 __global__ void __launch_bounds__(256) k_reduce_splits4(const float *__restrict__ part, int splits,
@@ -1126,31 +1106,17 @@
                                                          unsigned long long mask) {
   const int i = (blockIdx.x * 256 + threadIdx.x) * 4;
   if (i >= n) return;
-  float4 acc = *reinterpret_cast<const float4 *>(part + i);
-#pragma unroll 8
-  for (int k = 1; k < splits; ++k) {
-    const float4 v = *reinterpret_cast<const float4 *>(part + (size_t)k * n + i);
-    acc.x += v.x;
-    acc.y += v.y;
-    acc.z += v.z;
-    acc.w += v.w;
-  }
-  float r[4] = {acc.x, acc.y, acc.z, acc.w};
-#pragma unroll
-  for (int e = 0; e < 4; ++e)
-    if (!((mask >> ((i + e) % RS)) & 1ULL)) r[e] = 0.f;
-  float4 o = make_float4(r[0], r[1], r[2], r[3]);
-  if (accumulate) {
-    const float4 a = *reinterpret_cast<const float4 *>(out + i);
-    o.x += a.x; o.y += a.y; o.z += a.z; o.w += a.w;
-  }
-  *reinterpret_cast<float4 *>(out + i) = o;
+  reduce_splits4_thread(part, splits, n, out, accumulate, RS, mask, i);
 }
 
 static void reduce_splits(const float *part, int splits, int n, float *out, int accumulate, int RS,
                           unsigned long long mask, hipStream_t s) {
-  if (n % 4 == 0 && n >= 131072 && splits <= 64 && (reinterpret_cast<uintptr_t>(part) & 15) == 0 &&
-      (reinterpret_cast<uintptr_t>(out) & 15) == 0)
+  const bool f4 = n % 4 == 0 && n >= 131072 && splits <= 64 &&
+                  (reinterpret_cast<uintptr_t>(part) & 15) == 0 &&
+                  (reinterpret_cast<uintptr_t>(out) & 15) == 0;
+  if (pgrad_defer(SlabRec{part, out, mask, n, splits, RS, (accumulate ? 1 : 0) | (f4 ? 2 : 0)}))
+    return;
+  if (f4)
     hipLaunchKernelGGL(k_reduce_splits4, dim3(cdiv(n / 4, 256)), dim3(256), 0, s, part, splits, n,
                        out, accumulate, RS, mask);
   else
diff --git a/e2e-parking-carla_amd/csrc/ln.hip b/e2e-parking-carla_amd/csrc/ln.hip
--- a/e2e-parking-carla_amd/csrc/ln.hip
+++ b/e2e-parking-carla_amd/csrc/ln.hip
@@ -1,5 +1,6 @@
 #include "common.h"
 #include "dropout.h"
+#include "pgrad.h"
 
 namespace e2ep {
 
@@ -121,21 +122,7 @@
                                                          int E, float *__restrict__ dgamma,
                                                          float *__restrict__ dbeta) {
   __shared__ float red[16][64];
-  const int o = threadIdx.x & 63, r = threadIdx.x >> 6;
-  const int c = blockIdx.x * 64 + o;
-  const float *pp = part + (size_t)blockIdx.y * nblk * E;
-  float s = 0.f;
-  if (c < E)
-    for (int k = r; k < nblk; k += 16) s += pp[(size_t)k * E + c];
-  red[r][o] = s;
-  __syncthreads();
-  if (r == 0 && c < E) {
-    float t = 0.f;
-#pragma unroll
-    for (int j = 0; j < 16; ++j) t += red[j][o];
-    float *out = blockIdx.y == 0 ? dgamma : dbeta;
-    if (out) out[c] = t;
-  }
+  ln_param_grads_block(part, nblk, E, dgamma, dbeta, (int)blockIdx.x, (int)blockIdx.y, red);
 }
 
 }
@@ -189,7 +176,7 @@
   E2EP_REQUIRE(!(dgamma || dbeta) || workspace, E2EP_EINVAL, "e2ep_add_drop_ln_bwd: workspace needed");
   hipLaunchKernelGGL(k_add_drop_ln_bwd, dim3(nblk), dim3(256), 0, stream, dy, x, mean, rstd,
                      gamma, u, seed, p, scale, rows, E, da, db, part);
-  if (part)
+  if (part && !pgrad_defer(LnRec{part, dgamma, dbeta, nblk, E}))
     hipLaunchKernelGGL(k_ln_param_grads, dim3(cdiv(E, 64), 2), dim3(1024), 0, stream, part, nblk,
                        E, dgamma, dbeta);
   return launch_status("e2ep_add_drop_ln_bwd");
diff --git a/e2e-parking-carla_amd/csrc/pgrad.h b/e2e-parking-carla_amd/csrc/pgrad.h
--- /dev/null
+++ b/e2e-parking-carla_amd/csrc/pgrad.h
@@ -0,0 +1,139 @@
+#pragma once
+#include "common.h"
+
+namespace e2ep {
+
+
+__device__ __forceinline__ void reduce_splits_block(const float *__restrict__ part, int splits, int n,
+                                                    float *__restrict__ out, int accumulate, int RS,
+                                                    unsigned long long mask, int blk,
+                                                    float (*red)[64]) {
+  const int o = threadIdx.x & 63, r = threadIdx.x >> 6;
+  const int i = blk * 64 + o;
+  const bool live = (mask >> (i % RS)) & 1ULL;
+  float s0 = 0.f, s1 = 0.f, s2 = 0.f, s3 = 0.f;
+  if (i < n && live) {
+    int k = r;
+    for (; k + 48 < splits; k += 64) {
+      s0 += part[(size_t)(k + 0) * n + i];
+      s1 += part[(size_t)(k + 16) * n + i];
+      s2 += part[(size_t)(k + 32) * n + i];
+      s3 += part[(size_t)(k + 48) * n + i];
+    }
+    for (; k < splits; k += 16) s0 += part[(size_t)k * n + i];
+  }
+  red[r][o] = (s0 + s1) + (s2 + s3);
+  __syncthreads();
+  if (r == 0 && i < n) {
+    float s = 0.f;
+#pragma unroll
+    for (int j = 0; j < 16; ++j) s += red[j][o];
+    out[i] = accumulate ? out[i] + s : s;
+  }
+}
+
+__device__ __forceinline__ void reduce_splits4_thread(const float *__restrict__ part, int splits,
+                                                      int n, float *__restrict__ out,
+                                                      int accumulate, int RS,
+                                                      unsigned long long mask, int i) {
+  float4 acc = *reinterpret_cast<const float4 *>(part + i);
+#pragma unroll 8
+  for (int k = 1; k < splits; ++k) {
+    const float4 v = *reinterpret_cast<const float4 *>(part + (size_t)k * n + i);
+    acc.x += v.x;
+    acc.y += v.y;
+    acc.z += v.z;
+    acc.w += v.w;
+  }
+  float r[4] = {acc.x, acc.y, acc.z, acc.w};
+#pragma unroll
+  for (int e = 0; e < 4; ++e)
+    if (!((mask >> ((i + e) % RS)) & 1ULL)) r[e] = 0.f;
+  float4 o = make_float4(r[0], r[1], r[2], r[3]);
+  if (accumulate) {
+    const float4 a = *reinterpret_cast<const float4 *>(out + i);
+    o.x += a.x; o.y += a.y; o.z += a.z; o.w += a.w;
+  }
+  *reinterpret_cast<float4 *>(out + i) = o;
+}
+
+__device__ __forceinline__ void ln_param_grads_block(const float *__restrict__ part, int nblk, int E,
+                                                     float *__restrict__ dgamma,
+                                                     float *__restrict__ dbeta, int bx, int by,
+                                                     float (*red)[64]) {
+  const int o = threadIdx.x & 63, r = threadIdx.x >> 6;
+  const int c = bx * 64 + o;
+  const float *pp = part + (size_t)by * nblk * E;
+  float s = 0.f;
+  if (c < E)
+    for (int k = r; k < nblk; k += 16) s += pp[(size_t)k * E + c];
+  red[r][o] = s;
+  __syncthreads();
+  if (r == 0 && c < E) {
+    float t = 0.f;
+#pragma unroll
+    for (int j = 0; j < 16; ++j) t += red[j][o];
+    float *out = by == 0 ? dgamma : dbeta;
+    if (out) out[c] = t;
+  }
+}
+
+__device__ __forceinline__ void se_wgrad_thread(const float *__restrict__ pooled,
+                                                const float *__restrict__ hpre,
+                                                const float *__restrict__ da,
+                                                const float *__restrict__ dhpre, int N, int C, int sq,
+                                                float *__restrict__ dw1, float *__restrict__ db1,
+                                                float *__restrict__ dw2, float *__restrict__ db2,
+                                                int i) {
+  const int n1 = sq * C, n2 = C * sq;
+  float s = 0.f;
+  if (i < n1) {
+    const int k = i / C, c = i - k * C;
+#pragma unroll 8
+    for (int n = 0; n < N; ++n) s += dhpre[(size_t)n * sq + k] * pooled[(size_t)n * C + c];
+    if (dw1) dw1[i] = s;
+  } else if (i < n1 + n2) {
+    const int j = i - n1, c = j / sq, k = j - c * sq;
+#pragma unroll 8
+    for (int n = 0; n < N; ++n) {
+      const float z = hpre[(size_t)n * sq + k];
+      s += da[(size_t)n * C + c] * (z * sigmoid_f(z));
+    }
+    if (dw2) dw2[j] = s;
+  } else if (i < n1 + n2 + sq) {
+    const int k = i - n1 - n2;
+#pragma unroll 8
+    for (int n = 0; n < N; ++n) s += dhpre[(size_t)n * sq + k];
+    if (db1) db1[k] = s;
+  } else if (i < n1 + n2 + sq + C) {
+    const int c = i - n1 - n2 - sq;
+#pragma unroll 8
+    for (int n = 0; n < N; ++n) s += da[(size_t)n * C + c];
+    if (db2) db2[c] = s;
+  }
+}
+
+
+struct SlabRec {
+  const float *part;
+  float *out;
+  unsigned long long mask;
+  int n, splits, RS;
+  int flags;
+};
+struct LnRec {
+  const float *part;
+  float *dgamma, *dbeta;
+  int nblk, E;
+};
+struct SeRec {
+  const float *pooled, *hpre, *da, *dhpre;
+  float *dw1, *db1, *dw2, *db2;
+  int N, C, sq;
+};
+
+bool pgrad_defer(const SlabRec &r);
+bool pgrad_defer(const LnRec &r);
+bool pgrad_defer(const SeRec &r);
+
+}
diff --git a/e2e-parking-carla_amd/csrc/pgrad.hip b/e2e-parking-carla_amd/csrc/pgrad.hip
--- /dev/null
+++ b/e2e-parking-carla_amd/csrc/pgrad.hip
@@ -0,0 +1,174 @@
+#include <mutex>
+#include <vector>
+
+#include "pgrad.h"
+
+namespace e2ep {
+
+constexpr int SLAB_BATCH = 64;
+constexpr int LN_BATCH = 64;
+constexpr int SE_BATCH = 32;
+
+template <typename Rec, int MAX>
+struct Batch {
+  Rec r[MAX];
+  int first[MAX + 1];
+  int count;
+};
+
+template <typename Rec, int MAX>
+__device__ __forceinline__ int batch_find(const Batch<Rec, MAX> &t, int b) {
+  int lo = 0, hi = t.count;
+  while (hi - lo > 1) {
+    const int mid = (lo + hi) >> 1;
+    if (t.first[mid] <= b) lo = mid;
+    else hi = mid;
+  }
+  return lo;
+}
+
+__global__ void __launch_bounds__(1024) k_reduce_splits_batch(const Batch<SlabRec, SLAB_BATCH> t) {
+  __shared__ float red[16][64];
+  const int j = batch_find(t, (int)blockIdx.x);
+  const SlabRec &r = t.r[j];
+  const int blk = (int)blockIdx.x - t.first[j];
+  if (r.flags & 2) {
+    const int i = (blk * 1024 + (int)threadIdx.x) * 4;
+    if (i < r.n) reduce_splits4_thread(r.part, r.splits, r.n, r.out, r.flags & 1, r.RS, r.mask, i);
+  } else {
+    reduce_splits_block(r.part, r.splits, r.n, r.out, r.flags & 1, r.RS, r.mask, blk, red);
+  }
+}
+
+__global__ void __launch_bounds__(1024) k_ln_param_grads_batch(const Batch<LnRec, LN_BATCH> t) {
+  __shared__ float red[16][64];
+  const int j = batch_find(t, (int)blockIdx.x);
+  const LnRec &r = t.r[j];
+  const int blk = (int)blockIdx.x - t.first[j], gx = (r.E + 63) / 64;
+  ln_param_grads_block(r.part, r.nblk, r.E, r.dgamma, r.dbeta, blk % gx, blk / gx, red);
+}
+
+__global__ void __launch_bounds__(256) k_se_wgrad_batch(const Batch<SeRec, SE_BATCH> t) {
+  const int j = batch_find(t, (int)blockIdx.x);
+  const SeRec &r = t.r[j];
+  const int blk = (int)blockIdx.x - t.first[j];
+  se_wgrad_thread(r.pooled, r.hpre, r.da, r.dhpre, r.N, r.C, r.sq, r.dw1, r.db1, r.dw2, r.db2,
+                  blk * 256 + (int)threadIdx.x);
+}
+
+static std::mutex g_mu;
+static bool g_open = false;
+static int g_hold = 0;
+static std::vector<SlabRec> g_slabs;
+static std::vector<LnRec> g_lns;
+static std::vector<SeRec> g_ses;
+
+static bool defer_on(bool slabs) {
+  const int v = g_tune[TUNE_PGRAD_DEFER];
+  return g_open && !g_hold && (v == 2 || (v == 3 && slabs));
+}
+
+bool pgrad_defer(const SlabRec &r) {
+  std::lock_guard<std::mutex> lk(g_mu);
+  if (!defer_on(true)) return false;
+  g_slabs.push_back(r);
+  return true;
+}
+bool pgrad_defer(const LnRec &r) {
+  std::lock_guard<std::mutex> lk(g_mu);
+  if (!defer_on(false)) return false;
+  g_lns.push_back(r);
+  return true;
+}
+bool pgrad_defer(const SeRec &r) {
+  std::lock_guard<std::mutex> lk(g_mu);
+  if (!defer_on(false)) return false;
+  g_ses.push_back(r);
+  return true;
+}
+
+static int blocks_of(const SlabRec &r) {
+  return (r.flags & 2) ? cdiv(r.n / 4, 1024) : cdiv(r.n, 64);
+}
+static int blocks_of(const LnRec &r) { return cdiv(r.E, 64) * 2; }
+static int blocks_of(const SeRec &r) { return cdiv(2 * r.sq * r.C + r.sq + r.C, 256); }
+
+static bool repeats(const SlabRec *r, int have) {
+  for (int k = 0; k < have; ++k)
+    if (r[k].out == r[have].out) return true;
+  return false;
+}
+static bool repeats(const LnRec *, int) { return false; }
+static bool repeats(const SeRec *, int) { return false; }
+
+template <typename Rec, int MAX, typename K>
+static void flush_kind(const std::vector<Rec> &recs, K kernel, int threads, hipStream_t s) {
+  size_t at = 0;
+  while (at < recs.size()) {
+    Batch<Rec, MAX> t;
+    int c = 0, blocks = 0;
+    for (; c < MAX && at + c < recs.size() && !(c > 0 && repeats(&recs[at], c)); ++c) {
+      t.r[c] = recs[at + c];
+      t.first[c] = blocks;
+      blocks += blocks_of(t.r[c]);
+    }
+    for (int k = c; k <= MAX; ++k) t.first[k] = blocks;
+    for (int k = c; k < MAX; ++k) t.r[k] = Rec{};
+    t.count = c;
+    hipLaunchKernelGGL(kernel, dim3(blocks), dim3(threads), 0, s, t);
+    at += c;
+  }
+}
+
+}
+
+using namespace e2ep;
+
+extern "C" {
+
+int e2ep_defer_begin(void) {
+  std::lock_guard<std::mutex> lk(g_mu);
+  E2EP_REQUIRE(!g_open, E2EP_EINVAL, "e2ep_defer_begin: a deferral scope is already open");
+  g_open = true;
+  g_hold = 0;
+  return 0;
+}
+
+int e2ep_defer_flush(void *stream) {
+  std::lock_guard<std::mutex> lk(g_mu);
+  E2EP_REQUIRE(g_open, E2EP_EINVAL, "e2ep_defer_flush: no deferral scope is open");
+  hipStream_t s = as_stream(stream);
+  flush_kind<SlabRec, SLAB_BATCH>(g_slabs, k_reduce_splits_batch, 1024, s);
+  flush_kind<LnRec, LN_BATCH>(g_lns, k_ln_param_grads_batch, 1024, s);
+  flush_kind<SeRec, SE_BATCH>(g_ses, k_se_wgrad_batch, 256, s);
+  g_slabs.clear();
+  g_lns.clear();
+  g_ses.clear();
+  g_open = false;
+  g_hold = 0;
+  return launch_status("e2ep_defer_flush");
+}
+
+int e2ep_defer_abort(void) {
+  std::lock_guard<std::mutex> lk(g_mu);
+  g_slabs.clear();
+  g_lns.clear();
+  g_ses.clear();
+  g_open = false;
+  g_hold = 0;
+  return 0;
+}
+
+int e2ep_defer_pending(void) {
+  std::lock_guard<std::mutex> lk(g_mu);
+  return (int)(g_slabs.size() + g_lns.size() + g_ses.size());
+}
+
+int e2ep_defer_hold(int hold) {
+  std::lock_guard<std::mutex> lk(g_mu);
+  const int prev = g_hold;
+  g_hold = hold ? 1 : 0;
+  return prev;
+}
+
+}
diff --git a/e2e-parking-carla_amd/csrc/se.hip b/e2e-parking-carla_amd/csrc/se.hip
--- a/e2e-parking-carla_amd/csrc/se.hip
+++ b/e2e-parking-carla_amd/csrc/se.hip
@@ -1,4 +1,5 @@
 #include "common.h"
+#include "pgrad.h"
 
 #pragma clang fp contract(on)
 
@@ -328,33 +329,8 @@
                                                   int sq, float *__restrict__ dw1,
                                                   float *__restrict__ db1, float *__restrict__ dw2,
                                                   float *__restrict__ db2) {
-  const int i = blockIdx.x * blockDim.x + threadIdx.x;
-  const int n1 = sq * C, n2 = C * sq;
-  float s = 0.f;
-  if (i < n1) {
-    const int k = i / C, c = i - k * C;
-#pragma unroll 8
-    for (int n = 0; n < N; ++n) s += dhpre[(size_t)n * sq + k] * pooled[(size_t)n * C + c];
-    if (dw1) dw1[i] = s;
-  } else if (i < n1 + n2) {
-    const int j = i - n1, c = j / sq, k = j - c * sq;
-#pragma unroll 8
-    for (int n = 0; n < N; ++n) {
-      const float z = hpre[(size_t)n * sq + k];
-      s += da[(size_t)n * C + c] * (z * sigm(z));
-    }
-    if (dw2) dw2[j] = s;
-  } else if (i < n1 + n2 + sq) {
-    const int k = i - n1 - n2;
-#pragma unroll 8
-    for (int n = 0; n < N; ++n) s += dhpre[(size_t)n * sq + k];
-    if (db1) db1[k] = s;
-  } else if (i < n1 + n2 + sq + C) {
-    const int c = i - n1 - n2 - sq;
-#pragma unroll 8
-    for (int n = 0; n < N; ++n) s += da[(size_t)n * C + c];
-    if (db2) db2[c] = s;
-  }
+  se_wgrad_thread(pooled, hpre, da, dhpre, N, C, sq, dw1, db1, dw2, db2,
+                  (int)(blockIdx.x * blockDim.x + threadIdx.x));
 }
 
 __global__ void __launch_bounds__(256) k_se_dx(const float *__restrict__ dy,
@@ -501,7 +477,8 @@
   hipLaunchKernelGGL(k_se_dh, dim3(N, spans), dim3(256), 0, s, da, w2, C, sq, KT, dhp);
   hipLaunchKernelGGL(k_se_dpooled, dim3(N, cdiv(C, 256)), dim3(256), 0, s, dhp, spans, hpre, w1,
                      C, sq, dhpre, dpooled);
-  if (dw1 || db1 || dw2 || db2) {
+  if ((dw1 || db1 || dw2 || db2) &&
+      !pgrad_defer(SeRec{pooled, hpre, da, dhpre, dw1, db1, dw2, db2, N, C, sq})) {
     const int outs = 2 * sq * C + sq + C;
     hipLaunchKernelGGL(k_se_wgrad, dim3(cdiv(outs, 256)), dim3(256), 0, s, pooled, hpre, da, dhpre,
                        N, C, sq, dw1, db1, dw2, db2);
diff --git a/e2e-parking-carla_amd/csrc/tune.h b/e2e-parking-carla_amd/csrc/tune.h
--- a/e2e-parking-carla_amd/csrc/tune.h
+++ b/e2e-parking-carla_amd/csrc/tune.h
@@ -39,7 +39,8 @@
   TUNE_SE_EXCITE_MLP = 34,
   TUNE_STEM_DIRECT = 35,
   TUNE_MBCONV_MID = 36,
-  TUNE_N = 37
+  TUNE_PGRAD_DEFER = 37,
+  TUNE_N = 38
 };
 extern int g_tune[TUNE_N];
 }
diff --git a/e2e-parking-carla_amd/e2ep_amd/_lib.py b/e2e-parking-carla_amd/e2ep_amd/_lib.py
--- a/e2e-parking-carla_amd/e2ep_amd/_lib.py
+++ b/e2e-parking-carla_amd/e2ep_amd/_lib.py
@@ -146,6 +146,11 @@
     "e2ep_bn_small": (_i, [_i]),
     "e2ep_bn_small_limits": (_i, [_i, _i]),
     "e2ep_tune": (_i, [_i, _i]),
+    "e2ep_defer_begin": (_i, []),
+    "e2ep_defer_flush": (_i, [_p]),
+    "e2ep_defer_abort": (_i, []),
+    "e2ep_defer_pending": (_i, []),
+    "e2ep_defer_hold": (_i, [_i]),
     "e2ep_gemm": (_i, [_p, _i, _i, _p, _i, _i, _p, _p, _i, _p, _i, _i, _i, _i, _i, _p, _sz, _p]),
     "e2ep_gemm_rowsum_workspace": (_sz, [_i, _i, _i]),
     "e2ep_gemm_rowsum": (_i, [_p, _i, _p, _i, _p, _i, _p, _i, _i, _i, _p, _sz, _p]),
diff --git a/e2e-parking-carla_amd/e2ep_amd/bev_stem.py b/e2e-parking-carla_amd/e2ep_amd/bev_stem.py
--- a/e2e-parking-carla_amd/e2ep_amd/bev_stem.py
+++ b/e2e-parking-carla_amd/e2ep_amd/bev_stem.py
@@ -1,6 +1,6 @@
 import torch
 
-from . import _lib, conv, timing
+from . import _lib, conv, defer, timing
 
 
 class _BevStem(torch.autograd.Function):
@@ -27,6 +27,7 @@
                           torch.empty(B, Cout, P, Q, dtype=torch.float32, device=bev.device), w_layout=1)
         ctx.save_for_backward(x, w, wt)
         ctx.meta = (B, C, X, Y, H, W, sh, sw, dims)
+        ctx.pkeys = defer.note(w)
         return y
 
     @staticmethod
@@ -45,7 +46,7 @@
             fork = conv._Fork(gy.device, on=ctx.needs_input_grad[0],
                               work_us=conv.est_us(conv.conv_flops(dims)))
             with fork:
-                conv.conv_wgrad(gy, x, dims, dw, ws)
+                conv.conv_wgrad(gy, x, dims, dw, ws, ctx.pkeys)
         if ctx.needs_input_grad[0]:
             dres = conv.conv_dgrad(gy, wt, dims, C,
                                    torch.empty(B, C, H, W, dtype=torch.float32, device=gy.device), w_layout=1)
diff --git a/e2e-parking-carla_amd/e2ep_amd/conv.py b/e2e-parking-carla_amd/e2ep_amd/conv.py
--- a/e2e-parking-carla_amd/e2ep_amd/conv.py
+++ b/e2e-parking-carla_amd/e2ep_amd/conv.py
@@ -2,7 +2,7 @@
 
 import torch
 
-from . import _lib, streams, timing
+from . import _lib, defer, streams, timing
 
 
 def _ws(nbytes, device):
@@ -139,12 +139,13 @@
     return dx
 
 
-def conv_wgrad(gy, x, dims, dw, ws=None):
+def conv_wgrad(gy, x, dims, dw, ws=None, pkeys=defer.ANY):
     d = _lib.dims(dims)
     splits = _lib.load().e2ep_conv_wgrad_splits(d)
     if ws is None:
         ws = torch.empty(splits * dw.numel(), dtype=torch.float32, device=gy.device)
-    with timing.region(_rname("conv_wgrad", dims), conv_flops(dims)):
+    with timing.region(_rname("conv_wgrad", dims), conv_flops(dims)), defer.call(pkeys) as dc:
+        dc.keep(ws)
         _lib.call("e2ep_conv_wgrad", _lib.ptr(gy), _lib.ptr(x), d, splits, _lib.ptr(ws), _lib.nbytes(ws),
                   _lib.ptr(dw), 0, _lib.stream(), _io_x(x))
     return dw
@@ -224,7 +225,7 @@
     return prev
 
 
-def _conv_bwd_pair(gy, x, wt, dims, gc, gskip, wshape):
+def _conv_bwd_pair(gy, x, wt, dims, gc, gskip, wshape, pkeys=None):
     N, Cin, H, W = dims[:4]
     lib = _lib.load()
     d = _lib.dims(dims)
@@ -234,7 +235,9 @@
     wsd = _ws(lib.e2ep_conv_dgrad_workspace(d, gc), gy.device)
     res = gskip.contiguous() if (gskip is not None and gc == Cin) else None
     dxg = torch.empty(N, gc, H, W, dtype=x.dtype, device=x.device)
-    with timing.region(_rname("conv_bwd", dims, f"gc{gc}"), conv_flops(dims, gc) + conv_flops(dims)):
+    with timing.region(_rname("conv_bwd", dims, f"gc{gc}"), conv_flops(dims, gc) + conv_flops(dims)), \
+            defer.call(pkeys) as dc:
+        dc.keep(wsw)
         _lib.call("e2ep_conv_bwd", _lib.ptr(gy), _lib.ptr(x), _lib.ptr(wt), d, gc, _lib.ptr(res),
                   _lib.ptr(dxg), _lib.ptr(wsd), _lib.nbytes(wsd), splits, _lib.ptr(wsw),
                   _lib.nbytes(wsw), _lib.ptr(dw), _lib.stream(), (_IO_X | _IO_DX) if _io_x(x) else 0)
@@ -260,6 +263,7 @@
         ctx.dims, ctx.act, ctx.has_bias, ctx.gc = dims, act, b is not None, grad_channels
         ctx.save_for_backward(x, wt, y if act else None)
         ctx.wshape = w.shape
+        ctx.pkeys = defer.note(w)
         ctx.skip = skip
         ctx.set_materialize_grads(False)
         return (y, x) if skip else y
@@ -281,7 +285,7 @@
         xb = x.dtype == torch.bfloat16
         if want_w and ctx.needs_input_grad[0] and _CONV_PAIR[0] and (not xb or gskip is None) and \
                 _lib.load().e2ep_conv_bwd_pair_ok(_lib.dims(dims), gc):
-            dx, dw = _conv_bwd_pair(gy, x, wt, dims, gc, gskip, ctx.wshape)
+            dx, dw = _conv_bwd_pair(gy, x, wt, dims, gc, gskip, ctx.wshape, ctx.pkeys)
             if want_b:
                 db = torch.empty(Cout, dtype=torch.float32, device=x.device)
                 _lib.call("e2ep_bias_grad", _lib.ptr(gy), N, Cout, P * Q, _lib.ptr(db), s)
@@ -297,7 +301,7 @@
             fork = _Fork(x.device, on=ctx.needs_input_grad[0], work_us=est_us(conv_flops(dims)))
             with fork:
                 if want_w:
-                    conv_wgrad(gy, x, dims, dw, ws)
+                    conv_wgrad(gy, x, dims, dw, ws, ctx.pkeys)
                 if want_b:
                     _lib.call("e2ep_bias_grad", _lib.ptr(gy), N, Cout, P * Q, _lib.ptr(db),
                               _lib.stream())
@@ -338,6 +342,7 @@
         _skinny(x2, K, 1, w2, 1, K, b, N, M, K, y)
         ctx.save_for_backward(x2, w2)
         ctx.has_bias, ctx.wshape, ctx.xshape = b is not None, w.shape, x.shape
+        defer.note(w)
         return y.view(N, M, 1, 1)
 
     @staticmethod
diff --git a/e2e-parking-carla_amd/e2ep_amd/defer.py b/e2e-parking-carla_amd/e2ep_amd/defer.py
--- /dev/null
+++ b/e2e-parking-carla_amd/e2ep_amd/defer.py
@@ -0,0 +1,89 @@
+from . import _lib
+
+_SCOPES = []
+
+
+class ParamGradDefer:
+
+    def __init__(self, uses=None):
+        self.uses = {} if uses is None else uses
+        self.keep = []
+
+    def __enter__(self):
+        _lib.call("e2ep_defer_begin")
+        _SCOPES.append(self)
+        return self
+
+    def __exit__(self, *exc):
+        _SCOPES.pop()
+        try:
+            if exc[0] is None and _lib.call_raw("e2ep_defer_pending"):
+                _lib.call("e2ep_defer_flush", _lib.stream())
+            else:
+                _lib.call("e2ep_defer_abort")
+        finally:
+            self.keep = []
+        return False
+
+    def ok(self, keys):
+        if keys is None:
+            return False
+        for k in keys:
+            ent = self.uses.get(k)
+            if ent is None or ent[1] != 1 or not ent[0].is_leaf or ent[0].grad is not None:
+                return False
+        return True
+
+
+def active():
+    return _SCOPES[-1] if _SCOPES else None
+
+
+def note(*params):
+    if not _SCOPES:
+        return None
+    uses = _SCOPES[-1].uses
+    keys = []
+    for p in params:
+        if p is None:
+            continue
+        ent = uses.get(id(p))
+        if ent is None:
+            uses[id(p)] = [p, 1]
+        else:
+            ent[1] += 1
+        keys.append(id(p))
+    return tuple(keys)
+
+
+ANY = object()
+
+
+class call:
+
+    def __init__(self, keys=ANY):
+        self.scope = _SCOPES[-1] if _SCOPES else None
+        self.keys = keys
+        self.tensors = ()
+        self.held = False
+
+    def keep(self, *tensors):
+        self.tensors = tensors
+
+    def __enter__(self):
+        if self.scope is not None:
+            if self.keys is not ANY and not self.scope.ok(self.keys):
+                self.held = True
+                _lib.call_raw("e2ep_defer_hold", 1)
+            else:
+                self.before = _lib.call_raw("e2ep_defer_pending")
+        return self
+
+    def __exit__(self, *exc):
+        if self.scope is None:
+            return False
+        if self.held:
+            _lib.call_raw("e2ep_defer_hold", 0)
+        elif _lib.call_raw("e2ep_defer_pending") > self.before:
+            self.scope.keep.extend(t for t in self.tensors if t is not None)
+        return False
diff --git a/e2e-parking-carla_amd/e2ep_amd/nn_ops.py b/e2e-parking-carla_amd/e2ep_amd/nn_ops.py
--- a/e2e-parking-carla_amd/e2ep_amd/nn_ops.py
+++ b/e2e-parking-carla_amd/e2ep_amd/nn_ops.py
@@ -4,7 +4,7 @@
 import torch
 import torch.nn.functional as F
 
-from . import _lib, conv, rng, timing
+from . import _lib, conv, defer, rng, timing
 
 ACT = {None: 0, "none": 0, "relu": 1, "swish": 2}
 
@@ -605,6 +605,7 @@
                       _lib.ptr(y), _lib.stream(), 0)
         ctx.save_for_backward(x, w1c, w2c, pooled, hpre, a)
         ctx.shapes = (w1.shape, w2.shape, b1 is not None, b2 is not None)
+        ctx.pkeys = defer.note(w1, b1, w2, b2)
         return y
 
     @staticmethod
@@ -621,7 +622,9 @@
         dw2 = torch.empty(w2s, dtype=torch.float32, device=dev) if nig[3] else None
         db2 = torch.empty(C, dtype=torch.float32, device=dev) if (hb2 and nig[4]) else None
         ws = torch.empty(2 * N * C + 17 * N * sq, dtype=torch.float32, device=dev)
-        with timing.region(timing.name("se_bwd", x.shape, "_SqueezeExcite")):
+        with timing.region(timing.name("se_bwd", x.shape, "_SqueezeExcite")), \
+                defer.call(ctx.pkeys) as dc:
+            dc.keep(pooled, hpre, ws)
             _lib.call("e2ep_se_bwd", _lib.ptr(x), None, None, _lib.ptr(dy.contiguous()),
                       _lib.ptr(w1c), _lib.ptr(w2c), _lib.ptr(pooled), _lib.ptr(hpre), _lib.ptr(a),
                       N, C, H * W, sq, _lib.ptr(dx), None, _lib.ptr(dw1), _lib.ptr(db1), _lib.ptr(dw2), _lib.ptr(db2),
@@ -678,6 +681,7 @@
                       (_IO_X | (_IO_DX if yb else 0)) if hb else 0)
         ctx.save_for_backward(x, gamma, beta, stats, w1c, w2c, pooled, hpre, a)
         ctx.shapes = (w1.shape, w2.shape, b1 is not None, b2 is not None)
+        ctx.pkeys = defer.note(w1, b1, w2, b2)
         ctx.train = train
         return y
 
@@ -707,7 +711,9 @@
                  and _lib.load().e2ep_bn_bwd_split(N, C, H, W) == 1)
         if fused:
             planes = torch.empty(N * C * 4, dtype=torch.float64, device=dev)
-            with timing.region(timing.name("se_bwd", x.shape, "_BnSwishSE")):
+            with timing.region(timing.name("se_bwd", x.shape, "_BnSwishSE")), \
+                    defer.call(ctx.pkeys) as dc:
+                dc.keep(pooled, hpre, ws)
                 _lib.call("e2ep_se_bwd_bn", _lib.ptr(x), _lib.ptr(stats[2]), _lib.ptr(stats[3]),
                           _lib.ptr(stats[0]), _lib.ptr(stats[1]), _lib.ptr(gamma), _lib.ptr(beta),
                           _lib.ptr(dy), _lib.ptr(w1c), _lib.ptr(w2c), _lib.ptr(pooled),
@@ -720,7 +726,9 @@
                           _lib.ptr(dpooled), _lib.ptr(planes), N, C, H, W, ACT["swish"],
                           _lib.ptr(dx), _lib.ptr(dg), _lib.ptr(db), s, (io_in | _IO_DX) if hb else 0)
             return dx, dg, db, None, None, None, None, None, dw1, db1, dw2, db2, None, None, None
-        with timing.region(timing.name("se_bwd", x.shape, "_BnSwishSE")):
+        with timing.region(timing.name("se_bwd", x.shape, "_BnSwishSE")), \
+                defer.call(ctx.pkeys) as dc:
+            dc.keep(pooled, hpre, ws)
             _lib.call("e2ep_se_bwd", _lib.ptr(x), _lib.ptr(stats[2]), _lib.ptr(stats[3]),
                       _lib.ptr(dy), _lib.ptr(w1c), _lib.ptr(w2c), _lib.ptr(pooled),
                       _lib.ptr(hpre), _lib.ptr(a), N, C, H * W, sq, None, _lib.ptr(dpooled),
@@ -793,6 +801,7 @@
         ctx.save_for_backward(x, y1, w, g0, b0, st0, g1, b1, st1, w1c, w2c, pooled, hpre, a)
         ctx.dims = dims
         ctx.shapes = (w1.shape, w2.shape, sb1 is not None, sb2 is not None)
+        ctx.pkeys = defer.note(w1, sb1, w2, sb2)
         return y
 
     @staticmethod
@@ -811,7 +820,9 @@
         dsb2 = torch.empty(C, **f32) if (hb2 and nig[18]) else None
         dpooled = torch.empty(N, C, **f32)
         ws = torch.empty(2 * N * C + 17 * N * sq, **f32)
-        with timing.region(timing.name("se_bwd", x.shape, "_MBConvMid")):
+        with timing.region(timing.name("se_bwd", x.shape, "_MBConvMid")), \
+                defer.call(ctx.pkeys) as dc:
+            dc.keep(pooled, hpre, ws)
             _lib.call("e2ep_se_bwd", _lib.ptr(y1), _lib.ptr(st1[2]), _lib.ptr(st1[3]), _lib.ptr(dy),
                       _lib.ptr(w1c), _lib.ptr(w2c), _lib.ptr(pooled), _lib.ptr(hpre), _lib.ptr(a),
                       N, C, 256, sq, None, _lib.ptr(dpooled), _lib.ptr(dw1), _lib.ptr(dsb1),
@@ -972,6 +983,7 @@
                       _lib.ptr(mean), _lib.ptr(rstd), _lib.stream())
         ctx.save_for_backward(x, mean, rstd, gamma, mask)
         ctx.p, ctx.rows, ctx.E, ctx.seeded = float(p), rows, E, seed is not None
+        ctx.pkeys = defer.note(gamma, beta)
         return y
 
     @staticmethod
@@ -983,7 +995,9 @@
         dg = torch.empty_like(gamma) if (gamma is not None and nig[2]) else None
         dbeta = torch.empty_like(gamma) if (gamma is not None and nig[3]) else None
         ws = _ws(_lib.load().e2ep_add_drop_ln_bwd_workspace(ctx.rows, ctx.E), x.device)
-        with timing.region(timing.name("ln_bwd", x.shape, "_AddDropLN")):
+        with timing.region(timing.name("ln_bwd", x.shape, "_AddDropLN")), \
+                defer.call(ctx.pkeys) as dc:
+            dc.keep(ws)
             _lib.call("e2ep_add_drop_ln_bwd_seeded" if ctx.seeded else "e2ep_add_drop_ln_bwd",
                       _lib.ptr(dy.contiguous()), _lib.ptr(x), _lib.ptr(mean),
                       _lib.ptr(rstd), _lib.ptr(gamma), _lib.ptr(mask), ctx.p, ctx.rows, ctx.E,
diff --git a/e2e-parking-carla_amd/e2ep_amd/train.py b/e2e-parking-carla_amd/e2ep_amd/train.py
--- a/e2e-parking-carla_amd/e2ep_amd/train.py
+++ b/e2e-parking-carla_amd/e2ep_amd/train.py
@@ -3,7 +3,7 @@
 import torch
 import torch.distributed as dist
 
-from . import _lib, graphs, segments
+from . import _lib, defer, graphs, segments
 from .optim import FlatAdam
 
 BUCKET_MB = 25.0
@@ -177,12 +177,17 @@
         self.opt.zero_grad(set_to_none=True)
         if self.buckets is not None:
             self.buckets.arm()
+            loss = self._loss_backward()
+            self.buckets.finish()
+            return loss
+        with defer.ParamGradDefer():
+            return self._loss_backward()
+
+    def _loss_backward(self):
         loss = self.module.training_step(self.batch, 0)
         if getattr(self, "_one", None) is None or self._one.device != loss.device:
             self._one = torch.ones((), dtype=loss.dtype, device=loss.device)
         loss.backward(self._one)
-        if self.buckets is not None:
-            self.buckets.finish()
         return loss.detach()
 
     def _gather(self):
@@ -234,14 +239,17 @@
 
     def _stage1(self):
         self.opt.zero_grad(set_to_none=True)
-        with segments.record() as rec:
-            loss = self.module.training_step(self.batch, 0)
-        self._pairs = rec.pairs
-        loss.backward()
+        with defer.ParamGradDefer() as scope:
+            with segments.record() as rec:
+                loss = self.module.training_step(self.batch, 0)
+            self._pairs = rec.pairs
+            loss.backward()
+        self._defer_uses = scope.uses
         return loss.detach()
 
     def _stage2(self):
-        segments.backward_rest(self._pairs)
+        with defer.ParamGradDefer(uses=self._defer_uses):
+            segments.backward_rest(self._pairs)
 
     def _buckets_of(self, i0, i1, bucket_mb):
         cap = int(bucket_mb * 2 ** 20) // 4
diff --git a/include/e2ep.h b/include/e2ep.h
--- a/include/e2ep.h
+++ b/include/e2ep.h
@@ -344,6 +344,13 @@
 int e2ep_bn_small(int on);
 int e2ep_bn_small_limits(int fwd_max_vec, int bwd_max_vec);
 int e2ep_tune(int key, int value);
+
+int e2ep_defer_begin(void);
+int e2ep_defer_flush(void *stream);
+int e2ep_defer_abort(void);
+int e2ep_defer_pending(void);
+int e2ep_defer_hold(int hold);
+
 int e2ep_gemm(const float *A, int lda, int a_kcontig, const float *B, int ldb, int b_kcontig,
               const float *bias, const float *Cadd, int ldadd, float *C, int ldc, int M, int N,
               int K, int relu, void *workspace, size_t workspace_bytes, void *stream);
```

After: 402.3 samples/s, median of 6. +1.5%, better.
